# leejet/stable-diffusion.cpp

Hardware: AMD Instinct MI355X
Metric: denoise it/s (image-iterations/s: cond+uncond UNet forwards per image per step) (higher is better)
Workload: dtype f16; 1 GPU; sd15 UNet 512x512, cfg 7 (cond+uncond), f16 weights, batch 8/GPU, Euler-A step; global_batch=8, flash_attn=True, hip_graph=1, cfg_pair_in_one_graph=True, device_resident_sampler=True

## Files before the change

### include/ggml-mi355x.h

```cpp
#ifndef GGML_MI355X_H
#define GGML_MI355X_H

#include "ggml-abi.h"

#ifdef __cplusplus
extern "C" {
#endif

#define GGML_MI355X_API __attribute__((visibility("default")))

GGML_MI355X_API ggml_backend_reg_t ggml_backend_init(void);
GGML_MI355X_API int ggml_backend_score(void);
GGML_MI355X_API ggml_backend_reg_t ggml_backend_mi355x_reg(void);
GGML_MI355X_API int ggml_backend_mi355x_get_device_count(void);

struct ggml_backend_mi355x_stats {
    int64_t graphs_computed;
    int64_t plans_built;
    int64_t nodes_seen;
    int64_t kernels_planned;
    int64_t kernels_launched;
    int64_t fused_conv;
    int64_t fused_conv_bounced;
    int64_t fused_linear;
    int64_t fused_norm;
    int64_t fused_geglu;
    int64_t fused_attention;
    int64_t generic_matmul;
    int64_t swizzled_weight_bytes;
    int64_t graph_replays;
    int64_t fused_linear_geglu;
    int64_t split_k_gemms;
    int64_t head_major_gemms;
    int64_t fused_modulate;
    int64_t fused_gate;
    int64_t fused_gelu;
    int64_t fused_rope;
    int64_t fused_concat_heads;
    int64_t qgemv_linears;
    int64_t fused_chan_add;
    int64_t fused_proj_tokens;
    int64_t gemm_attention;
    int64_t fused_q16;
    int64_t split_k_inlaunch;
    int64_t qgemm16_linears;
    int64_t fgemv_linears;
    int64_t fused_presilu;
    int64_t fused_sibling_linears;
    int64_t hoisted_kv_linears;
    int64_t window_convs;
    int64_t hoisted_emb_linears;
    int64_t fused_rows16;
    int64_t fused_joint_qkv;
    int64_t jit_images;
    int64_t fused_cat_rows16;
    int64_t fused_gn_stats;
    int64_t fused_ln_reduce;
    int64_t redirect_fallbacks;
    int64_t fused_concat_gn;
    int64_t fused_conv_scale;
    int64_t view_graphs;
    int64_t plans_evicted;
    int64_t hoisted_mod_linears;
    int64_t view_external_nodes;
    int64_t qinloop_linears;
    int64_t flash_out_alias;
    int64_t flash_slice_images;
    int64_t flash_short_launches;
    int64_t flash_qb2_launches;
    int64_t flash_mslot_launches;
    int64_t flash_generic_launches;
    int64_t fused_gn_epilogue;
    int64_t fused_tile_merge;
};
GGML_MI355X_API void ggml_backend_mi355x_get_stats(struct ggml_backend_mi355x_stats* out);
GGML_MI355X_API int ggml_backend_mi355x_resolve_enums(const char* (*op_name)(int), const char* (*unary_op_name)(int), const char* (*type_name)(int));
GGML_MI355X_API const char* ggml_backend_mi355x_enum_status(void);
GGML_MI355X_API void ggml_backend_mi355x_get_enum_maps(uint8_t* ops256, uint8_t* unary256);
struct ggml_backend_mi355x_kernel_timing {
    char kernel[96];
    int64_t launches;
    double total_ms;
    double total_flops;
    double total_bytes;
    int32_t bound;
    int32_t family;
};
GGML_MI355X_API void ggml_backend_mi355x_kernel_timing_enable(int enable);
GGML_MI355X_API void ggml_backend_mi355x_kernel_timing_enable_mask(uint32_t family_mask);
GGML_MI355X_API void ggml_backend_mi355x_get_kernel_timing(struct ggml_backend_mi355x_kernel_timing* out);
GGML_MI355X_API int ggml_backend_mi355x_get_kernel_timings(struct ggml_backend_mi355x_kernel_timing* out, int capacity);
GGML_MI355X_API void ggml_backend_mi355x_set_option(const char* key, int value);
struct ggml_backend_mi355x_calibration {
    float mfma_f16_tflops;
    float mfma_clock_mhz;
    float copy_tbs;
    float read_tbs;
    int compute_units;
};
GGML_MI355X_API int ggml_backend_mi355x_calibrate(struct ggml_backend_mi355x_calibration* out);
GGML_MI355X_API void* ggml_backend_mi355x_get_stream(ggml_backend_t backend);
GGML_MI355X_API bool ggml_backend_mi355x_step_cache_probe(ggml_backend_t backend, const float* x, float c_in, const float* prev_in, int64_t n, float* stats);
GGML_MI355X_API bool ggml_backend_mi355x_step_cache_record(ggml_backend_t backend, const float* in, const float* out, float* prev_in, float* prev_out, float* diff, int64_t per,
                                                           int k, int64_t nb, bool has_prev_out, float* stats);
GGML_MI355X_API bool ggml_backend_mi355x_step_cache_probe_rel(ggml_backend_t backend, const float* x, float c_in, const float* prev_in, int64_t n, float* stats);
GGML_MI355X_API bool ggml_backend_mi355x_spectrum_predict(ggml_backend_t backend, const float* ring, int64_t slot_stride, const int* order, int k, const float* weights, float w,
                                                          int64_t n, float* out);
GGML_MI355X_API bool ggml_backend_mi355x_spectrum_push(ggml_backend_t backend, const float* src, float* dst, int64_t n);
GGML_MI355X_API const char* ggml_backend_mi355x_hip_library(void);
GGML_MI355X_API int ggml_backend_mi355x_set_device(int hip_device);
GGML_MI355X_API int ggml_backend_mi355x_get_device(void);

#ifdef __cplusplus
}
#endif
#endif
```

### include/sd-mi355x.h

```cpp
#ifndef SD_MI355X_H
#define SD_MI355X_H

#include <stdbool.h>
#include <stddef.h>
#include <stdint.h>

#ifdef __cplusplus
extern "C" {
#endif

#define SD_API __attribute__((visibility("default")))

enum sd_model_family_t {
    SD_MODEL_SD15       = 0,
    SD_MODEL_SDXL       = 1,
    SD_MODEL_SD15_TINY  = 2,
    SD_MODEL_SDXL_TINY  = 3,
    SD_MODEL_SD35_LARGE = 4,
    SD_MODEL_SD35_TINY  = 5,
    SD_MODEL_FLUX_DEV   = 6,
    SD_MODEL_FLUX_TINY  = 7,
    SD_MODEL_SD35_WIDE2 = 8,
    SD_MODEL_FLUX_WIDE1 = 9,
    SD_MODEL_SD3M_TINY  = 10,
// ... 139 lines not shown
    SDM_CACHE_CACHE_DIT  = 5,
    SDM_CACHE_SPECTRUM   = 6
};
typedef struct {
    enum sdm_cache_mode_t mode;
    float reuse_threshold;
    float start_percent;
    float end_percent;
    float error_decay_rate;
    bool use_relative_threshold;
    bool reset_error_on_compute;
} sdm_cache_params_t;
SD_API void sdm_cache_params_init(sdm_cache_params_t* p);
SD_API bool sd_set_step_cache(sdm_ctx_t* ctx, const sdm_cache_params_t* params);
typedef struct {
    int Fn_compute_blocks;
    int Bn_compute_blocks;
    float residual_diff_threshold;
} sdm_cache_dit_params_t;
typedef struct {
    float w;
    int m;
    float lam;
    int window_size;
    float flex_window;
    int warmup_steps;
    float stop_percent;
} sdm_spectrum_params_t;
SD_API void sdm_cache_dit_params_init(sdm_cache_dit_params_t* p);
SD_API void sdm_spectrum_params_init(sdm_spectrum_params_t* p);
SD_API bool sd_set_step_cache_ex(sdm_ctx_t* ctx, const sdm_cache_params_t* params, const sdm_cache_dit_params_t* cache_dit, const sdm_spectrum_params_t* spectrum);
typedef struct {
    int step;
    float sigma;
    bool active;
    bool skipped;
    float input_change;
    float output_change;
    float output_norm;
    float rate;
    float accumulated;
    float threshold;
} sdm_cache_step_t;
SD_API int sd_step_cache_trace(sdm_ctx_t* ctx, sdm_cache_step_t* out, int capacity);
SD_API const char* sd_step_cache_status(sdm_ctx_t* ctx);
SD_API bool sd_step_cache_device_passes(sdm_ctx_t* ctx);
SD_API float sd_t_to_sigma(sdm_ctx_t* ctx, float t);
SD_API bool sd_step_cache_kernels(sdm_ctx_t* ctx, const float* in, const float* out, const float* prev_in, const float* prev_out, int64_t n, int k, int nb, float c_in,
                                  float* stats, float* diff_out, float* prev_in_out, float* prev_out_out);
SD_API bool sd_step_cache_kernels_rel(sdm_ctx_t* ctx, const float* in, const float* prev_in, int64_t n, float c_in, float* sums);
SD_API bool sd_spectrum_schedule(const sdm_spectrum_params_t* params, int n_calls, uint8_t* predicted);
SD_API bool sd_spectrum_weights(const sdm_spectrum_params_t* params, const float* taus, int k, float tau_at, float* weights);
SD_API bool sd_spectrum_kernels(sdm_ctx_t* ctx, const float* hist, int k, int64_t n, const float* weights, float w, float* out);

SD_API void sd_philox_randn(uint64_t seed, uint32_t offset, uint32_t n, float* out);
SD_API void sd_philox_uint32(uint64_t seed, uint32_t offset, uint32_t n, uint32_t* out );
SD_API int sd_get_sigmas(int steps, float* out );
typedef bool (*sd_pair_exchange_fn)(void* device_eps, int64_t count, void* stream, void* user);
SD_API void sd_set_pair_exchange(sdm_ctx_t* ctx, sd_pair_exchange_fn fn, void* user, int branch);
SD_API bool sd_rccl_get_unique_id(void* id128);
SD_API void* sd_rccl_comm_create(int device, int nranks, int rank, const void* id128);
SD_API void sd_rccl_comm_destroy(void* comm);
SD_API bool sd_set_pair_exchange_rccl(sdm_ctx_t* ctx, void* comm, int branch);
SD_API const char* sd_rccl_last_error(void);
SD_API void sd_set_guidance(sdm_ctx_t* ctx, float guidance);
SD_API void sd_cfg_combine(const float* cond, const float* uncond, int64_t n, float scale, float* out);
SD_API void sd_planar_rgb_to_u8(const float* chw, int width, int height, uint8_t* out);
SD_API int sd_sample_synthetic(int family, int steps, int image_seq_len, int64_t n, uint64_t seed, int method, float eta, float* out, float* aux);
SD_API int sd_sample_synthetic2(int family, int steps, int image_seq_len, int64_t n, uint64_t seed, int method, int scheduler, float eta, float* out, float* aux, int aux_calls);
SD_API int sd_get_sigmas_sched(int family, int scheduler, int steps, int image_seq_len, float shift, float* out);
SD_API void sd_apg_sequence(const float* cond, const float* uncond, int64_t n, int steps, float scale, float eta, float momentum, float norm_threshold,
                            float norm_threshold_smoothing, float* out);
SD_API bool sd_set_vae_conv2d_scale(sdm_ctx_t* ctx, float scale);
SD_API int sd_get_flux_sigmas(int steps, int image_seq_len, float* out );
SD_API int sd_gen_flux_pe(int h, int w, int patch_size, int context_len, const int* axes_dim, int n_axes, float theta, float* out);
SD_API int sd_get_flow_sigmas(int steps, float shift, float* out );
SD_API float sd_sigma_to_t(float sigma);

struct ggml_tensor;
struct ggml_cgraph;
struct ggml_backend;
typedef bool (*sdm_graph_eval_callback_t)(struct ggml_tensor* t, bool ask, void* user_data);
SD_API void sdm_set_backend_eval_callback(sdm_graph_eval_callback_t cb, void* user_data);
SD_API int sdm_backend_graph_compute_with_eval_callback(struct ggml_backend* backend, struct ggml_cgraph* gf, sdm_graph_eval_callback_t cb, void* user_data);

SD_API size_t sdm_graph_describe(struct ggml_cgraph* gf, char* buf, size_t cap);
SD_API void sdm_set_graph_capture(int on);
SD_API size_t sdm_last_graph_description(char* buf, size_t cap);

typedef struct {
    double last_sample_ms;
    double last_decode_ms;
    int64_t unet_calls;
    int64_t graph_nodes;
    size_t compute_buffer_bytes;
    size_t weight_bytes;
    double host_build_ms, host_alloc_ms, host_submit_ms;
    int64_t graph_cache_hits;
    int64_t steps_skipped;
} sd_stats_t;
SD_API void sd_get_stats(sdm_ctx_t* ctx, sd_stats_t* out);
typedef struct {
    const int32_t* ids;
    const float* weights;
    int n;
} sd_token_list_t;
SD_API bool sd_text_encoders_init(sdm_ctx_t* ctx);
SD_API int64_t sd_clip_forward(sdm_ctx_t* ctx, int which, const int32_t* ids, int n_tokens, int max_token_idx, bool return_pooled, int clip_skip, float* out,
                               int64_t out_capacity);
SD_API int64_t sd_t5_forward(sdm_ctx_t* ctx, const int32_t* ids, int n_tokens, float* out, int64_t out_capacity);
SD_API int sd_t5_relative_position_buckets(int q_len, int k_len, int32_t* out );
SD_API bool sd_get_learned_condition(sdm_ctx_t* ctx, const sd_token_list_t* clip_l, const sd_token_list_t* clip_g, const sd_token_list_t* t5, int clip_skip,
                                     int width, int height, bool zero_out_masked, float* crossattn_out, int64_t crossattn_capacity, int64_t* crossattn_ne,
                                     float* vector_out, int64_t vector_capacity, int64_t* vector_n);


#ifdef __cplusplus
}
#endif
#endif
```

### stable-diffusion.cpp_amd/__init__.py

```python
from __future__ import annotations

import ctypes as C
import os
from pathlib import Path

import numpy as np

PKG_DIR = Path(__file__).resolve().parent
ROOT = PKG_DIR.parent
LIB_DIR = PKG_DIR / "lib"
HOST_LIB = Path(os.environ.get("SDCPP_HOST_LIB", str(LIB_DIR / "libsdcpp-host.so")))
BACKEND_LIB = Path(os.environ.get("SDCPP_BACKEND_LIB", str(LIB_DIR / "libggml-mi355x.so")))

F32, F16, Q4_0, Q8_0, I32, BF16 = 0, 1, 2, 8, 26, 30
TYPE_SIZE = {F32: 4, F16: 2, BF16: 2, I32: 4}

SD15, SDXL, SD15_TINY, SDXL_TINY, SD35_LARGE, SD35_TINY, FLUX_DEV, FLUX_TINY, SD35_WIDE2, FLUX_WIDE1, SD3M_TINY, SD35_WIDE8, FLUX_WIDE8 = 0, 1, 2, 3, 4, 5, 6, 7, 8, 9, 10, 11, 12
PAIR_EXCHANGE_FN = C.CFUNCTYPE(C.c_bool, C.c_void_p, C.c_int64, C.c_void_p, C.c_void_p)
EVAL_CALLBACK_FN = C.CFUNCTYPE(C.c_bool, C.c_void_p, C.c_bool, C.c_void_p)
EULER, EULER_A, HEUN, DPM2, DPMPP2S_A, DPMPP2M, DPMPP2Mv2, IPNDM, IPNDM_V, LCM, DDIM_TRAILING = range(11)
TCD, RES_MULTISTEP, RES_2S, ER_SDE, EULER_CFG_PP, EULER_A_CFG_PP, EULER_GE, DPMPP2M_SDE, DPMPP2M_SDE_BT, LMS = range(11, 21)
SAMPLE_METHOD_DEFAULT = 21
SCHED_DISCRETE, SCHED_KARRAS, SCHED_EXPONENTIAL, SCHED_AYS, SCHED_GITS, SCHED_SGM_UNIFORM, SCHED_SIMPLE, SCHED_SMOOTHSTEP, SCHED_KL_OPTIMAL, SCHED_LCM = range(10)
SCHED_BONG_TANGENT, SCHED_FLUX, SCHED_BETA, SCHEDULER_DEFAULT = 10, 14, 15, 16
# ... 28 lines not shown
    _fields_ = [("mem_size", C.c_size_t), ("mem_buffer", C.c_void_p), ("no_alloc", C.c_bool)]


class SdCtxParams(C.Structure):
    _fields_ = [
        ("backend", C.c_char_p),
        ("model", C.c_int),
        ("wtype", C.c_int),
        ("diffusion_flash_attn", C.c_bool),
        ("diffusion_conv_direct", C.c_bool),
        ("vae_decode_only", C.c_bool),
        ("weight_seed", C.c_uint64),
        ("n_threads", C.c_int),
    ]


class SdSampleParams(C.Structure):
    _fields_ = [("txt_cfg", C.c_float), ("scheduler", C.c_int), ("sample_method", C.c_int),
                ("sample_steps", C.c_int), ("eta", C.c_float), ("custom_sigmas", C.c_void_p), ("custom_sigmas_count", C.c_int),
                ("slg_layers", C.c_void_p), ("slg_layer_count", C.c_int), ("slg_layer_start", C.c_float), ("slg_layer_end", C.c_float), ("slg_scale", C.c_float),
                ("apg_eta", C.c_float), ("apg_momentum", C.c_float), ("apg_norm_threshold", C.c_float), ("apg_norm_threshold_smoothing", C.c_float),
                ("shifted_timestep", C.c_int), ("flow_shift", C.c_float)]


class SdCondition(C.Structure):
    _fields_ = [("c_crossattn", C.POINTER(C.c_float)), ("ctx_dim", C.c_int64), ("n_tokens", C.c_int64),
                ("c_vector", C.POINTER(C.c_float)), ("vector_dim", C.c_int64)]


class SdImgGenParams(C.Structure):
    _fields_ = [("cond", SdCondition), ("uncond", SdCondition), ("width", C.c_int), ("height", C.c_int),
                ("sample_params", SdSampleParams), ("seed", C.c_int64), ("batch_count", C.c_int),
                ("device_batch", C.c_int), ("decode", C.c_bool), ("fuse_cfg_pair", C.c_bool), ("device_sampler", C.c_bool),
                ("init_latent", C.c_void_p), ("denoise_mask", C.c_void_p), ("strength", C.c_float)]


class SdTokenList(C.Structure):
    _fields_ = [("ids", C.POINTER(C.c_int32)), ("weights", C.POINTER(C.c_float)), ("n", C.c_int)]


class SdImage(C.Structure):
    _fields_ = [("width", C.c_uint32), ("height", C.c_uint32), ("channel", C.c_uint32), ("data", C.POINTER(C.c_uint8))]


class SdTilingParams(C.Structure):
    _fields_ = [("enabled", C.c_bool), ("tile_size_x", C.c_int), ("tile_size_y", C.c_int), ("target_overlap", C.c_float),
                ("rel_size_x", C.c_float), ("rel_size_y", C.c_float), ("tile_batch", C.c_int)]


class SdStats(C.Structure):
    _fields_ = [("last_sample_ms", C.c_double), ("last_decode_ms", C.c_double), ("unet_calls", C.c_int64),
                ("graph_nodes", C.c_int64), ("compute_buffer_bytes", C.c_size_t), ("weight_bytes", C.c_size_t),
                ("host_build_ms", C.c_double), ("host_alloc_ms", C.c_double), ("host_submit_ms", C.c_double),
                ("graph_cache_hits", C.c_int64), ("steps_skipped", C.c_int64)]


class SdCacheParams(C.Structure):
    _fields_ = [("mode", C.c_int), ("reuse_threshold", C.c_float), ("start_percent", C.c_float), ("end_percent", C.c_float), ("error_decay_rate", C.c_float),
                ("use_relative_threshold", C.c_bool), ("reset_error_on_compute", C.c_bool)]


class SdCacheDitParams(C.Structure):
    _fields_ = [("Fn_compute_blocks", C.c_int), ("Bn_compute_blocks", C.c_int), ("residual_diff_threshold", C.c_float)]


class SdSpectrumParams(C.Structure):
    _fields_ = [("w", C.c_float), ("m", C.c_int), ("lam", C.c_float), ("window_size", C.c_int), ("flex_window", C.c_float), ("warmup_steps", C.c_int),
                ("stop_percent", C.c_float)]


def cache_dit_params(**over) -> SdCacheDitParams:
    p = SdCacheDitParams()
    lib().sdm_cache_dit_params_init(C.byref(p))
    for k, v in over.items():
        setattr(p, {"Fn": "Fn_compute_blocks", "Bn": "Bn_compute_blocks", "threshold": "residual_diff_threshold"}.get(k, k), v)
    return p


def spectrum_params(**over) -> SdSpectrumParams:
    p = SdSpectrumParams()
    lib().sdm_spectrum_params_init(C.byref(p))
    for k, v in over.items():
        if k not in dict(SdSpectrumParams._fields_):
            raise TypeError("sdm_spectrum_params_t has no field " + k)
        setattr(p, k, v)
    return p


def spectrum_schedule(n_calls: int, **over) -> str:
    p = spectrum_params(**over)
    buf = (C.c_uint8 * max(n_calls, 1))()
    L = lib()
    L.sd_spectrum_schedule.argtypes = [C.POINTER(SdSpectrumParams), C.c_int, C.c_void_p]
    L.sd_spectrum_schedule.restype = C.c_bool
    if not L.sd_spectrum_schedule(C.byref(p), n_calls, buf):
        raise EngineError("sd_spectrum_schedule failed: " + L.sd_last_error().decode())
    return "".join("P" if buf[i] else "C" for i in range(n_calls))


def spectrum_weights(taus, tau_at: float, **over) -> np.ndarray:
    p = spectrum_params(**over)
    t = np.ascontiguousarray(taus, dtype=np.float32)
    out = np.empty(t.size, dtype=np.float32)
    L = lib()
    L.sd_spectrum_weights.argtypes = [C.POINTER(SdSpectrumParams), C.c_void_p, C.c_int, C.c_float, C.c_void_p]
    L.sd_spectrum_weights.restype = C.c_bool
    if not L.sd_spectrum_weights(C.byref(p), _fptr(t), int(t.size), float(tau_at), _fptr(out)):
# ... 164 lines not shown
    L.sd_set_pair_exchange_rccl.argtypes = [C.c_void_p, C.c_void_p, C.c_int]
    L.sd_set_pair_exchange_rccl.restype = C.c_bool
    L.sd_rccl_last_error.restype = C.c_char_p
    L.sd_gen_flux_pe.argtypes = [C.c_int, C.c_int, C.c_int, C.c_int, C.POINTER(C.c_int), C.c_int, C.c_float, C.c_void_p]
    L.sd_sigma_to_t.argtypes = [C.c_float]
    L.sd_sigma_to_t.restype = C.c_float
    L.sd_get_stats.argtypes = [C.c_void_p, C.POINTER(SdStats)]
    L.sd_load_weights_prefixed.argtypes = [C.c_void_p, C.c_char_p, C.c_char_p, C.POINTER(C.c_int64), C.POINTER(C.c_int64)]
    L.sd_load_weights_prefixed.restype = C.c_int64
    L.sd_convert_tensor_name.argtypes = [C.c_void_p, C.c_char_p, C.c_char_p, C.c_size_t]
    L.sd_convert_tensor_name.restype = C.c_bool
    L.sd_text_encoders_init.argtypes = [C.c_void_p]
    L.sd_text_encoders_init.restype = C.c_bool
    L.sd_clip_forward.argtypes = [C.c_void_p, C.c_int, C.c_void_p, C.c_int, C.c_int, C.c_bool, C.c_int, C.c_void_p, C.c_int64]
    L.sd_clip_forward.restype = C.c_int64
    L.sd_t5_forward.argtypes = [C.c_void_p, C.c_void_p, C.c_int, C.c_void_p, C.c_int64]
    L.sd_t5_forward.restype = C.c_int64
    L.sd_t5_relative_position_buckets.argtypes = [C.c_int, C.c_int, C.c_void_p]
    L.sd_get_learned_condition.argtypes = [C.c_void_p, C.POINTER(SdTokenList), C.POINTER(SdTokenList), C.POINTER(SdTokenList), C.c_int, C.c_int, C.c_int,
                                           C.c_bool, C.c_void_p, C.c_int64, C.POINTER(C.c_int64), C.c_void_p, C.c_int64, C.POINTER(C.c_int64)]
    L.sd_get_learned_condition.restype = C.c_bool
    L.sdm_set_backend_eval_callback.argtypes = [EVAL_CALLBACK_FN, C.c_void_p]
    L.sdm_set_backend_eval_callback.restype = None
    L.sdm_backend_graph_compute_with_eval_callback.argtypes = [C.c_void_p, C.c_void_p, EVAL_CALLBACK_FN, C.c_void_p]
    L.sdm_backend_graph_compute_with_eval_callback.restype = C.c_int
    _lib = L
    return L


_loaded_plugins: set[str] = set()


def load_backend(path: os.PathLike | str) -> None:
    p = str(Path(path).resolve())
    if p in _loaded_plugins:
        return
    if not lib().sd_load_backend(p.encode()):
        raise EngineError(f"failed to load backend plug-in {p}")
    _loaded_plugins.add(p)


def load_mi355x_backend() -> None:
    if not BACKEND_LIB.exists():
        raise EngineError(f"{BACKEND_LIB} missing — the HIP backend was not built")
    load_backend(BACKEND_LIB)
    names = devices()
    if not any(n.upper().startswith("MI355X") for n in names):
        raise EngineError(f"libggml-mi355x.so loaded but exposes no MI355X device (devices: {names}); is a gfx950 GPU visible?")


_BACKEND_STAT_FIELDS = ("graphs_computed plans_built nodes_seen kernels_planned kernels_launched fused_conv fused_conv_bounced fused_linear "
                        "fused_norm fused_geglu fused_attention generic_matmul swizzled_weight_bytes graph_replays fused_linear_geglu "
                        "split_k_gemms head_major_gemms fused_modulate fused_gate fused_gelu fused_rope fused_concat_heads qgemv_linears fused_chan_add fused_proj_tokens gemm_attention fused_q16 split_k_inlaunch qgemm16_linears fgemv_linears fused_presilu fused_sibling_linears hoisted_kv_linears window_convs hoisted_emb_linears fused_rows16 fused_joint_qkv jit_images fused_cat_rows16 fused_gn_stats fused_ln_reduce redirect_fallbacks fused_concat_gn fused_conv_scale view_graphs plans_evicted hoisted_mod_linears view_external_nodes qinloop_linears flash_out_alias flash_slice_images "
                        "flash_short_launches flash_qb2_launches flash_mslot_launches flash_generic_launches fused_gn_epilogue fused_tile_merge").split()


class BackendStats(C.Structure):
    _fields_ = [(n, C.c_int64) for n in _BACKEND_STAT_FIELDS]


_backend_cdll = None


def _backend() -> C.CDLL:
    global _backend_cdll
    if _backend_cdll is None:
        load_mi355x_backend()
        _backend_cdll = C.CDLL(str(BACKEND_LIB))
        _backend_cdll.ggml_backend_mi355x_get_stats.argtypes = [C.POINTER(BackendStats)]
        _backend_cdll.ggml_backend_mi355x_set_option.argtypes = [C.c_char_p, C.c_int]
    return _backend_cdll


def backend_stats() -> dict:
    st = BackendStats()
    _backend().ggml_backend_mi355x_get_stats(C.byref(st))
    return {n: int(getattr(st, n)) for n in _BACKEND_STAT_FIELDS}


class KernelTiming(C.Structure):
    _fields_ = [("kernel", C.c_char * 96), ("launches", C.c_int64), ("total_ms", C.c_double), ("total_flops", C.c_double),
                ("total_bytes", C.c_double), ("bound", C.c_int32), ("family", C.c_int32)]


KF_ALL = 0x3FFFF


def kernel_timing_enable(on) -> None:
    b = _backend()
    b.ggml_backend_mi355x_kernel_timing_enable_mask.argtypes = [C.c_uint32]
    mask = 1 if on is True else int(on or 0)
    b.ggml_backend_mi355x_kernel_timing_enable_mask(mask)


def _timing_dict(kt) -> dict:
    return {"kernel": kt.kernel.decode(), "family": int(kt.family), "bound": "hbm" if kt.bound else "mfma", "launches": int(kt.launches),
            "total_ms": float(kt.total_ms), "total_flops": float(kt.total_flops), "total_bytes": float(kt.total_bytes)}


def kernel_timings() -> list:
    arr = (KernelTiming * 32)()
    b = _backend()
    b.ggml_backend_mi355x_get_kernel_timings.argtypes = [C.POINTER(KernelTiming), C.c_int]
    b.ggml_backend_mi355x_get_kernel_timings.restype = C.c_int
    n = b.ggml_backend_mi355x_get_kernel_timings(arr, 32)
    return [_timing_dict(arr[i]) for i in range(n)]

# ... 271 lines not shown
            ok = L.sd_set_step_cache(self._ctx, None if p is None else C.byref(p))
        else:
            d = None if cache_dit is None else C.byref(cache_dit_params(**cache_dit))
            sp = None if spectrum is None else C.byref(spectrum_params(**spectrum))
            ok = L.sd_set_step_cache_ex(self._ctx, None if p is None else C.byref(p), d, sp)
        if not ok:
            raise EngineError("sd_set_step_cache failed: " + L.sd_last_error().decode())

    def step_cache_trace(self) -> list:
        L = lib()
        L.sd_step_cache_trace.argtypes = [C.c_void_p, C.POINTER(SdCacheStep), C.c_int]
        L.sd_step_cache_trace.restype = C.c_int
        n = L.sd_step_cache_trace(self._ctx, None, 0)
        buf = (SdCacheStep * max(n, 1))()
        n = min(n, L.sd_step_cache_trace(self._ctx, buf, n))
        return [{f[0]: getattr(buf[i], f[0]) for f in SdCacheStep._fields_} for i in range(n)]

    def step_cache_status(self) -> str:
        L = lib()
        L.sd_step_cache_status.argtypes = [C.c_void_p]
        L.sd_step_cache_status.restype = C.c_char_p
        return L.sd_step_cache_status(self._ctx).decode()

    def step_cache_device_passes(self) -> bool:
        L = lib()
        L.sd_step_cache_device_passes.argtypes = [C.c_void_p]
        L.sd_step_cache_device_passes.restype = C.c_bool
        return bool(L.sd_step_cache_device_passes(self._ctx))

    def step_cache_kernels_rel(self, inp: np.ndarray, prev_in: np.ndarray, c_in: float = 1.0) -> np.ndarray:
        a = np.ascontiguousarray(inp, dtype=np.float32).ravel()
        pi = np.ascontiguousarray(prev_in, dtype=np.float32).ravel()
        assert a.size == pi.size
        sums = np.zeros(2, dtype=np.float32)
        L = lib()
        L.sd_step_cache_kernels_rel.argtypes = [C.c_void_p, C.c_void_p, C.c_void_p, C.c_int64, C.c_float, C.c_void_p]
        L.sd_step_cache_kernels_rel.restype = C.c_bool
        if not L.sd_step_cache_kernels_rel(self._ctx, _fptr(a), _fptr(pi), a.size, float(c_in), _fptr(sums)):
            raise EngineError("sd_step_cache_kernels_rel failed: " + L.sd_last_error().decode())
        return sums

    def spectrum_kernels(self, hist: np.ndarray, weights: np.ndarray, w: float) -> np.ndarray:
        h = np.ascontiguousarray(hist, dtype=np.float32)
        wt = np.ascontiguousarray(weights, dtype=np.float32)
        k, n = h.shape
        assert wt.size == k
        out = np.empty(n, dtype=np.float32)
        L = lib()
        L.sd_spectrum_kernels.argtypes = [C.c_void_p, C.c_void_p, C.c_int, C.c_int64, C.c_void_p, C.c_float, C.c_void_p]
        L.sd_spectrum_kernels.restype = C.c_bool
        if not L.sd_spectrum_kernels(self._ctx, _fptr(h), k, n, _fptr(wt), float(w), _fptr(out)):
            raise EngineError("sd_spectrum_kernels failed: " + L.sd_last_error().decode())
        return out

    def t_to_sigma(self, t: float) -> float:
        L = lib()
        L.sd_t_to_sigma.argtypes = [C.c_void_p, C.c_float]
        L.sd_t_to_sigma.restype = C.c_float
        return float(L.sd_t_to_sigma(self._ctx, float(t)))

    def step_cache_kernels(self, inp: np.ndarray, out: np.ndarray, prev_in: np.ndarray, prev_out: np.ndarray | None, c_in: float = 1.0):
        a, o, pi = _f32(inp), _f32(out), _f32(prev_in)
        po = None if prev_out is None else _f32(prev_out)
        nb, n = a.shape
        k = o.shape[1]
        assert o.shape == (nb, k, n) and pi.shape == a.shape and (po is None or po.shape == a.shape)
        stats = np.zeros(3, dtype=np.float32)
        diff, pin2, pout2 = np.empty_like(o), np.empty_like(a), np.empty_like(a)
        L = lib()
        L.sd_step_cache_kernels.argtypes = [C.c_void_p, C.c_void_p, C.c_void_p, C.c_void_p, C.c_void_p, C.c_int64, C.c_int, C.c_int, C.c_float, C.c_void_p, C.c_void_p,
                                            C.c_void_p, C.c_void_p]
        L.sd_step_cache_kernels.restype = C.c_bool
        if not L.sd_step_cache_kernels(self._ctx, _fptr(a), _fptr(o), _fptr(pi), _fptr(po), n, k, nb, float(c_in), _fptr(stats), _fptr(diff), _fptr(pin2), _fptr(pout2)):
            raise EngineError("sd_step_cache_kernels failed: " + L.sd_last_error().decode())
        return stats, diff, pin2, pout2

    def vae_encode(self, rgb: np.ndarray, seed: int = 42, return_moments: bool = False):
        x = _f32(rgb)
        n, c, h, w = x.shape
        assert c == 3
        zc = 16 if self.model in (SD35_LARGE, SD35_TINY, FLUX_DEV, FLUX_TINY, SD35_WIDE2, FLUX_WIDE1, SD3M_TINY, SD35_WIDE8, FLUX_WIDE8) else 4
        out = np.empty((n, zc, h // 8, w // 8), dtype=np.float32)
        mom = np.empty((n, 2 * zc, h // 8, w // 8), dtype=np.float32)
        L = lib()
        L.sd_vae_encode.argtypes = [C.c_void_p, C.c_void_p, C.c_int, C.c_int, C.c_int, C.c_uint64, C.c_void_p, C.c_void_p]
        L.sd_vae_encode.restype = C.c_bool
        if not L.sd_vae_encode(self._ctx, _fptr(x), w, h, n, seed, _fptr(out), _fptr(mom)):
            raise EngineError("sd_vae_encode failed: " + L.sd_last_error().decode())
        return (out, mom) if return_moments else out

    def tae_decode(self, latents: np.ndarray) -> np.ndarray:
        z = _f32(latents)
        n, c, h, w = z.shape
        out = np.empty((n, 3, h * 8, w * 8), dtype=np.float32)
        L = lib()
        L.sd_tae_decode.argtypes = [C.c_void_p, C.c_void_p, C.c_int, C.c_int, C.c_int, C.c_int, C.c_void_p]
        L.sd_tae_decode.restype = C.c_bool
        if not L.sd_tae_decode(self._ctx, _fptr(z), w, h, c, n, _fptr(out)):
            raise EngineError("sd_tae_decode failed: " + L.sd_last_error().decode())
        return out

    def set_prediction(self, prediction: int):
        L = lib()
        L.sd_set_prediction.argtypes = [C.c_void_p, C.c_int]
        L.sd_set_prediction.restype = C.c_bool
        if not L.sd_set_prediction(self._ctx, int(prediction)):
# ... 325 lines not shown
```

### stable-diffusion.cpp_amd/csrc/backend/backend.cpp

```cpp
#include <hip/hip_runtime.h>

#include <atomic>
#include <cstdio>
#include <cstdlib>
#include <cstring>
#include <mutex>
#include <string>
#include <vector>

#include "ggml-abi.h"
#include "ggml-abi-check.h"
#include <dlfcn.h>
#include <link.h>

#include "ggml-mi355x.h"
#include "ktime.h"
#include "planner.h"
#include "kernels.h"

namespace mi355x {

#define HIP_OK(expr)                                                                                          \
    do {                                                                                                      \
        hipError_t _e = (expr);                                                                               \
// ... 187 lines not shown
    p->name        = dev_get_name(d);
    p->description = dev_get_desc(d);
    dev_get_memory(d, &p->memory_free, &p->memory_total);
    p->type                      = GGML_BACKEND_DEVICE_TYPE_GPU;
    p->caps.async                = true;
    p->caps.host_buffer          = false;
    p->caps.buffer_from_host_ptr = false;
    p->caps.events               = false;
}
static ggml_backend_t dev_init_backend(ggml_backend_dev_t d, const char*) {
    DeviceCtx* dc = (DeviceCtx*)d->context;
    if (hipSetDevice(dc->id) != hipSuccess) return nullptr;
    BackendCtx* c = new BackendCtx();
    c->dev        = dc;
    if (hipStreamCreate(&c->stream) != hipSuccess) {
        delete c;
        return nullptr;
    }
    c->planner       = planner_create(dc->id);
    ggml_backend* b  = new ggml_backend();
    memset(b, 0, sizeof(*b));
    b->guid                   = &g_guid;
    b->iface.get_name         = be_get_name;
    b->iface.free             = be_free;
    b->iface.set_tensor_async = be_set_async;
    b->iface.get_tensor_async = be_get_async;
    b->iface.synchronize      = be_synchronize;
    b->iface.graph_compute    = be_graph_compute;
    b->device                 = d;
    b->context                = c;
    return b;
}
static ggml_backend_buffer_type_t dev_get_buft(ggml_backend_dev_t d) { return &((DeviceCtx*)d->context)->buft; }
static bool dev_supports_op(ggml_backend_dev_t, const ggml_tensor* op) { return planner_supports_op(op); }
static bool dev_supports_buft(ggml_backend_dev_t d, ggml_backend_buffer_type_t t) { return t == &((DeviceCtx*)d->context)->buft; }
static bool dev_offload_op(ggml_backend_dev_t, const ggml_tensor*) { return false; }

static const char* reg_get_name(ggml_backend_reg_t) { return "MI355X"; }
static size_t reg_dev_count(ggml_backend_reg_t) { return g_devices.size(); }
static ggml_backend_dev_t reg_get_dev(ggml_backend_reg_t, size_t i) { return i < g_devices.size() ? &g_devices[i]->dev : nullptr; }
static void* reg_get_proc(ggml_backend_reg_t, const char* name) {
    if (strcmp(name, "ggml_backend_mi355x_get_stats") == 0) return (void*)ggml_backend_mi355x_get_stats;
    if (strcmp(name, "ggml_backend_mi355x_set_option") == 0) return (void*)ggml_backend_mi355x_set_option;
    if (strcmp(name, "ggml_backend_mi355x_kernel_timing_enable") == 0) return (void*)ggml_backend_mi355x_kernel_timing_enable;
    if (strcmp(name, "ggml_backend_mi355x_get_kernel_timing") == 0) return (void*)ggml_backend_mi355x_get_kernel_timing;
    if (strcmp(name, "ggml_backend_mi355x_get_kernel_timings") == 0) return (void*)ggml_backend_mi355x_get_kernel_timings;
    if (strcmp(name, "ggml_backend_mi355x_kernel_timing_enable_mask") == 0) return (void*)ggml_backend_mi355x_kernel_timing_enable_mask;
    if (strcmp(name, "ggml_backend_mi355x_get_stream") == 0) return (void*)ggml_backend_mi355x_get_stream;
    if (strcmp(name, "ggml_backend_mi355x_step_cache_probe") == 0) return (void*)ggml_backend_mi355x_step_cache_probe;
    if (strcmp(name, "ggml_backend_mi355x_step_cache_record") == 0) return (void*)ggml_backend_mi355x_step_cache_record;
    if (strcmp(name, "ggml_backend_mi355x_step_cache_probe_rel") == 0) return (void*)ggml_backend_mi355x_step_cache_probe_rel;
    if (strcmp(name, "ggml_backend_mi355x_spectrum_predict") == 0) return (void*)ggml_backend_mi355x_spectrum_predict;
    if (strcmp(name, "ggml_backend_mi355x_spectrum_push") == 0) return (void*)ggml_backend_mi355x_spectrum_push;
    if (strcmp(name, "ggml_backend_mi355x_hip_library") == 0) return (void*)ggml_backend_mi355x_hip_library;
    if (strcmp(name, "ggml_backend_mi355x_set_device") == 0) return (void*)ggml_backend_mi355x_set_device;
    if (strcmp(name, "ggml_backend_mi355x_get_device") == 0) return (void*)ggml_backend_mi355x_get_device;
    return nullptr;
}

typedef const char* (*name_of_fn)(int);
static std::string g_enum_status = "not resolved (ggml_backend_init not called)";
static bool g_enum_ok            = true;
static std::mutex g_enum_mu;
static bool g_enum_explicit = false;

static void* find_host_symbol(const char* sym) {
    if (void* p = dlsym(RTLD_DEFAULT, sym)) return p;
    struct Ctx {
        const char* sym;
        void* found;
    } ctx{sym, nullptr};
    dl_iterate_phdr(
        [](struct dl_phdr_info* info, size_t, void* data) -> int {
            Ctx* c = (Ctx*)data;
            if (!info->dlpi_name || !info->dlpi_name[0]) return 0;
            if (void* h = dlopen(info->dlpi_name, RTLD_NOLOAD | RTLD_LAZY)) {
                void* p = dlsym(h, c->sym);
                dlclose(h);
                if (p) {
                    c->found = p;
                    return 1;
                }
            }
            return 0;
        },
        &ctx);
    return ctx.found;
}

static bool resolve_host_enums(name_of_fn opn, name_of_fn unn, name_of_fn tyn, const char* how) {
    char err[256] = {0};
    if (!opn && !unn && !tyn) {
        g_enum_status = "host exports no ggml_op_name / ggml_unary_op_name / ggml_type_name: enum numbering of include/ggml-abi.h assumed";
        g_enum_ok     = true;
        return true;
    }
    g_enum_ok = planner_build_op_maps(opn, unn, tyn, err, sizeof(err));
    if (g_enum_ok)
        g_enum_status = std::string("op / unary-op numbers translated by name, type numbers verified (") + how + ")";
    else
        g_enum_status = std::string("ENUM MISMATCH (") + how + "): " + err;
    return g_enum_ok;
}

static void init_once() {
    static std::once_flag once;
// ... 115 lines not shown
    o->total_ms    = t.total_ms;
    o->total_flops = t.total_flops;
    o->total_bytes = t.total_bytes;
    o->bound       = t.bound;
    o->family      = family;
}
GGML_MI355X_API void ggml_backend_mi355x_kernel_timing_enable(int enable) { mi355x::ktime_enable(enable ? 1u : 0u); }
GGML_MI355X_API void ggml_backend_mi355x_kernel_timing_enable_mask(uint32_t family_mask) { mi355x::ktime_enable(family_mask); }
GGML_MI355X_API void* ggml_backend_mi355x_get_stream(ggml_backend_t backend) {
    return backend ? (void*)((mi355x::BackendCtx*)backend->context)->stream : nullptr;
}
static float* step_cache_scratch(mi355x::BackendCtx* c) {
    if (!c->step_cache_partial && hipMalloc((void**)&c->step_cache_partial, mi355x::step_cache_partial_bytes()) != hipSuccess) {
        (void)hipGetLastError();
        c->step_cache_partial = nullptr;
    }
    return c->step_cache_partial;
}
GGML_MI355X_API bool ggml_backend_mi355x_step_cache_probe(ggml_backend_t backend, const float* x, float c_in, const float* prev_in, int64_t n, float* stats) {
    if (!backend || !x || !prev_in || !stats) return false;
    mi355x::BackendCtx* c = (mi355x::BackendCtx*)backend->context;
    if (hipSetDevice(c->dev->id) != hipSuccess) return false;
    float* partial = step_cache_scratch(c);
    return partial && mi355x::launch_step_cache_probe(c->stream, x, c_in, prev_in, n, partial, stats);
}
GGML_MI355X_API bool ggml_backend_mi355x_step_cache_record(ggml_backend_t backend, const float* in, const float* out, float* prev_in, float* prev_out, float* diff, int64_t per,
                                                           int k, int64_t nb, bool has_prev_out, float* stats) {
    if (!backend || !in || !out || !prev_in || !prev_out || !diff || !stats) return false;
    mi355x::BackendCtx* c = (mi355x::BackendCtx*)backend->context;
    if (hipSetDevice(c->dev->id) != hipSuccess) return false;
    float* partial = step_cache_scratch(c);
    return partial && mi355x::launch_step_cache_record(c->stream, in, out, prev_in, prev_out, diff, per, k, nb, has_prev_out, partial, stats + 1);
}
GGML_MI355X_API bool ggml_backend_mi355x_step_cache_probe_rel(ggml_backend_t backend, const float* x, float c_in, const float* prev_in, int64_t n, float* stats) {
    if (!backend || !x || !prev_in || !stats) return false;
    mi355x::BackendCtx* c = (mi355x::BackendCtx*)backend->context;
    if (hipSetDevice(c->dev->id) != hipSuccess) return false;
    float* partial = step_cache_scratch(c);
    return partial && mi355x::launch_step_cache_probe_rel(c->stream, x, c_in, prev_in, n, partial, stats);
}
GGML_MI355X_API bool ggml_backend_mi355x_spectrum_predict(ggml_backend_t backend, const float* ring, int64_t slot_stride, const int* order, int k, const float* weights, float w,
                                                          int64_t n, float* out) {
    if (!backend || !ring || !order || !weights || !out) return false;
    mi355x::BackendCtx* c = (mi355x::BackendCtx*)backend->context;
    if (hipSetDevice(c->dev->id) != hipSuccess) return false;
    return mi355x::launch_spectrum_predict(c->stream, ring, slot_stride, order, k, weights, w, n, out);
}
GGML_MI355X_API bool ggml_backend_mi355x_spectrum_push(ggml_backend_t backend, const float* src, float* dst, int64_t n) {
    if (!backend || !src || !dst || n < 1) return false;
    mi355x::BackendCtx* c = (mi355x::BackendCtx*)backend->context;
    if (hipSetDevice(c->dev->id) != hipSuccess) return false;
    return hipMemcpyAsync(dst, src, (size_t)n * sizeof(float), hipMemcpyDeviceToDevice, c->stream) == hipSuccess;
}
GGML_MI355X_API const char* ggml_backend_mi355x_hip_library(void) {
    static std::string path;
    if (path.empty()) {
        Dl_info info;
        if (dladdr((void*)&hipGetDeviceCount, &info) && info.dli_fname) path = info.dli_fname;
    }
    return path.c_str();
}
GGML_MI355X_API int ggml_backend_mi355x_set_device(int hip_device) { return hipSetDevice(hip_device) == hipSuccess ? 0 : -1; }
GGML_MI355X_API int ggml_backend_mi355x_get_device(void) {
    int d = -1;
    return hipGetDevice(&d) == hipSuccess ? d : -1;
}
GGML_MI355X_API int ggml_backend_mi355x_get_kernel_timings(struct ggml_backend_mi355x_kernel_timing* out, int capacity) {
    mi355x::KFamTiming t[mi355x::KF_COUNT];
    int fam[mi355x::KF_COUNT];
    const int n = mi355x::ktime_read(t, mi355x::KF_COUNT, fam);
    int m       = 0;
    for (int i = 0; i < n && m < capacity; ++i) fill_timing(&out[m++], t[i], fam[i]);
    return m;
}
GGML_MI355X_API void ggml_backend_mi355x_get_kernel_timing(struct ggml_backend_mi355x_kernel_timing* out) {
    struct ggml_backend_mi355x_kernel_timing all[mi355x::KF_COUNT];
    const int n = ggml_backend_mi355x_get_kernel_timings(all, mi355x::KF_COUNT);
    if (n > 0) {
        *out = all[0];
    } else {
        memset(out, 0, sizeof(*out));
        snprintf(out->kernel, sizeof(out->kernel), "(no timed launches)");
    }
}
}
```

### stable-diffusion.cpp_amd/csrc/backend/planner.cpp

```cpp
#include "planner.h"

#include <atomic>
#include <cstddef>
#include <cstdio>
#include <cstdlib>
#include <cstring>
#include <functional>
#include <memory>
#include <mutex>
#include <string>
#include <algorithm>
#include <map>
#include <unordered_map>
#include <unordered_set>
#include <vector>

#include "kernels.h"
#include "ktime.h"

namespace mi355x {

static uint8_t g_opmap[256];
static uint8_t g_unmap[256];
static bool g_opmap_init = [] {
// ... 1266 lines not shown
            for (int c : cj) {
                gi.done[c] = 1;
                members.push_back(c);
            }
        }
    }
    B.hm_grouping = false;
    const Builder::HmLaunch& h0 = B.hm_group[0];
    bool fuse = B.hm_group.size() >= 2;
    for (const auto& h : B.hm_group) {
        fuse = fuse && h.a_off == h0.a_off && h.lda == h0.lda && h.tokens == h0.tokens && h.K == h0.K && h.M == h0.M && h.hd == h0.hd && h.hH == h0.hH && h.hL == h0.hL &&
               h.ep.scale == h0.ep.scale;
        emit_pos = std::max(emit_pos, h.out_node);
    }
    for (const auto& h : B.hm_group) fuse = fuse && read_only_after(gi, h.out_node, emit_pos, members);
    if (!fuse) {
        for (const auto& h : B.hm_group) {
            if (h.node == i)
                B.emit(hm_single_step(P, h));
            else
                B.deferred[h.node].push_back(hm_single_step(P, h));
        }
        B.hm_group.clear();
        return;
    }
    const std::vector<Builder::HmLaunch> grp = B.hm_group;
    B.hm_group.clear();
    STAT(fused_sibling_linears) += (int64_t)grp.size() - 1;
    B.emit_at(emit_pos, i, [=](hipStream_t st) {
        float* dst[16]        = {};
        void* dst16[16]       = {};
        const void* wswz[16]  = {};
        const float* bias[16] = {};
        const int nn = (int)grp.size();
        for (int k = 0; k < nn; ++k) {
            dst[k]   = grp[k].dst;
            dst16[k] = grp[k].dst16_arena ? (void*)(P->arena + grp[k].dst16_off) : grp[k].dst16;
            wswz[k]  = grp[k].swz;
            bias[k]  = grp[k].ep.bias;
        }
        launch_gemm16_linear_multi(st, nn, dst, dst16, P->arena + grp[0].a_off, grp[0].lda, wswz, grp[0].tokens, grp[0].K, grp[0].M, bias, grp[0].ep.scale, grp[0].hd, grp[0].hH,
                                   grp[0].hL);
    });
}

void plan_hoisted_kv(Builder& B, hipStream_t s) {
    if (!g_opt.hoist_kv || !g_opt.fusion || !g_opt.fuse_siblings) return;
    GInfo& gi  = B.gi;
    Planner* P = B.P;
    struct Key {
        const ggml_tensor* x;
        int wtype;
        int64_t K, M, d, H, L;
        bool operator<(const Key& o) const { return std::tie(x, wtype, K, M, d, H, L) < std::tie(o.x, o.wtype, o.K, o.M, o.d, o.H, o.L); }
    };
    std::map<Key, std::vector<int>> groups;
    for (int j = 0; j < gi.g->n_nodes; ++j) {
        const ggml_tensor* n = gi.node(j);
        if (xop(n) != GGML_OP_MUL_MAT || !linear_fast_ok(n)) continue;
        const ggml_tensor* x  = n->src[1];
        const ggml_tensor* xr = strip_reshape(x);
        if (!(gi.idx(xr) < 0 || xop(xr) == GGML_OP_REPEAT)) continue;
        const int j1 = gi.sole(j);
        const int j2 = (j1 >= 0 && xop(gi.node(j1)) == GGML_OP_RESHAPE) ? gi.sole(j1) : -1;
        const int j3 = (j2 >= 0 && xop(gi.node(j2)) == GGML_OP_PERMUTE) ? gi.sole(j2) : -1;
        const int j4 = (j3 >= 0 && xop(gi.node(j3)) == GGML_OP_CONT) ? gi.sole(j3) : -1;
        const int j5 = (j4 >= 0 && xop(gi.node(j4)) == GGML_OP_RESHAPE) ? gi.sole(j4) : -1;
        if (j5 < 0 || xop(gi.node(j5)) != GGML_OP_CPY || gi.node(j5)->type != GGML_TYPE_F16) continue;
        int jf = -1, nread = 0;
        for (int c : gi.consumers[j5])
            if (c != j5) {
                jf = c;
                ++nread;
            }
        if (nread != 1 || (gi.node(j5)->flags & GGML_TENSOR_FLAG_OUTPUT) || xop(gi.node(jf)) != GGML_OP_FLASH_ATTN_EXT || !planner_supports_op(gi.node(jf))) continue;
        const ggml_tensor* f = gi.node(jf);
        if (!((f->src[1] == gi.node(j5)) != (f->src[2] == gi.node(j5))) || f->src[0] == gi.node(j5)) continue;
        const ggml_tensor* r4 = gi.node(j1);
        const ggml_tensor* w  = n->src[0];
        groups[Key{x, (int)w->type, w->ne[0], w->ne[1], r4->ne[0], r4->ne[1], r4->ne[2]}].push_back(j);
    }
    for (auto& kv : groups) {
        std::vector<int>& mem = kv.second;
        if (mem.size() < 3) continue;
        const int j0 = mem[0];
        for (size_t c0 = 0; c0 < mem.size(); c0 += 16) {
            const size_t c1 = std::min(mem.size(), c0 + 16);
            if (c1 - c0 < 2) break;
            B.hm_group.clear();
            B.hm_grouping = true;
            B.hm_hoisting = true;
            for (size_t m = c0; m < c1; ++m) {
                const int j = mem[m];
                std::vector<int> cj;
                B.emit_redirect = j;
                if (m == c0) B.emit_redirect = j0;
                const size_t before = B.hm_group.size();
                plan_linear(B, j, s, cj);
                B.emit_redirect = -1;
                if (B.hm_group.size() != before + 1) {
                    fprintf(stderr, "[ggml-mi355x] plan_hoisted_kv: projection at node %d was not captured\n", j);
                    abort();
                }
                for (int c : cj) gi.done[c] = 1;
            }
            B.hm_grouping = false;
            B.hm_hoisting = false;
            std::vector<Builder::HmLaunch> grp = B.hm_group;
            B.hm_group.clear();
            bool ok = grp.size() >= 2;
            for (const auto& h : grp)
                ok = ok && h.dst16 && !h.dst && !h.dst16_arena && h.a_off == grp[0].a_off && h.lda == grp[0].lda && h.tokens == grp[0].tokens && h.K == grp[0].K && h.M == grp[0].M &&
                     h.hd == grp[0].hd && h.hH == grp[0].hH && h.hL == grp[0].hL && h.ep.scale == grp[0].ep.scale;
            if (!ok) {
                for (const auto& h : grp) B.deferred[h.node].push_back(hm_single_step(P, h));
                continue;
            }
            for (auto& h : grp) {
                h.dst16_off   = B.alloc((size_t)h.tokens * h.M * 2);
                h.dst16_arena = true;
                h.dst16       = nullptr;
                B.moved[gi.node(h.out_node)] = h.dst16_off;
            }
            STAT(hoisted_kv_linears) += (int64_t)grp.size();
            STAT(fused_sibling_linears) += (int64_t)grp.size() - 1;
            B.deferred[j0].push_back([=](hipStream_t st) {
                float* dst[16]        = {};
                void* dst16[16]       = {};
                const void* wswz[16]  = {};
                const float* bias[16] = {};
                const int nn = (int)grp.size();
                for (int k = 0; k < nn; ++k) {
                    dst16[k] = P->arena + grp[k].dst16_off;
                    wswz[k]  = grp[k].swz;
                    bias[k]  = grp[k].ep.bias;
                }
                launch_gemm16_linear_multi(st, nn, dst, dst16, P->arena + grp[0].a_off, grp[0].lda, wswz, grp[0].tokens, grp[0].K, grp[0].M, bias, grp[0].ep.scale, grp[0].hd,
                                           grp[0].hH, grp[0].hL);
            });
        }
    }
}

struct EmbMember {
    int silu, mm, add;
    int64_t M;
};
void plan_hoisted_emb(Builder& B, hipStream_t s) {
    if (!g_opt.hoist_emb || !g_opt.fusion || !g_opt.fuse_chan_add) return;
    GInfo& gi  = B.gi;
    Planner* P = B.P;
    struct Key {
        const ggml_tensor* e;
        int wtype;
        int64_t K, rows;
        bool operator<(const Key& o) const { return std::tie(e, wtype, K, rows) < std::tie(o.e, o.wtype, o.K, o.rows); }
    };
    std::map<Key, std::vector<EmbMember>> groups;
    for (int j = 0; j < gi.g->n_nodes; ++j) {
        const ggml_tensor* n = gi.node(j);
        if (xop(n) != GGML_OP_MUL_MAT || !linear_fast_ok(n)) continue;
        const ggml_tensor* w = n->src[0];
        const ggml_tensor* x = n->src[1];
        const int is = gi.idx(x);
        if (is < 0 || xop(x) != GGML_OP_UNARY || xunary(x) != GGML_UNARY_OP_SILU || gi.sole(is) != j || !contig(x) || !is_f32(x)) continue;
        const ggml_tensor* e = x->src[0];
        if (!e || !is_f32(e) || !contig(e) || e->ne[2] != 1 || e->ne[3] != 1 || !aligned16(e->data) || (x->flags & GGML_TENSOR_FLAG_OUTPUT)) continue;
        const int64_t K = w->ne[0], M = w->ne[1], rows = x->ne[1];
        if (x->ne[2] != 1 || x->ne[3] != 1 || !aligned16(w->data) || w->nb[1] != ggml_abi_row_size(w->type, K)) continue;
        const bool fg = g_opt.fgemv && fgemv_supported((int)w->type, rows, K);
        const bool qg = g_opt.qgemv && qgemv_supported((int)w->type, rows, K);
        if (!fg && !qg) continue;
        const int ja = gi.sole(j);
        if (ja < 0 || xop(gi.node(ja)) != GGML_OP_ADD || gi.node(ja)->src[0] != n || !bias_like_row(gi.node(ja)->src[1], M) || gi.node(ja)->data != n->data ||
            !is_static_weight(gi.node(ja)->src[1]) || (gi.node(ja)->flags & GGML_TENSOR_FLAG_OUTPUT))
            continue;
        int jr = gi.sole(ja);
        if (jr < 0 || xop(gi.node(jr)) != GGML_OP_RESHAPE) continue;
        const ggml_tensor* r = gi.node(jr);
        if (!(r->ne[0] == 1 && r->ne[1] == 1 && r->ne[2] == M && r->ne[3] == rows)) continue;
        const int jc = gi.sole(jr);
        if (jc < 0 || xop(gi.node(jc)) != GGML_OP_ADD || gi.node(jc)->src[1] != r) continue;
        if (gi.idx(e) > j) continue;
        groups[Key{e, (int)w->type, K, rows}].push_back(EmbMember{is, j, ja, M});
    }
    for (auto& kv : groups) {
// ... 2285 lines not shown
        case GGML_OP_NORM:
        case GGML_OP_RMS_NORM:
            return f32c(n) && f32c(n->src[0]) && n->src[0]->nb[0] == 4;
        case GGML_OP_GROUP_NORM:
            return f32c(n) && f32c(n->src[0]) && ggml_abi_is_contiguous(n->src[0]) && ggml_abi_is_contiguous(n);
        case GGML_OP_SOFT_MAX:
            return f32c(n) && f32c(n->src[0]) && ggml_abi_is_contiguous(n->src[0]) && ggml_abi_op_param_f32(n, 1) == 0.0f &&
                   (!n->src[1] || ((n->src[1]->type == GGML_TYPE_F16 || n->src[1]->type == GGML_TYPE_F32) && n->src[1]->ne[2] == 1 && n->src[1]->ne[3] == 1));
        case GGML_OP_MUL_MAT: {
            const ggml_tensor *a = n->src[0], *b = n->src[1];
            if (!a || !b || n->type != GGML_TYPE_F32) return false;
            const bool at = a->type == GGML_TYPE_F32 || a->type == GGML_TYPE_F16 || a->type == GGML_TYPE_BF16 || a->type == GGML_TYPE_Q8_0 || a->type == GGML_TYPE_Q4_0;
            const bool bt = b->type == GGML_TYPE_F32 || b->type == GGML_TYPE_F16;
            return at && bt && a->nb[0] == ggml_abi_type_size(a->type) && b->nb[0] == ggml_abi_type_size(b->type);
        }
        case GGML_OP_IM2COL:
            return f32c(n->src[1]) && (n->type == GGML_TYPE_F16 || n->type == GGML_TYPE_F32);
        case GGML_OP_CONV_2D: {
            const ggml_tensor *k = n->src[0], *x = n->src[1];
            if (!k || !x || k->type != GGML_TYPE_F16 || !f32c(x) || !ggml_abi_is_contiguous(x) || !ggml_abi_is_contiguous(k)) return false;
            const int32_t* p = n->op_params;
            const int ks     = (int)k->ne[0];
            if (k->ne[1] != ks || p[0] != p[1] || p[2] != p[3] || p[4] != 1 || p[5] != 1) return false;
            return (ks == 3 && p[2] == 1 && (p[0] == 1 || p[0] == 2)) || (ks == 1 && p[2] == 0 && p[0] == 1);
        }
        case GGML_OP_CONCAT:
        case GGML_OP_REPEAT:
        case GGML_OP_UPSCALE:
        case GGML_OP_PAD:
            if (xop(n) == GGML_OP_UPSCALE && n->op_params[0] != GGML_SCALE_MODE_NEAREST) return false;
            return f32c(n) && f32c(n->src[0]);
        case GGML_OP_GET_ROWS: {
            const ggml_tensor *a = n->src[0], *b = n->src[1];
            if (!a || !b || !f32c(n) || b->type != GGML_TYPE_I32 || n->nb[0] != 4) return false;
            const bool at = a->type == GGML_TYPE_F32 || a->type == GGML_TYPE_F16 || a->type == GGML_TYPE_BF16 || a->type == GGML_TYPE_Q8_0 || a->type == GGML_TYPE_Q4_0;
            return at && a->nb[0] == ggml_abi_type_size(a->type);
        }
        case GGML_OP_TIMESTEP_EMBEDDING:
            return f32c(n) && f32c(n->src[0]);
        case GGML_OP_FLASH_ATTN_EXT: {
            const ggml_tensor *q = n->src[0], *k = n->src[1], *v = n->src[2];
            if (!q || !k || !v || n->src[3] != nullptr) return false;
            if (!f32c(q) || !(k->type == GGML_TYPE_F16 || k->type == GGML_TYPE_F32) || v->type != k->type) return false;
            if (ggml_abi_op_param_f32(n, 1) != 0.0f || ggml_abi_op_param_f32(n, 2) != 0.0f) return false;
            if (q->nb[0] != 4 || k->nb[0] != ggml_abi_type_size(k->type) || v->nb[0] != ggml_abi_type_size(v->type)) return false;
            if (q->ne[3] != 1 || k->ne[2] != q->ne[2]) return false;
            return flash_attn_supported(q->ne[0], v->ne[0]);
        }
        default:
            return false;
    }
}

void planner_get_stats(ggml_backend_mi355x_stats* o) {
    int64_t* out = reinterpret_cast<int64_t*>(o);
    for (size_t i = 0; i < N_STATS; ++i) out[i] = g_stat_counters[i].load();
    o->flash_short_launches   = flash_attn_variant_launches(FLASH_VAR_SHORT);
    o->flash_qb2_launches     = flash_attn_variant_launches(FLASH_VAR_QB2);
    o->flash_mslot_launches   = flash_attn_variant_launches(FLASH_VAR_MSLOT);
    o->flash_generic_launches = flash_attn_variant_launches(FLASH_VAR_GENERIC);
}

namespace {
struct OptionRow {
    const char* key;
    std::atomic<int> Options::*member;
    void (*setter)(int);
};
#define OPT(name) {#name, &Options::name, nullptr}
const OptionRow g_option_table[] = {
    OPT(fusion),
    OPT(mfma_gemm),
    OPT(hip_graph),
    OPT(flash_pattern),
    {"gemm16_t320", nullptr, gemm16_set_t320},
    {"t256p_pad", nullptr, gemm16_set_t256p_pad},
    {"tail_split", nullptr, gemm16_set_tail_split},
    {"conv_wmajor", nullptr, gemm16_set_conv_wmajor},
    {"ln16_rows", nullptr, gemm16_set_ln16_rows},
    {"t320_linear_max_split", nullptr, gemm16_set_t320_linear_max_split},
    OPT(qgemv),
    OPT(fuse_q16),
    {"streamk", nullptr, gemm16_set_streamk},
    {"geglu16", nullptr, gemm16_set_geglu16},
    {"bn64_max_tiles", nullptr, gemm16_set_bn64_max},
    {"conv3w_prio", nullptr, conv3w_set_prio},
    {"t256p_min_nt_sk", nullptr, gemm16_set_t256p_min_nt_sk},
    {"t256p_min_tiles_sk", nullptr, gemm16_set_t256p_min_tiles_sk},
    {"conv3w", nullptr, conv3w_set},
    OPT(hoist_emb),
    OPT(fuse_rows16),
    OPT(fuse_cat_rows16),
    OPT(fuse_gn_stats),
    OPT(fuse_gn_epilogue),
    OPT(fuse_tile_merge),
    OPT(fuse_joint_qkv),
    OPT(fuse_ln_reduce),
    OPT(jit_qimages),
    {"qinloop_min_rows", nullptr, gemm16_set_qinloop_min_rows},
    OPT(fuse_flash_slices),
    {"gemm16_t192p", nullptr, gemm16_set_t192p},
    {"conv3w_min_blocks", nullptr, conv3w_set_min_blocks},
    {"conv3w_min_blocks_deep", nullptr, conv3w_set_min_blocks_deep},
    {"gemm16_bn64", nullptr, gemm16_set_bn64},
    OPT(qgemm16),
    {"qgemv_max_rows", nullptr, qgemv_set_max_rows},
// ... 60 lines not shown
```

### stable-diffusion.cpp_amd/csrc/backend/planner.h

```cpp
#pragma once
#include <hip/hip_runtime.h>

#include "ggml-abi.h"
#include "ggml-mi355x.h"

namespace mi355x {

struct Planner;
Planner* planner_create(int device);
void planner_destroy(Planner* p);
enum ggml_status planner_compute(Planner* p, ggml_cgraph* g, hipStream_t stream);
bool planner_supports_op(const ggml_tensor* op);
void planner_forget_range(const void* ptr, size_t size);
void planner_get_stats(ggml_backend_mi355x_stats* out);
void planner_set_option(const char* key, int value);
bool planner_build_op_maps(const char* (*op_name)(int), const char* (*unary_name)(int), const char* (*type_name)(int), char* err, size_t err_len);
void planner_get_op_maps(uint8_t* ops256, uint8_t* unary256);

}
```

### stable-diffusion.cpp_amd/csrc/host/engine.cpp

```cpp
#include <dlfcn.h>

#include <atomic>
#include <chrono>
#include <cmath>
#include <cstdio>
#include <cstdlib>
#include <cstring>
#include <future>
#include <memory>
#include <mutex>
#include <string>
#include <thread>
#include <unordered_map>
#include <vector>

#include "ggml.h"
#include "models.hpp"
#include "conditioner.hpp"
#include "sampler.hpp"
#include "step_cache.hpp"
#include "model_io.hpp"
#include "torch_ckpt_io.hpp"
#include "name_conversion.hpp"
#include "sd-mi355x.h"
// ... 256 lines not shown
                    ggml_fp32_to_bf16_row(src + i0, (ggml_bf16_t*)dst + i0, (int64_t)(i1 - i0));
            }, 1 << 20);
        } else if (n < (1 << 20)) {
            ggml_quantize_chunk(ty, src, dst, 0, rows, per_row, nullptr);
        } else {
            parallel_chunks((size_t)rows, [&](size_t r0, size_t r1) { ggml_quantize_chunk(ty, src, dst, (int64_t)r0 * per_row, (int64_t)(r1 - r0), per_row, nullptr); }, 2);
        }
        ggml_backend_tensor_set(t, scratch.data(), 0, scratch.size());
    }

    std::string cache_sig;
    ggml_context* cache_ctx = nullptr;
    ggml_cgraph* cache_gf   = nullptr;
    ggml_tensor* cache_res  = nullptr;
    std::vector<HostInput> cache_inputs, cache_builtin;
    int64_t cache_hits = 0;
    void drop_cache() {
        if (cache_ctx) ggml_free(cache_ctx);
        cache_ctx = nullptr;
        cache_gf  = nullptr;
        cache_res = nullptr;
        cache_inputs.clear();
        cache_builtin.clear();
        cache_sig.clear();
    }

    template <typename BuildFn>
    bool compute(BuildFn&& build, float* out, size_t out_bytes, const std::string& sig = std::string(), const std::vector<const void*>& ptrs = {}) {
        ggml_context* cctx = nullptr;
        ggml_cgraph* gf    = nullptr;
        ggml_tensor* res   = nullptr;
        std::vector<HostInput> local_inputs, local_builtin;
        std::vector<HostInput>* inputs = &local_inputs;
        const bool cacheable = !sig.empty();
        double t_s = now_ms();
        if (cacheable && cache_ctx && cache_sig == sig && cache_inputs.size() == ptrs.size()) {
            cctx = cache_ctx;
            gf   = cache_gf;
            res  = cache_res;
            for (size_t i = 0; i < ptrs.size(); ++i) cache_inputs[i].data = ptrs[i];
            inputs = &cache_inputs;
            ++cache_hits;
        } else {
            drop_cache();
            ggml_init_params ip{0, nullptr, true};
            cctx = ggml_init(ip);
            gf   = ggml_new_graph_custom(cctx, graph_size, false);
            GraphCtx g;
            g.ctx            = cctx;
            g.backend        = backend;
            const double t_b = now_ms();
            res              = build(g, local_inputs);
            ggml_set_name(res, "ggml_runner_final_result_tensor");
            ggml_build_forward_expand(gf, res);
            {
                ggml_tensor* one = ggml_new_tensor_1d(cctx, GGML_TYPE_F32, 1);
                ggml_set_name(one, "ggml_runner_build_in_tensor:one");
                ggml_set_input(one);
                ggml_tensor* zero_int = ggml_new_tensor_1d(cctx, GGML_TYPE_I32, 1);
                ggml_set_name(zero_int, "ggml_runner_build_in_tensor:zero_int");
                ggml_set_input(zero_int);
                ggml_build_forward_expand(gf, one);
                ggml_build_forward_expand(gf, zero_int);
                static const float one_v    = 1.f;
                static const int32_t zero_v = 0;
                local_builtin.push_back(HostInput{one, &one_v, sizeof(one_v)});
                local_builtin.push_back(HostInput{zero_int, &zero_v, sizeof(zero_v)});
            }
            const double t_a = now_ms();
            build_ms += t_a - t_b;
            if (!galloc) galloc = ggml_gallocr_new(ggml_backend_get_default_buffer_type(backend));
            const bool ok = ggml_gallocr_alloc_graph(galloc, gf);
            t_s           = now_ms();
            alloc_ms += t_s - t_a;
            if (!ok) {
                set_error("compute buffer allocation failed");
                ggml_free(cctx);
                return false;
            }
            if (cacheable) {
                bool same = ptrs.size() == local_inputs.size();
                for (size_t i = 0; same && i < ptrs.size(); ++i) same = ptrs[i] == local_inputs[i].data;
                if (same) {
                    cache_sig    = sig;
                    cache_ctx    = cctx;
                    cache_gf     = gf;
                    cache_res    = res;
                    cache_inputs = local_inputs;
                    inputs       = &cache_inputs;
                    cache_builtin = local_builtin;
                }
            }
        }
        const bool keep  = cctx == cache_ctx;
        const bool async = out == nullptr;
        if (g_graph_capture) g_last_graph = describe_graph(gf);
        if (g_graph_capture == 2) {
            set_error("graph captured, compute skipped (sdm_set_graph_capture(2))");
            if (keep)
                drop_cache();
            else
                ggml_free(cctx);
            return false;
        }
        for (const std::vector<HostInput>* list : {(const std::vector<HostInput>*)inputs, (const std::vector<HostInput>*)(keep ? &cache_builtin : &local_builtin)})
            for (auto& in : *list) {
// ... 36 lines not shown
struct sdm_ctx_t {
    sdm_ctx_params_t params;
    ggml_backend_t backend = nullptr;
    Runner unet_runner, vae_runner;
    UNetModel unet;
    MMDiTModel mmdit;
    FluxModel flux;
    bool is_dit = false, is_flux = false;
    float guidance = 3.5f;
    float vae_conv2d_scale = 1.f;
    FluxFlowDenoiser flux_denoiser;
    VaeDecoder vae;
    CompVisDenoiser denoiser;
    DiscreteFlowDenoiser flow_denoiser;
    int in_channels() const { return is_flux ? 16 : (is_dit ? (int)mmdit.cfg.in_channels : unet.cfg.in_channels); }
    int out_channels() const { return is_flux ? 16 : (is_dit ? (int)mmdit.cfg.out_channels : unet.cfg.out_channels); }
    std::vector<float> get_sigmas(uint32_t n, int image_seq_len, int sched = SCHED_COUNT) const {
        if (sched == SCHED_COUNT) sched = is_flux ? SCHED_FLUX : SCHED_DISCRETE;
        if (sched == SCHED_FLUX) return flux_denoiser.get_sigmas(n, image_seq_len);
        if (is_flux) return scheduler_sigmas(sched, n, flux_denoiser.sigma_min(), flux_denoiser.sigma_max(), [&](float t) { return flux_denoiser.t_to_sigma(t); }, -1);
        if (is_dit) return scheduler_sigmas(sched, n, flow_denoiser.sigma_min(), flow_denoiser.sigma_max(), [&](float t) { return flow_denoiser.t_to_sigma(t); }, -1);
        const int ays = (params.model == SD_MODEL_SD15 || params.model == SD_MODEL_SD15_TINY) ? 0 : 1;
        return scheduler_sigmas(sched, n, denoiser.sigma_min(), denoiser.sigma_max(), [&](float t) { return denoiser.t_to_sigma(t); }, ays);
    }
    void scalings(float sigma, float& c_skip, float& c_out, float& c_in) const {
        if (is_flux)
            flux_denoiser.scalings(sigma, c_skip, c_out, c_in);
        else if (is_dit)
            flow_denoiser.scalings(sigma, c_skip, c_out, c_in);
        else if (prediction == SDM_V_PRED) {
            const float sigma_data = 1.0f;
            c_skip = sigma_data * sigma_data / (sigma * sigma + sigma_data * sigma_data);
            c_out  = -sigma * sigma_data / std::sqrt(sigma * sigma + sigma_data * sigma_data);
            c_in   = 1.0f / std::sqrt(sigma * sigma + sigma_data * sigma_data);
        } else
            denoiser.scalings(sigma, c_skip, c_out, c_in);
    }
    int prediction = SDM_EPS_PRED;
    float sigma_to_t(float sigma) const { return is_flux ? sigma : (is_dit ? flow_denoiser.sigma_to_t(sigma) : denoiser.sigma_to_t(sigma)); }
    sd_stats_t stats{};
    std::vector<std::pair<std::string, ggml_tensor*>> all_tensors;
    struct TextEncoders {
        Runner l_runner, g_runner, t5_runner;
        ClipTextModel clip_l, clip_g;
        T5Model t5;
        ConditionerSpec spec;
        Runner* runner(int which) { return which == 0 ? &l_runner : (which == 1 ? &g_runner : &t5_runner); }
    };
    std::unique_ptr<TextEncoders> te;
    struct SamplerState {
        ggml_context* sctx        = nullptr;
        ggml_backend_buffer_t buf = nullptr;
        ggml_tensor *x = nullptr, *noise = nullptr, *eps = nullptr;
        int64_t W = 0, H = 0, C = 0, N = 0;
        struct Cache {
            ggml_context* cctx        = nullptr;
            ggml_backend_buffer_t buf = nullptr;
            ggml_tensor *in = nullptr, *out = nullptr, *prev_in = nullptr, *prev_out = nullptr, *diff = nullptr, *stats = nullptr;
            int k = 0;
            uint64_t serial = 0;
            ~Cache() {
                if (buf) ggml_backend_buffer_free(buf);
                if (cctx) ggml_free(cctx);
            }
        };
        std::unique_ptr<Cache> cache;
        struct Spectrum {
            ggml_context* cctx        = nullptr;
            ggml_backend_buffer_t buf = nullptr;
            ggml_tensor *ring = nullptr, *denoised = nullptr;
            int K = 0;
            int64_t stride = 0;
            uint64_t serial = 0;
            ~Spectrum() {
                if (buf) ggml_backend_buffer_free(buf);
                if (cctx) ggml_free(cctx);
            }
        };
        std::unique_ptr<Spectrum> spectrum;
        ~SamplerState() {
            cache.reset();
            spectrum.reset();
            if (buf) ggml_backend_buffer_free(buf);
            if (sctx) ggml_free(sctx);
        }
    };
    std::unique_ptr<SamplerState> sstate;
    sd_pair_exchange_fn pair_fn = nullptr;
    void* pair_user             = nullptr;
    int pair_branch             = 0;
    Runner pair_runner;
    sdm_cache_params_t cache_params{SDM_CACHE_DISABLED, INFINITY, 0.15f, 0.95f, 1.0f, true, true};
    sdm_cache_dit_params_t cache_dit_params{8, 0, 0.08f};
    sdm_spectrum_params_t spectrum_params{0.40f, 3, 1.0f, 2, 0.50f, 4, 0.9f};
    StepCacheRuntime step_cache;
    Runner skip_runner;
    float t_to_sigma(float t) const { return is_flux ? flux_denoiser.t_to_sigma(t) : (is_dit ? flow_denoiser.t_to_sigma(t) : denoiser.t_to_sigma(t)); }
    bool step_cache_would_arm(int method) const {
        if (!StepCacheRuntime::has_valid_cache_percent_range(cache_params)) return false;
        if (cache_params.mode == SDM_CACHE_SPECTRUM) return !sample_method_needs_uncond(method);
        if (StepCacheRuntime::is_cachedit_mode(cache_params.mode)) return is_dit;
        return (cache_params.mode == SDM_CACHE_EASYCACHE && is_dit) || (cache_params.mode == SDM_CACHE_UCACHE && !is_dit);
    }
    void step_cache_begin_trajectory(const std::vector<float>& sigmas, int method) {
        step_cache.init(&cache_params, is_dit, !is_dit, [this](float t) { return t_to_sigma(t); }, sigmas, &cache_dit_params, &spectrum_params,
                        sample_method_needs_uncond(method));
    }
    std::vector<float> pe_cache;
    int pe_h = 0, pe_w = 0;
    int64_t pe_tokens = 0;
    Runner vae_enc_runner;
    VaeEncoder vae_enc;
    bool vae_enc_ready = false;
    Runner tae_runner;
    TaeDecoder tae;
    bool tae_ready = false, tae_for_images = false;
    sdm_tiling_params_t tiling{false, 0, 0, 0.5f, 0.f, 0.f, 0};
    struct TileState {
        ggml_context* sctx        = nullptr;
        ggml_backend_buffer_t buf = nullptr;
        ggml_gallocr_t merge_galloc = nullptr;
        ggml_tensor* canvas = nullptr;
        ggml_tensor* store[2] = {nullptr, nullptr};
        ggml_tensor *wx = nullptr, *wy = nullptr;
        std::string key;
        uint64_t serial = 0;
        ~TileState() {
            if (merge_galloc) ggml_gallocr_free(merge_galloc);
            if (buf) ggml_backend_buffer_free(buf);
            if (sctx) ggml_free(sctx);
        }
    };
    std::unique_ptr<TileState> tstate[3];
    std::vector<Runner*> runners() {
        std::vector<Runner*> v{&unet_runner, &vae_runner};
        if (tae_ready) v.push_back(&tae_runner);
        if (vae_enc_ready) v.push_back(&vae_enc_runner);
        if (te) {
            if (te->spec.has_l) v.push_back(&te->l_runner);
            if (te->spec.has_g) v.push_back(&te->g_runner);
            if (te->spec.has_t5) v.push_back(&te->t5_runner);
        }
        return v;
    }
    ~sdm_ctx_t() {
    }
};

extern "C" {
// ... 59 lines not shown
    ggml_backend_dev_t dev = ggml_backend_dev_by_name(dev_name);
    if (!dev && !params->backend) {
        const std::string path = self_dir() + "/libggml-mi355x.so";
        if (!ggml_backend_load(path.c_str())) {
            set_error("MI355X backend plug-in missing or failed to load: " + path);
            return nullptr;
        }
        dev = ggml_backend_dev_by_name(dev_name);
    }
    if (!dev) {
        set_error(std::string("no ggml device named '") + dev_name + "' (is a gfx950 GPU visible?)");
        return nullptr;
    }
    ggml_backend_t backend = ggml_backend_dev_init(dev, nullptr);
    if (!backend) {
        set_error("ggml_backend_dev_init failed");
        return nullptr;
    }
    sdm_ctx_t* ctx = new sdm_ctx_t();
    ctx->params   = *params;
    ctx->backend  = backend;

    const bool xl   = params->model == SD_MODEL_SDXL || params->model == SD_MODEL_SDXL_TINY;
    const bool tiny = params->model == SD_MODEL_SD15_TINY || params->model == SD_MODEL_SDXL_TINY;
    const bool flux     = params->model == SD_MODEL_FLUX_DEV || params->model == SD_MODEL_FLUX_TINY || params->model == SD_MODEL_FLUX_WIDE1 || params->model == SD_MODEL_FLUX_WIDE8;
    const bool dit      = params->model == SD_MODEL_SD35_LARGE || params->model == SD_MODEL_SD35_TINY || params->model == SD_MODEL_SD35_WIDE2 || params->model == SD_MODEL_SD35_WIDE8 || params->model == SD_MODEL_SD3M_TINY || flux;
    const bool dit_tiny = params->model == SD_MODEL_SD35_TINY || params->model == SD_MODEL_FLUX_TINY || params->model == SD_MODEL_SD3M_TINY;
    UNetConfig ucfg = tiny ? UNetConfig::tiny(xl) : (xl ? UNetConfig::sdxl_base() : UNetConfig::sd15());
    VaeConfig vcfg  = (tiny || dit_tiny) ? VaeConfig::tiny() : (xl ? VaeConfig::sdxl() : VaeConfig::sd15());
    if (tiny && xl) vcfg.scale_factor = 0.13025f;
    if (dit) {
        vcfg.z_channels   = 16;
        vcfg.use_quant    = false;
        vcfg.scale_factor = flux ? 0.3611f : 1.5305f;
        vcfg.shift_factor = flux ? 0.1159f : 0.0609f;
    }

    ctx->unet_runner.backend        = backend;
    ctx->unet_runner.ps.linear_type = (ggml_type)params->wtype;
    ctx->is_dit                     = dit;
    ctx->is_flux                    = flux;
    if (flux) {
        ctx->unet_runner.graph_size = 32768 * 4;
        ctx->flux.init(ctx->unet_runner.ps, "model.diffusion_model.", dit_tiny ? FluxConfig::tiny() : (params->model == SD_MODEL_FLUX_WIDE1 ? FluxConfig::flux_wide1() : (params->model == SD_MODEL_FLUX_WIDE8 ? FluxConfig::flux_wide8() : FluxConfig::flux_dev())));
    } else if (dit) {
        ctx->unet_runner.graph_size = 10240 * 8;
        ctx->mmdit.init(ctx->unet_runner.ps, "model.diffusion_model.", dit_tiny ? (params->model == SD_MODEL_SD3M_TINY ? MMDiTConfig::tiny_medium() : MMDiTConfig::tiny()) : (params->model == SD_MODEL_SD35_WIDE2 ? MMDiTConfig::sd35_wide2() : (params->model == SD_MODEL_SD35_WIDE8 ? MMDiTConfig::sd35_wide8() : MMDiTConfig::sd35_large())));
    } else
        ctx->unet.init(ctx->unet_runner.ps, "model.diffusion_model.", ucfg);
    ctx->pair_runner.backend       = backend;
    ctx->pair_runner.graph_size    = 256;
    ctx->skip_runner.backend       = backend;
    ctx->skip_runner.graph_size    = 256;
    ctx->vae_runner.backend        = backend;
    ctx->vae_runner.ps.linear_type = GGML_TYPE_F16;
    ctx->vae_runner.graph_size     = 20480;
    ctx->vae.init(ctx->vae_runner.ps, "first_stage_model.", vcfg);
    if (xl) {
        ctx->vae_conv2d_scale = 1.f / 32.f;
        ctx->vae.set_conv2d_scale(ctx->vae_conv2d_scale);
    }

    if (!ctx->unet_runner.alloc_weights(params->weight_seed) || !ctx->vae_runner.alloc_weights(params->weight_seed)) {
        set_error("weight buffer allocation failed");
        sdm_free_ctx(ctx);
        return nullptr;
    }
    for (auto* r : {&ctx->unet_runner, &ctx->vae_runner})
        for (auto& sp : r->ps.specs) ctx->all_tensors.push_back({sp.name, sp.tensor});
    ctx->stats.weight_bytes = ggml_backend_buffer_get_size(ctx->unet_runner.weights) + ggml_backend_buffer_get_size(ctx->vae_runner.weights);
    return ctx;
}

void sdm_free_ctx(sdm_ctx_t* ctx) {
    if (!ctx) return;
    ggml_backend_t b = ctx->backend;
    delete ctx;
    ggml_backend_free(b);
}

int64_t sd_tensor_count(sdm_ctx_t* ctx) { return (int64_t)ctx->all_tensors.size(); }
const char* sd_tensor_name(sdm_ctx_t* ctx, int64_t i) { return ctx->all_tensors[i].first.c_str(); }
static ggml_tensor* find_tensor(sdm_ctx_t* ctx, const char* name) {
    for (Runner* r : ctx->runners()) {
        auto it = r->ps.by_name.find(name);
        if (it != r->ps.by_name.end()) return it->second;
    }
    return nullptr;
}
bool sd_tensor_info(sdm_ctx_t* ctx, const char* name, int64_t* ne, int* type, size_t* nbytes) {
    ggml_tensor* t = find_tensor(ctx, name);
    if (!t) return false;
    for (int i = 0; i < 4; ++i) ne[i] = t->ne[i];
    *type   = (int)t->type;
    *nbytes = ggml_nbytes(t);
    return true;
}
bool sd_get_tensor(sdm_ctx_t* ctx, const char* name, void* dst, size_t nbytes) {
    ggml_tensor* t = find_tensor(ctx, name);
    if (!t || nbytes != ggml_nbytes(t)) return false;
    ggml_backend_tensor_get(t, dst, 0, nbytes);
    return true;
}
bool sd_get_tensor_f32(sdm_ctx_t* ctx, const char* name, float* dst, int64_t nelem) {
    ggml_tensor* t = find_tensor(ctx, name);
    if (!t || nelem != ggml_nelements(t)) return false;
// ... 1249 lines not shown
        ggml_backend_tensor_get(prev_in, b.data(), 0, (size_t)n * sizeof(float));
        float sum = 0.0f, mag = 0.0f;
        for (int64_t i = 0; i < n; ++i) {
            const float m = a[(size_t)i] * c_in;
            sum += std::fabs(b[(size_t)i] - m);
            mag += std::fabs(b[(size_t)i]);
        }
        ggml_backend_tensor_set(stats, &sum, 0, sizeof(float));
        ggml_backend_tensor_set(stats, &mag, 3 * sizeof(float), sizeof(float));
        return true;
    }
    bool spectrum_predict(ggml_tensor* ring, int64_t stride, int K, const int* order, int k, const float* weights, float w, int64_t n, ggml_tensor* out) {
        if (predict_k) return predict_k(backend, (const float*)ring->data, stride, order, k, weights, w, n, (float*)out->data);
        a.resize((size_t)(stride * K)), b.resize((size_t)n);
        ggml_backend_tensor_get(ring, a.data(), 0, a.size() * sizeof(float));
        spectrum_predict_host(a.data(), (size_t)stride, order, k, weights, w, (size_t)n, b.data());
        ggml_backend_tensor_set(out, b.data(), 0, (size_t)n * sizeof(float));
        return true;
    }
    bool spectrum_push(ggml_tensor* src, ggml_tensor* ring, int64_t stride, int slot, int64_t n) {
        if (push_k) return push_k(backend, (const float*)src->data, (float*)ring->data + (int64_t)slot * stride, n);
        a.resize((size_t)n);
        ggml_backend_tensor_get(src, a.data(), 0, (size_t)n * sizeof(float));
        ggml_backend_tensor_set(ring, a.data(), (size_t)slot * (size_t)stride * sizeof(float), (size_t)n * sizeof(float));
        return true;
    }
    bool record(ggml_tensor* in, ggml_tensor* out, ggml_tensor* prev_in, ggml_tensor* prev_out, ggml_tensor* diff, int64_t per, int k, int64_t nb, bool has_prev_out,
                ggml_tensor* stats) {
        if (record_k)
            return record_k(backend, (const float*)in->data, (const float*)out->data, (float*)prev_in->data, (float*)prev_out->data, (float*)diff->data, per, k, nb, has_prev_out,
                            (float*)stats->data);
        const size_t n = (size_t)(per * nb);
        a.resize(n), b.resize(n * k), c.resize(n), d.resize(n * k);
        ggml_backend_tensor_get(in, a.data(), 0, n * sizeof(float));
        ggml_backend_tensor_get(out, b.data(), 0, n * k * sizeof(float));
        if (has_prev_out) ggml_backend_tensor_get(prev_out, c.data(), 0, n * sizeof(float));
        float sums[2] = {0.0f, 0.0f};
        for (int64_t im = 0; im < nb; ++im)
            for (int64_t i = 0; i < per; ++i) {
                const size_t e = (size_t)(im * per + i), o = (size_t)(im * k * per + i);
                for (int j = 0; j < k; ++j) d[o + (size_t)j * per] = b[o + (size_t)j * per] - a[e];
                if (has_prev_out) sums[0] += std::fabs(b[o] - c[e]);
                sums[1] += std::fabs(b[o]);
                c[e] = b[o];
            }
        ggml_backend_tensor_set(diff, d.data(), 0, n * k * sizeof(float));
        ggml_backend_tensor_set(prev_in, a.data(), 0, n * sizeof(float));
        ggml_backend_tensor_set(prev_out, c.data(), 0, n * sizeof(float));
        ggml_backend_tensor_set(stats, sums, sizeof(float), sizeof(sums));
        return true;
    }
};

static bool sample_group_device(sdm_ctx_t* ctx, const sdm_img_gen_params_t* p, int b0, int nb, float* out, bool* handled) {
    *handled = false;
    const int W = p->width / 8, H = p->height / 8, C = ctx->in_channels();
    const sdm_sample_params_t& sp = p->sample_params;
    const bool use_cfg = sp.txt_cfg != 1.0f && p->uncond.c_crossattn != nullptr;
    const bool has_y   = p->cond.c_vector != nullptr;
    if (use_cfg && (p->cond.ctx_dim != p->uncond.ctx_dim || p->cond.n_tokens != p->uncond.n_tokens || has_y != (p->uncond.c_vector != nullptr))) return true;
    if (ctx->out_channels() != C) return true;
    int method, scheduler;
    float eta;
    if (!resolve_sampling(ctx, sp, method, scheduler, eta)) {
        *handled = true;
        return false;
    }
    if (method != SDM_EULER_SAMPLE_METHOD && method != SDM_EULER_A_SAMPLE_METHOD) return true;
    if (p->denoise_mask && p->init_latent) return true;
    if (ApgParams{sp.apg_eta, sp.apg_momentum, sp.apg_norm_threshold, sp.apg_norm_threshold_smoothing}.enabled()) return true;
    if (sp.slg_scale != 0.0f && sp.slg_layers && sp.slg_layer_count > 0 && ctx->is_dit && !ctx->is_flux) return true;
    *handled = true;
    const size_t per = (size_t)W * H * C;
    const std::vector<float> sigmas = call_sigmas(ctx, p, W * H, scheduler);
    const int steps                 = (int)sigmas.size() - 1;
    if (steps < 1) {
        set_error("the scheduler returned no sigma ladder for " + std::to_string(sp.sample_steps) + " steps");
        return false;
    }
    const bool euler_a              = method == SDM_EULER_A_SAMPLE_METHOD;
    const bool flow                 = ctx->is_dit;

    if (!ctx->sstate || ctx->sstate->W != W || ctx->sstate->H != H || ctx->sstate->C != C || ctx->sstate->N != nb) {
        ctx->sstate.reset(new sdm_ctx_t::SamplerState());
        auto& st = *ctx->sstate;
        ggml_init_params ip{0, nullptr, true};
        st.sctx  = ggml_init(ip);
        st.x     = ggml_new_tensor_4d(st.sctx, GGML_TYPE_F32, W, H, C, nb);
        st.noise = ggml_new_tensor_4d(st.sctx, GGML_TYPE_F32, W, H, C, nb);
        st.eps   = ggml_new_tensor_4d(st.sctx, GGML_TYPE_F32, W, H, C, nb);
        ggml_set_name(st.eps, "sampler.eps");
        ggml_set_name(st.x, "sampler.x");
        ggml_set_name(st.noise, "sampler.noise");
        st.buf = ggml_backend_alloc_ctx_tensors(st.sctx, ctx->backend);
        if (!st.buf) {
            ctx->sstate.reset();
            set_error("sampler state allocation failed");
            return false;
        }
        st.W = W, st.H = H, st.C = C, st.N = nb;
    }
    auto& st = *ctx->sstate;

    std::vector<PhiloxRNG> rngs;
    std::vector<float> x(per * nb), noise(per * nb, 0.f);
    for (int b = 0; b < nb; ++b) rngs.emplace_back((uint64_t)(p->seed + b0 + b));
    parallel_chunks((size_t)nb, [&](size_t i0, size_t i1) {
        for (size_t b = i0; b < i1; ++b) {
            std::vector<float> nz = rngs[b].randn((uint32_t)per);
            noise_scaling(&x[b * per], nz.data(), p->init_latent, per, sigmas[0], ctx->is_dit);
        }
    }, 2);
    ggml_backend_tensor_set_async(ctx->backend, st.x, x.data(), 0, x.size() * sizeof(float));
    ggml_backend_tensor_set_async(ctx->backend, st.noise, noise.data(), 0, noise.size() * sizeof(float));

    const bool pair = ctx->pair_fn != nullptr && use_cfg;
    const bool both   = use_cfg && !pair;
    const int n_model = both ? 2 * nb : nb;
    const int ctx_n   = both ? 2 : 1;
    const size_t cn   = (size_t)p->cond.ctx_dim * p->cond.n_tokens;
    const sd_condition_t& first = (pair && ctx->pair_branch == 1) ? p->uncond : p->cond;
    std::vector<float> c2(cn * ctx_n), y2;
    memcpy(&c2[0], first.c_crossattn, cn * sizeof(float));
    if (both) memcpy(&c2[cn], p->uncond.c_crossattn, cn * sizeof(float));
    if (has_y) {
        y2.resize((size_t)p->cond.vector_dim * ctx_n);
        memcpy(&y2[0], first.c_vector, p->cond.vector_dim * sizeof(float));
        if (both) memcpy(&y2[p->cond.vector_dim], p->uncond.c_vector, p->cond.vector_dim * sizeof(float));
    }
    void* pair_stream = nullptr;
    if (pair) {
        typedef void* (*get_stream_fn)(ggml_backend_t);
        ggml_backend_dev_t dev = ggml_backend_get_device(ctx->backend);
        ggml_backend_reg_t reg = dev ? ggml_backend_dev_backend_reg(dev) : nullptr;
        get_stream_fn gs       = reg ? (get_stream_fn)ggml_backend_reg_get_proc_address(reg, "ggml_backend_mi355x_get_stream") : nullptr;
        pair_stream            = gs ? gs(ctx->backend) : nullptr;
    }
    ctx->step_cache_begin_trajectory(sigmas, method);
    StepCacheRuntime& rt = ctx->step_cache;
    const int ck = both ? 2 : 1;
    StepCacheDevice cache_dev(ctx->backend);
    if ((rt.is_cachedit() || rt.spectrum_enabled) && cache_dev.mode_exports_missing) {
        set_error("step cache: the MI355X backend does not export the passes of this mode (ggml_backend_mi355x_step_cache_probe_rel / _spectrum_predict / _spectrum_push)");
        return false;
    }
    if (rt.spectrum_enabled) {
// ... 27 lines not shown
        }
        if (!st.cache || st.cache->k != ck) {
            st.cache.reset(new sdm_ctx_t::SamplerState::Cache());
            auto& cc = *st.cache;
            ggml_init_params ip{0, nullptr, true};
            cc.cctx     = ggml_init(ip);
            cc.in       = ggml_new_tensor_4d(cc.cctx, GGML_TYPE_F32, W, H, C, nb);
            cc.prev_in  = ggml_new_tensor_4d(cc.cctx, GGML_TYPE_F32, W, H, C, nb);
            cc.prev_out = ggml_new_tensor_4d(cc.cctx, GGML_TYPE_F32, W, H, C, nb);
            cc.out   = both ? ggml_new_tensor_3d(cc.cctx, GGML_TYPE_F32, (int64_t)((size_t)W * H * C), 2, nb) : ggml_new_tensor_4d(cc.cctx, GGML_TYPE_F32, W, H, C, nb);
            cc.diff  = both ? ggml_new_tensor_3d(cc.cctx, GGML_TYPE_F32, (int64_t)((size_t)W * H * C), 2, nb) : ggml_new_tensor_4d(cc.cctx, GGML_TYPE_F32, W, H, C, nb);
            cc.stats = ggml_new_tensor_1d(cc.cctx, GGML_TYPE_F32, 4);
            ggml_set_name(cc.in, "cache.in");
            ggml_set_name(cc.out, "cache.out");
            ggml_set_name(cc.prev_in, "cache.prev_in");
            ggml_set_name(cc.prev_out, "cache.prev_out");
            ggml_set_name(cc.diff, "cache.diff");
            ggml_set_name(cc.stats, "cache.stats");
            cc.buf = ggml_backend_alloc_ctx_tensors(cc.cctx, ctx->backend);
            if (!cc.buf) {
                st.cache.reset();
                set_error("step cache state allocation failed");
                return false;
            }
            cc.k = ck;
            static std::atomic<uint64_t> g_cache_serial{0};
            cc.serial = ++g_cache_serial;
        }
    }
    sdm_ctx_t::SamplerState::Cache* cc = rt.armed() ? st.cache.get() : nullptr;
    int pending = -1;
    auto book_pending = [&](const float* stats) {
        sdm_cache_step_t* rec = &rt.trace[(size_t)pending];
        const float ne        = static_cast<float>(per * (size_t)nb);
        rt.after_condition(0, stats[1] / ne, stats[2] / ne, rec);
        if (ck == 2) rt.after_condition(1, 0.0f, 0.0f, rec);
        pending = -1;
    };
    ModelSideInputs si;
    if (!prepare_side_inputs(ctx, W, H, n_model, p->cond.n_tokens, has_y, si)) return false;
    std::vector<float> ts(n_model);
    Runner& r = ctx->unet_runner;
    char step_sig[200];
    snprintf(step_sig, sizeof(step_sig), "step %d %d %d %d cfg%d ea%d %lld %lld y%lld %p pair%d", W, H, C, nb, (int)use_cfg, (int)euler_a + 2 * (int)flow, (long long)p->cond.ctx_dim,
             (long long)p->cond.n_tokens, (long long)(has_y ? p->cond.vector_dim : -1), (void*)st.x, (int)pair);
    const std::string update_sig = std::string("update ") + step_sig;
    const std::string cache_tag  = cc ? " cache" + std::to_string(cc->serial) : std::string();
    const std::string record_sig = std::string("record ") + step_sig + cache_tag;
    const std::string skip_sig   = std::string("skip ") + step_sig + cache_tag;
    const std::string spectrum_tag        = ss ? " spectrum" + std::to_string(ss->serial) : std::string();
    const std::string spectrum_record_sig = std::string("spectrum-record ") + step_sig + spectrum_tag;
    const std::string spectrum_step_sig   = std::string("spectrum-step ") + step_sig + spectrum_tag;
    const bool rel = rt.is_cachedit();

    for (int i = 0; i < steps; ++i) {
        const float sigma = sigmas[i], sigma_to = sigmas[i + 1];
        float c_skip, c_out, c_in, t_model;
        step_scalings(ctx, sp, sigma, c_skip, c_out, c_in, t_model);
        std::fill(ts.begin(), ts.end(), t_model);
        float sc[8] = {c_in, pair ? (ctx->pair_branch == 0 ? sp.txt_cfg : 1.0f - sp.txt_cfg) : sp.txt_cfg, c_out, c_skip, 0.f, 0.f, 0.f, 1.f};
        bool fresh_noise = false;
        if (euler_a) {
            if (sigma_to == 0.f) {
                sc[4] = 0.f, sc[5] = 1.f;
            } else if (eta == 0.f) {
                const float ratio = sigma_to / sigma;
                sc[4] = ratio, sc[5] = (float)(1.0 - ratio);
            } else {
                float sigma_down, sigma_up, alpha_scale = 1.f;
                if (flow)
                    ancestral_step_flow(sigma, sigma_to, eta, sigma_down, sigma_up, alpha_scale);
                else
                    ancestral_step(sigma, sigma_to, eta, sigma_down, sigma_up);
                const float ratio = sigma_down / sigma;
                sc[4] = ratio, sc[5] = 1.0f - ratio;
                if (sigma_up > 0.f) {
                    sc[6]       = sigma_up;
                    sc[7]       = alpha_scale;
                    fresh_noise = true;
                }
            }
        } else {
            sc[4] = sigma, sc[5] = sigma_to - sigma;
        }
        if (fresh_noise) {
            parallel_chunks((size_t)nb, [&](size_t i0, size_t i1) {
                for (size_t b = i0; b < i1; ++b) {
                    std::vector<float> nz = rngs[b].randn((uint32_t)per);
                    memcpy(&noise[b * per], nz.data(), per * sizeof(float));
                }
            }, 2);
            ggml_backend_tensor_set_async(ctx->backend, st.noise, noise.data(), 0, noise.size() * sizeof(float));
        }
        bool skip_step = false, record_step = false;
        if (cc) {
            const bool active  = rt.in_window(sigma);
            const bool measure = active && (pending >= 0 || rt.core().has_prev_input);
            float stats[4]     = {0.f, 0.f, 0.f, 0.f};
            if (measure && !(rel ? cache_dev.probe_rel(st.x, c_in, cc->prev_in, (int64_t)(per * (size_t)nb), cc->stats)
                                 : cache_dev.probe(st.x, c_in, cc->prev_in, (int64_t)(per * (size_t)nb), cc->stats))) {
                set_error("step cache: the probe pass could not be enqueued");
                return false;
            }
            if (measure || (pending >= 0 && !rel)) ggml_backend_tensor_get(cc->stats, stats, 0, sizeof(stats));
            if (pending >= 0) book_pending(stats);
            rt.begin_call(i + 1, sigma);
// ... 15 lines not shown
            in.push_back({tsc, sc, sizeof(sc)});
            auto S = [&](int k) { return ggml_view_1d(c, tsc, 1, (size_t)k * sizeof(float)); };
            ggml_tensor* xs     = st.x;
            ggml_tensor* noised = variant == 4 ? nullptr : ggml_mul(c, xs, S(0));
            if (variant == 1) noised = ggml_cpy(c, noised, cc->in);
            ggml_tensor *eps = nullptr, *e3 = nullptr;
            if (variant == 4) {
            } else if (variant == 2) {
                if (both) {
                    ggml_tensor* flat = ggml_reshape_3d(c, noised, (int64_t)per, 1, nb);
                    ggml_tensor* rep  = ggml_repeat(c, flat, ggml_new_tensor_3d(c, GGML_TYPE_F32, (int64_t)per, 2, nb));
                    e3                = ggml_add(c, rep, cc->diff);
                } else {
                    eps = ggml_add(c, noised, cc->diff);
                }
            } else {
                ggml_tensor* xin = noised;
                if (both) {
                    ggml_tensor* flat = ggml_reshape_3d(c, noised, (int64_t)per, 1, nb);
                    ggml_tensor* rep  = ggml_repeat(c, flat, ggml_new_tensor_3d(c, GGML_TYPE_F32, (int64_t)per, 2, nb));
                    xin               = ggml_reshape_4d(c, rep, W, H, C, 2 * nb);
                }
                eps = build_model_call(ctx, g, in, xin, n_model, ts.data(), c2.data(), p->cond.ctx_dim, p->cond.n_tokens, ctx_n,
                                       has_y ? y2.data() : nullptr, p->cond.vector_dim, ctx_n, si);
                if (pair) return ggml_cpy(c, ggml_mul(c, eps, S(1)), st.eps);
                if (both) {
                    e3 = ggml_reshape_3d(c, ggml_cont(c, eps), (int64_t)per, 2, nb);
                    if (variant == 1) e3 = ggml_cpy(c, e3, cc->out);
                } else if (variant == 1) {
                    eps = ggml_cpy(c, eps, cc->out);
                }
            }
            ggml_tensor* guided = eps;
            if (both && variant != 4) {
                ggml_tensor* ec = ggml_view_3d(c, e3, (int64_t)per, 1, nb, e3->nb[1], e3->nb[2], 0);
                ggml_tensor* eu = ggml_view_3d(c, e3, (int64_t)per, 1, nb, e3->nb[1], e3->nb[2], e3->nb[1]);
                ggml_tensor* d  = ggml_mul(c, ggml_sub(c, ec, eu), S(1));
                guided          = ggml_reshape_4d(c, ggml_add(c, eu, d), W, H, C, nb);
            }
            ggml_tensor* den = variant == 4 ? ss->denoised : ggml_add(c, ggml_mul(c, guided, S(2)), ggml_mul(c, xs, S(3)));
            if (variant == 3) den = ggml_cpy(c, den, ss->denoised);
            ggml_tensor* xn;
            if (euler_a) {
                xn = ggml_add(c, ggml_mul(c, xs, S(4)), ggml_mul(c, den, S(5)));
                if (flow) xn = ggml_mul(c, xn, S(7));
                xn = ggml_add(c, xn, ggml_mul(c, st.noise, S(6)));
            } else {
                ggml_tensor* d = ggml_div(c, ggml_sub(c, xs, den), S(4));
                xn             = ggml_add(c, xs, ggml_mul(c, d, S(5)));
            }
            return ggml_cpy(c, xn, xs);
          };
        };
        std::vector<const void*> ptrs{sc, ts.data(), c2.data()};
        if (has_y) ptrs.push_back(y2.data());
        if (ctx->is_flux) {
            ptrs.push_back(si.guidance.data());
            ptrs.push_back(si.pe().data());
        }
        if (skip_step) {
            if (!ctx->skip_runner.compute(build_variant(2), nullptr, 0, skip_sig, {sc})) return false;
            continue;
        }
        if (predict_step) {
            float weights[SpectrumState::MAX_K];
            int order[SpectrumState::MAX_K];
            const int k = rt.spectrum.predict(weights, order);
            if (!cache_dev.spectrum_predict(ss->ring, ss->stride, ss->K, order, k, weights, rt.spectrum.config.w, (int64_t)(per * (size_t)nb), ss->denoised)) {
                set_error("step cache: the spectrum forecast pass could not be enqueued");
                return false;
            }
            if (!ctx->skip_runner.compute(build_variant(4), nullptr, 0, spectrum_step_sig, {sc})) return false;
            continue;
        }
        if (!r.compute(build_variant(record_step ? 1 : (spectrum_record ? 3 : 0)), nullptr, 0,
                       record_step ? record_sig : (spectrum_record ? spectrum_record_sig : std::string(step_sig)), ptrs))
            return false;
        if (ss) {
            const int slot = rt.spectrum.update();
            if (spectrum_record && !cache_dev.spectrum_push(ss->denoised, ss->ring, ss->stride, slot, (int64_t)(per * (size_t)nb))) {
                set_error("step cache: the spectrum ring copy could not be enqueued");
                return false;
            }
        }
        if (record_step) {
            if (!cache_dev.record(cc->in, cc->out, cc->prev_in, cc->prev_out, cc->diff, (int64_t)per, ck, nb, rt.core().has_prev_output, cc->stats)) {
                set_error("step cache: the record pass could not be enqueued");
                return false;
            }
            pending = (int)rt.trace.size() - 1;
        }
        if (pair) {
            if (!ctx->pair_fn(st.eps->data, (int64_t)(per * nb), pair_stream, ctx->pair_user)) {
                set_error("CFG-pair exchange failed");
                return false;
            }
            auto update = [&](GraphCtx& g, std::vector<HostInput>& in) {
                ggml_context* c  = g.ctx;
                ggml_tensor* tsc = ggml_new_tensor_1d(c, GGML_TYPE_F32, 8);
                ggml_set_input(tsc);
                in.push_back({tsc, sc, sizeof(sc)});
                auto S = [&](int k) { return ggml_view_1d(c, tsc, 1, (size_t)k * sizeof(float)); };
                ggml_tensor* xs  = st.x;
                ggml_tensor* den = ggml_add(c, ggml_mul(c, st.eps, S(2)), ggml_mul(c, xs, S(3)));
                ggml_tensor* xn;
                if (euler_a) {
// ... 8 lines not shown
            };
            if (!ctx->pair_runner.compute(update, nullptr, 0, update_sig, {sc})) return false;
        }
    }
    ggml_backend_tensor_get(st.x, out, 0, per * nb * sizeof(float));
    if (pending >= 0) {
        float stats[4];
        ggml_backend_tensor_get(cc->stats, stats, 0, sizeof(stats));
        book_pending(stats);
    }
    ctx->stats.unet_calls  = r.calls;
    ctx->stats.graph_nodes = r.last_nodes;
    if (r.galloc) ctx->stats.compute_buffer_bytes = ggml_gallocr_get_buffer_size(r.galloc, 0);
    return true;
}

void sdm_cache_params_init(sdm_cache_params_t* p) { *p = sdm_cache_params_t{SDM_CACHE_DISABLED, INFINITY, 0.15f, 0.95f, 1.0f, true, true}; }
bool sd_set_step_cache(sdm_ctx_t* ctx, const sdm_cache_params_t* params) {
    if (params && params->mode != SDM_CACHE_DISABLED &&
        (std::isnan(params->reuse_threshold) || std::isnan(params->start_percent) || std::isnan(params->end_percent) || std::isnan(params->error_decay_rate))) {
        set_error("sd_set_step_cache: NaN parameter");
        return false;
    }
    if (params)
        ctx->cache_params = *params;
    else
        sdm_cache_params_init(&ctx->cache_params);
    if (ctx->cache_params.mode == SDM_CACHE_DISABLED && ctx->sstate) ctx->sstate->cache.reset();
    if (ctx->cache_params.mode != SDM_CACHE_SPECTRUM && ctx->sstate) ctx->sstate->spectrum.reset();
    sdm_cache_dit_params_init(&ctx->cache_dit_params);
    sdm_spectrum_params_init(&ctx->spectrum_params);
    return true;
}
void sdm_cache_dit_params_init(sdm_cache_dit_params_t* p) { *p = sdm_cache_dit_params_t{8, 0, 0.08f}; }
void sdm_spectrum_params_init(sdm_spectrum_params_t* p) { *p = sdm_spectrum_params_t{0.40f, 3, 1.0f, 2, 0.50f, 4, 0.9f}; }
bool sd_set_step_cache_ex(sdm_ctx_t* ctx, const sdm_cache_params_t* params, const sdm_cache_dit_params_t* cache_dit, const sdm_spectrum_params_t* spectrum) {
    if (cache_dit && std::isnan(cache_dit->residual_diff_threshold)) {
        set_error("sd_set_step_cache_ex: NaN parameter");
        return false;
    }
    if (spectrum && (std::isnan(spectrum->w) || std::isnan(spectrum->lam) || std::isnan(spectrum->flex_window) || std::isnan(spectrum->stop_percent))) {
        set_error("sd_set_step_cache_ex: NaN parameter");
        return false;
    }
    if (spectrum && (spectrum->m < 0 || spectrum->m > SpectrumState::MAX_K - 1)) {
        set_error("sd_set_step_cache_ex: spectrum m must be 0 .. 15 (the history holds max(m + 1, 6) <= 16 tensors)");
        return false;
    }
    if (!sd_set_step_cache(ctx, params)) return false;
    if (cache_dit) ctx->cache_dit_params = *cache_dit;
    if (spectrum) ctx->spectrum_params = *spectrum;
    return true;
}
bool sd_spectrum_schedule(const sdm_spectrum_params_t* params, int n_calls, uint8_t* predicted) {
    if (!params || n_calls < 0 || (n_calls > 0 && !predicted) || params->m < 0 || params->m > SpectrumState::MAX_K - 1) {
        set_error("sd_spectrum_schedule: bad arguments");
        return false;
    }
    SpectrumState s;
    s.init(SpectrumConfig{params->w, params->m, params->lam, params->window_size, params->flex_window, params->warmup_steps, params->stop_percent}, (size_t)n_calls);
    float weights[SpectrumState::MAX_K];
    int order[SpectrumState::MAX_K];
    for (int i = 0; i < n_calls; ++i) {
        predicted[i] = s.should_predict() ? 1 : 0;
        if (predicted[i])
            s.predict(weights, order);
        else
            s.update();
    }
    return true;
}
bool sd_spectrum_weights(const sdm_spectrum_params_t* params, const float* taus, int k, float tau_at, float* weights) {
    if (!params || !taus || !weights || k < 1 || k > SpectrumState::MAX_K || params->m < 0 || params->m > SpectrumState::MAX_K - 1) {
        set_error("sd_spectrum_weights: bad arguments");
        return false;
    }
    SpectrumState::weights(SpectrumConfig{params->w, params->m, params->lam, params->window_size, params->flex_window, params->warmup_steps, params->stop_percent}, taus, k, tau_at,
                           weights);
    return true;
}
bool sd_spectrum_kernels(sdm_ctx_t* ctx, const float* hist, int k, int64_t n, const float* weights, float w, float* out) {
    if (!hist || !weights || !out || k < 2 || k > SpectrumState::MAX_K || n < 1) {
        set_error("sd_spectrum_kernels: bad arguments");
        return false;
    }
    ggml_init_params ip{0, nullptr, true};
    ggml_context* c       = ggml_init(ip);
    const int64_t stride  = (n + 3) / 4 * 4;
    ggml_tensor* t_ring   = ggml_new_tensor_2d(c, GGML_TYPE_F32, stride, k);
    ggml_tensor* t_src    = ggml_new_tensor_1d(c, GGML_TYPE_F32, n);
    ggml_tensor* t_out    = ggml_new_tensor_1d(c, GGML_TYPE_F32, n);
    ggml_backend_buffer_t buf = ggml_backend_alloc_ctx_tensors(c, ctx->backend);
    if (!buf) {
        ggml_free(c);
        set_error("sd_spectrum_kernels: allocation failed");
        return false;
    }
    StepCacheDevice dev(ctx->backend);
    bool ok = !dev.mode_exports_missing;
    int order[SpectrumState::MAX_K];
    for (int j = 0; ok && j < k; ++j) {
        order[j] = (j + 1) % k;
        ggml_backend_tensor_set(t_src, hist + (size_t)j * (size_t)n, 0, (size_t)n * sizeof(float));
        ok = dev.spectrum_push(t_src, t_ring, stride, order[j], n);
        ggml_backend_synchronize(ctx->backend);
    }
// ... 50 lines not shown
float sd_t_to_sigma(sdm_ctx_t* ctx, float t) { return ctx->t_to_sigma(t); }
bool sd_step_cache_device_passes(sdm_ctx_t* ctx) { return StepCacheDevice(ctx->backend).on_device(); }
bool sd_step_cache_kernels(sdm_ctx_t* ctx, const float* in, const float* out, const float* prev_in, const float* prev_out, int64_t n, int k, int nb, float c_in, float* stats,
                           float* diff_out, float* prev_in_out, float* prev_out_out) {
    if (!in || !out || !prev_in || !stats || n < 1 || nb < 1 || k < 1 || k > 2) {
        set_error("sd_step_cache_kernels: bad arguments");
        return false;
    }
    ggml_init_params ip{0, nullptr, true};
    ggml_context* c = ggml_init(ip);
    ggml_tensor* t_in   = ggml_new_tensor_2d(c, GGML_TYPE_F32, n, nb);
    ggml_tensor* t_pin  = ggml_new_tensor_2d(c, GGML_TYPE_F32, n, nb);
    ggml_tensor* t_pout = ggml_new_tensor_2d(c, GGML_TYPE_F32, n, nb);
    ggml_tensor* t_out  = ggml_new_tensor_3d(c, GGML_TYPE_F32, n, k, nb);
    ggml_tensor* t_diff = ggml_new_tensor_3d(c, GGML_TYPE_F32, n, k, nb);
    ggml_tensor* t_st   = ggml_new_tensor_1d(c, GGML_TYPE_F32, 4);
    ggml_backend_buffer_t buf = ggml_backend_alloc_ctx_tensors(c, ctx->backend);
    if (!buf) {
        ggml_free(c);
        set_error("sd_step_cache_kernels: allocation failed");
        return false;
    }
    const size_t bytes = (size_t)n * nb * sizeof(float);
    const float zero[4] = {0.f, 0.f, 0.f, 0.f};
    ggml_backend_tensor_set(t_in, in, 0, bytes);
    ggml_backend_tensor_set(t_out, out, 0, bytes * k);
    ggml_backend_tensor_set(t_pin, prev_in, 0, bytes);
    if (prev_out) ggml_backend_tensor_set(t_pout, prev_out, 0, bytes);
    ggml_backend_tensor_set(t_st, zero, 0, sizeof(zero));
    StepCacheDevice dev(ctx->backend);
    const bool ok = !dev.exports_missing && dev.probe(t_in, c_in, t_pin, n * nb, t_st) && dev.record(t_in, t_out, t_pin, t_pout, t_diff, n, k, nb, prev_out != nullptr, t_st);
    if (ok) {
        float st4[4];
        ggml_backend_tensor_get(t_st, st4, 0, sizeof(st4));
        memcpy(stats, st4, 3 * sizeof(float));
        if (diff_out) ggml_backend_tensor_get(t_diff, diff_out, 0, bytes * k);
        if (prev_in_out) ggml_backend_tensor_get(t_pin, prev_in_out, 0, bytes);
        if (prev_out_out) ggml_backend_tensor_get(t_pout, prev_out_out, 0, bytes);
    } else {
        ggml_backend_synchronize(ctx->backend);
        set_error("sd_step_cache_kernels: the passes could not be run (size beyond the summation-depth bound?)");
    }
    ggml_backend_buffer_free(buf);
    ggml_free(c);
    return ok;
}

bool sd_sample_latents(sdm_ctx_t* ctx, const sdm_img_gen_params_t* p, float* out_latents) {
    const int W = p->width / 8, H = p->height / 8, C = ctx->in_channels();
    const size_t per = (size_t)W * H * C;
    const int group  = p->device_batch > 0 ? p->device_batch : p->batch_count;
    const double t0  = now_ms();
    ctx->stats.steps_skipped = 0;
    if (ctx->step_cache_would_arm(resolve_sample_method(ctx, p->sample_params.sample_method))) {
        const sdm_sample_params_t& sp = p->sample_params;
        if (ctx->is_dit && !ctx->is_flux && sp.slg_scale != 0.0f && sp.slg_layers && sp.slg_layer_count > 0) {
            set_error("step cache: not available together with skip-layer guidance");
            return false;
        }
        if (ctx->pair_fn != nullptr && p->device_sampler) {
            set_error("step cache: not available with a CFG-pair exchange (the anchor condition lives on one rank only)");
            return false;
        }
    }
    for (int b0 = 0; b0 < p->batch_count; b0 += group) {
        const int nb = std::min(group, p->batch_count - b0);
        if (p->device_sampler) {
            bool handled = false;
            if (!sample_group_device(ctx, p, b0, nb, out_latents + b0 * per, &handled)) return false;
            if (handled) {
                ctx->stats.steps_skipped += ctx->step_cache.total_steps_skipped();
                continue;
            }
        }
        if (!sample_group(ctx, p, b0, nb, out_latents + b0 * per)) return false;
        ctx->stats.steps_skipped += ctx->step_cache.total_steps_skipped();
    }
    ctx->stats.last_sample_ms = now_ms() - t0;
    return true;
}

static inline uint8_t float_to_u8(float v) {
    if (v <= 0.0f) return 0;
    if (v >= 1.0f) return 255;
    return (uint8_t)(v * 255.0f + 0.5f);
}

static void planar_rgb_to_u8(const float* f, size_t pix, uint8_t* d) {
    parallel_chunks(pix, [&](size_t i0, size_t i1) {
        for (size_t i = i0; i < i1; ++i) {
            d[i * 3 + 0] = float_to_u8(f[i]);
            d[i * 3 + 1] = float_to_u8(f[pix + i]);
            d[i * 3 + 2] = float_to_u8(f[2 * pix + i]);
        }
    });
}
void sd_planar_rgb_to_u8(const float* chw, int width, int height, uint8_t* out) { planar_rgb_to_u8(chw, (size_t)width * height, out); }

bool sdm_generate_image(sdm_ctx_t* ctx, const sdm_img_gen_params_t* p, sdm_image_t** images_out, int* num_images_out) {
    const int W = p->width / 8, H = p->height / 8, C = ctx->in_channels();
    const size_t per = (size_t)W * H * C;
    std::vector<float> latents(per * p->batch_count);
    if (!sd_sample_latents(ctx, p, latents.data())) return false;
    const int PW = W * 8, PH = H * 8;
    const size_t pix = (size_t)PW * PH;
    sdm_image_t* imgs = (sdm_image_t*)calloc(p->batch_count, sizeof(sdm_image_t));
// ... 232 lines not shown
```

### stable-diffusion.cpp_amd/csrc/host/models.hpp

```cpp
#pragma once
#include <algorithm>

#include "nn.hpp"

namespace sdmi {

struct UNetConfig {
    bool sdxl                              = false;
    int in_channels                        = 4;
    int out_channels                       = 4;
    int num_res_blocks                     = 2;
    std::vector<int> attention_resolutions = {4, 2, 1};
    std::vector<int> channel_mult          = {1, 2, 4, 4};
    std::vector<int> transformer_depth     = {1, 1, 1, 1};
    int time_embed_dim                     = 1280;
    int num_heads                          = 8;
    int num_head_channels                  = -1;
    int context_dim                        = 768;
    bool use_linear_projection             = false;
    int model_channels                     = 320;
    int adm_in_channels                    = 2816;

    static UNetConfig sd15() { return UNetConfig(); }
    static UNetConfig sdxl_base() {
// ... 83 lines not shown
            if (i != L - 1) {
                ++idx;
                Level lv;
                lv.down = std::make_unique<Conv2d>();
                lv.down->init(ps, prefix + "input_blocks." + std::to_string(idx) + ".0.op.", ch, ch, 3, 2, 1);
                input_blocks.push_back(std::move(lv));
                chans.push_back(ch);
                ds *= 2;
            }
        }
        {
            int nh, dh;
            heads(ch, nh, dh);
            mid0.res = std::make_unique<ResBlock>();
            mid0.res->init(ps, prefix + "middle_block.0.", ch, ted, ch);
            mid1.attn = std::make_unique<SpatialTransformer>();
            mid1.attn->init(ps, prefix + "middle_block.1.", ch, nh, dh, cfg.transformer_depth.back(), cfg.context_dim, cfg.use_linear_projection);
            mid2.res = std::make_unique<ResBlock>();
            mid2.res->init(ps, prefix + "middle_block.2.", ch, ted, ch);
        }
        int oidx = 0;
        for (int i = L - 1; i >= 0; --i) {
            const int mult = cfg.channel_mult[i];
            for (int j = 0; j < cfg.num_res_blocks + 1; ++j) {
                const int ich = chans.back();
                chans.pop_back();
                Level lv;
                lv.res = std::make_unique<ResBlock>();
                lv.res->init(ps, prefix + "output_blocks." + std::to_string(oidx) + ".0.", ch + ich, ted, mult * mc);
                ch         = mult * mc;
                int up_idx = 1;
                if (has_attn(ds)) {
                    int nh, dh;
                    heads(ch, nh, dh);
                    lv.attn = std::make_unique<SpatialTransformer>();
                    lv.attn->init(ps, prefix + "output_blocks." + std::to_string(oidx) + ".1.", ch, nh, dh, cfg.transformer_depth[i], cfg.context_dim, cfg.use_linear_projection);
                    ++up_idx;
                }
                if (i > 0 && j == cfg.num_res_blocks) {
                    lv.up = std::make_unique<Conv2d>();
                    lv.up->init(ps, prefix + "output_blocks." + std::to_string(oidx) + "." + std::to_string(up_idx) + ".conv.", ch, ch, 3, 1, 1);
                    ds /= 2;
                }
                output_blocks.push_back(std::move(lv));
                ++oidx;
            }
        }
        out_norm.init(ps, prefix + "out.0.", ch);
        out_conv.init(ps, prefix + "out.2.", mc, cfg.out_channels, 3, 1, 1);
    }

    ggml_tensor* forward(GraphCtx& g, ggml_tensor* x, ggml_tensor* timesteps, ggml_tensor* context, ggml_tensor* y) const {
        ggml_context* c = g.ctx;
        if (context != nullptr && context->ne[2] != x->ne[3]) {
            context = ggml_repeat(c, context, ggml_new_tensor_3d(c, GGML_TYPE_F32, context->ne[0], context->ne[1], x->ne[3]));
        }
        if (y != nullptr && y->ne[1] != x->ne[3]) {
            y = ggml_repeat(c, y, ggml_new_tensor_2d(c, GGML_TYPE_F32, y->ne[0], x->ne[3]));
        }
        ggml_tensor* t_emb = ggml_timestep_embedding(c, ext_scale(c, timesteps, 1.0f), cfg.model_channels, 10000);
        ggml_tensor* emb   = time_embed_0.forward(g, t_emb);
        emb                = ggml_silu_inplace(c, emb);
        emb                = time_embed_2.forward(g, emb);
        if (y != nullptr) {
            ggml_tensor* le = label_emb_0.forward(g, y);
            le              = ggml_silu_inplace(c, le);
            le              = label_emb_2.forward(g, le);
            emb             = ggml_add(c, emb, le);
        }
        std::vector<ggml_tensor*> hs;
        ggml_tensor* h = input_conv.forward(g, x);
        ggml_set_name(h, "bench-start");
        hs.push_back(h);
        for (auto& lv : input_blocks) {
            if (lv.down) {
                h = lv.down->forward(g, h);
            } else {
                h = lv.res->forward(g, h, emb);
                if (lv.attn) h = lv.attn->forward(g, h, context);
            }
            hs.push_back(h);
        }
        h = mid0.res->forward(g, h, emb);
        h = mid1.attn->forward(g, h, context);
        h = mid2.res->forward(g, h, emb);
        for (auto& lv : output_blocks) {
            ggml_tensor* skip = hs.back();
            hs.pop_back();
            h = ggml_concat(c, h, skip, 2);
            h = lv.res->forward(g, h, emb);
            if (lv.attn) h = lv.attn->forward(g, h, context);
            if (lv.up) {
                h = ggml_upscale(c, h, 2, GGML_SCALE_MODE_NEAREST);
                h = lv.up->forward(g, h);
            }
        }
        h = out_norm.forward(g, h);
        h = ggml_silu_inplace(c, h);
        h = out_conv.forward(g, h);
        ggml_set_name(h, "bench-end");
        return h;
    }
};

struct VaeResnetBlock {
    int64_t in_ch = 0, out_ch = 0;
    GroupNorm32 norm1, norm2;
    Conv2d conv1, conv2, nin;
    void init(ParamStore& ps, const std::string& prefix, int64_t ic, int64_t oc) {
        in_ch  = ic;
        out_ch = oc;
        norm1.init(ps, prefix + "norm1.", ic);
        conv1.init(ps, prefix + "conv1.", ic, oc, 3, 1, 1);
        norm2.init(ps, prefix + "norm2.", oc);
        conv2.init(ps, prefix + "conv2.", oc, oc, 3, 1, 1);
        if (ic != oc) nin.init(ps, prefix + "nin_shortcut.", ic, oc, 1, 1, 0);
    }
    ggml_tensor* forward(GraphCtx& g, ggml_tensor* x) const {
        ggml_context* c = g.ctx;
        ggml_tensor* h  = norm1.forward(g, x);
        h               = ggml_silu_inplace(c, h);
        h               = conv1.forward(g, h);
        h               = norm2.forward(g, h);
        h               = ggml_silu_inplace(c, h);
        h               = conv2.forward(g, h);
        if (in_ch != out_ch) x = nin.forward(g, x);
        return ggml_add(c, h, x);
    }
};

struct VaeAttnBlock {
    GroupNorm32 norm;
    Conv2d q, k, v, proj_out;
    void init(ParamStore& ps, const std::string& prefix, int64_t ch) {
        norm.init(ps, prefix + "norm.", ch);
        q.init(ps, prefix + "q.", ch, ch, 1);
        k.init(ps, prefix + "k.", ch, ch, 1);
        v.init(ps, prefix + "v.", ch, ch, 1);
        proj_out.init(ps, prefix + "proj_out.", ch, ch, 1);
    }
    ggml_tensor* forward(GraphCtx& g, ggml_tensor* x) const {
        ggml_context* cx = g.ctx;
        ggml_tensor* h_  = norm.forward(g, x);
        const int64_t n = h_->ne[3], c = h_->ne[2], h = h_->ne[1], w = h_->ne[0];
        auto tok = [&](const Conv2d& proj) {
            ggml_tensor* t = proj.forward(g, h_);
            t              = ggml_cont(cx, ggml_permute(cx, t, 1, 2, 0, 3));
            return ggml_reshape_3d(cx, t, c, h * w, n);
        };
        ggml_tensor* qq = tok(q);
        ggml_tensor* kk = tok(k);
        ggml_tensor* vv = tok(v);
        h_              = ext_attention(g, qq, kk, vv, 1);
        h_              = ggml_cont(cx, ggml_permute(cx, h_, 1, 0, 2, 3));
// ... 756 lines not shown
```

### stable-diffusion.cpp_amd/csrc/host/nn.hpp

```cpp
#pragma once
#include <cmath>
#include <cstring>
#include <functional>
#include <map>
#include <memory>
#include <string>
#include <vector>

#include "ggml.h"

namespace sdmi {

enum class InitKind { WEIGHT, BIAS, NORM_SCALE, ZERO };

struct ParamSpec {
    std::string name;
    ggml_tensor* tensor;
    InitKind kind;
    int64_t fan_in;
};

struct ParamStore {
    ggml_context* ctx = nullptr;
    std::vector<ParamSpec> specs;
    std::map<std::string, ggml_tensor*> by_name;
    ggml_type linear_type = GGML_TYPE_F16;

    ParamStore() {
        ggml_init_params p{0, nullptr, true};
        ctx = ggml_init(p);
    }
    ~ParamStore() { ggml_free(ctx); }
    ParamStore(const ParamStore&) = delete;

    ggml_tensor* add(const std::string& name, ggml_type type, std::vector<int64_t> ne, InitKind kind, int64_t fan_in) {
        ggml_tensor* t = ggml_new_tensor(ctx, type, (int)ne.size(), ne.data());
        ggml_set_name(t, name.c_str());
        specs.push_back({name, t, kind, fan_in});
        by_name[name] = t;
        return t;
    }
};

struct GraphCtx {
    ggml_context* ctx      = nullptr;
    ggml_backend_t backend = nullptr;
    bool flash_attn        = false;
    bool conv_direct       = false;
    const std::vector<int>* skip_layers = nullptr;
};

inline bool is_padded_1d(const ggml_tensor* x) {
    return x->nb[0] == ggml_type_size(x->type) && x->nb[2] == x->nb[1] * x->ne[1] && x->nb[3] == x->nb[2] * x->ne[2];
}
inline ggml_tensor* ext_scale(ggml_context* c, ggml_tensor* x, float f, bool inplace = false) {
    if (!is_padded_1d(x)) x = ggml_cont(c, x);
    return inplace ? ggml_scale_inplace(c, x, f) : ggml_scale(c, x, f);
}
inline ggml_tensor* ext_cont(ggml_context* c, ggml_tensor* x) { return ggml_is_contiguous(x) ? x : ggml_cont(c, x); }
inline ggml_tensor* ext_gelu(ggml_context* c, ggml_tensor* x, bool inplace) {
    if (!ggml_is_contiguous(x)) x = ggml_cont(c, x);
    return inplace ? ggml_gelu_inplace(c, x) : ggml_gelu(c, x);
}
inline std::vector<ggml_tensor*> ext_chunk(ggml_context* c, ggml_tensor* x, int num, int64_t dim, bool cont) {
    std::vector<ggml_tensor*> out;
    const int64_t chunk = x->ne[dim] / num;
    const size_t stride = chunk * x->nb[dim];
    int64_t ne[4]       = {x->ne[0], x->ne[1], x->ne[2], x->ne[3]};
    ne[dim]             = chunk;
    for (int i = 0; i < num; ++i) {
        ggml_tensor* v = ggml_view_4d(c, x, ne[0], ne[1], ne[2], ne[3], x->nb[1], x->nb[2], x->nb[3], stride * i);
        out.push_back(cont ? ggml_cont(c, v) : v);
    }
    return out;
}

inline ggml_tensor* ext_linear(ggml_context* c, ggml_tensor* x, ggml_tensor* w, ggml_tensor* b, bool force_prec_f32 = false, float scale = 1.f) {
    if (scale != 1.f) x = ext_scale(c, x, scale);
    if (x->ne[2] * x->ne[3] > 1024) {
        const int64_t ne2 = x->ne[2], ne3 = x->ne[3];
        x = ggml_reshape_2d(c, x, x->ne[0], x->ne[1] * x->ne[2] * x->ne[3]);
        x = ggml_mul_mat(c, w, x);
        if (force_prec_f32) ggml_mul_mat_set_prec(x, GGML_PREC_F32);
        x = ggml_reshape_4d(c, x, x->ne[0], x->ne[1] / ne2 / ne3, ne2, ne3);
    } else {
        x = ggml_mul_mat(c, w, x);
        if (force_prec_f32) ggml_mul_mat_set_prec(x, GGML_PREC_F32);
    }
    if (scale != 1.f) x = ext_scale(c, x, 1.f / scale);
    if (b != nullptr) x = ggml_add_inplace(c, x, b);
    return x;
}

inline ggml_tensor* ext_conv_2d(ggml_context* c, ggml_tensor* x, ggml_tensor* w, ggml_tensor* b, int s0, int s1, int p0, int p1, int d0, int d1, bool direct, float scale = 1.f) {
    if (scale != 1.f) x = ext_scale(c, x, scale);
    if (w->ne[2] != x->ne[2] && ggml_n_dims(w) == 2) w = ggml_reshape_4d(c, w, 1, 1, w->ne[0], w->ne[1]);
    x = direct ? ggml_conv_2d_direct(c, w, x, s0, s1, p0, p1, d0, d1) : ggml_conv_2d(c, w, x, s0, s1, p0, p1, d0, d1);
    if (scale != 1.f) x = ext_scale(c, x, 1.f / scale);
    if (b != nullptr) {
        b = ggml_reshape_4d(c, b, 1, 1, b->ne[0], 1);
        x = ggml_add_inplace(c, x, b);
    }
// ... 26 lines not shown
    ggml_context* c = g.ctx;
    int64_t L_q = q->ne[1], L_k = k->ne[1], C = q->ne[0], N = q->ne[2];
    int64_t d_head = C / n_head, n_kv_head = k->ne[0] / d_head;
    if (!skip_reshape) {
        q = ggml_reshape_4d(c, q, d_head, n_head, L_q, N);
        q = ext_cont(c, ggml_permute(c, q, 0, 2, 1, 3));
        q = ggml_reshape_3d(c, q, d_head, L_q, n_head * N);
        k = ggml_reshape_4d(c, k, d_head, n_kv_head, L_k, N);
        k = ext_cont(c, ggml_permute(c, k, 0, 2, 1, 3));
        k = ggml_reshape_3d(c, k, d_head, L_k, n_kv_head * N);
        v = ggml_reshape_4d(c, v, d_head, n_kv_head, L_k, N);
    } else {
        d_head    = v->ne[0];
        N         = v->ne[3];
        n_kv_head = k->ne[2] / N;
        C         = d_head * n_head;
    }

    const float scale = 1.0f / sqrtf((float)d_head);
    ggml_tensor* kqv  = nullptr;
    if (g.flash_attn && (mask == nullptr || mask->ne[3] == 1)) {
        ggml_tensor* k_in = ggml_cast(c, k, GGML_TYPE_F16);
        ggml_tensor* v_in = ext_cont(c, ggml_permute(c, v, 0, 2, 1, 3));
        v_in              = ggml_reshape_3d(c, v_in, d_head, L_k, n_kv_head * N);
        v_in              = ggml_cast(c, v_in, GGML_TYPE_F16);
        ggml_tensor* m_in = mask;
        if (m_in != nullptr) {
            if (m_in->ne[1] != L_q) m_in = ggml_repeat(c, m_in, ggml_new_tensor_4d(c, m_in->type, m_in->ne[0], L_q, m_in->ne[2], m_in->ne[3]));
            m_in = ggml_cast(c, m_in, GGML_TYPE_F16);
        }
        ggml_tensor* out  = ggml_flash_attn_ext(c, q, k_in, v_in, m_in, scale, 0, 0);
        if (g.backend == nullptr || ggml_backend_supports_op(g.backend, out)) {
            ggml_flash_attn_ext_set_prec(out, GGML_PREC_F32);
            kqv = ggml_view_4d(c, out, d_head, n_head, L_q, N, out->nb[1], out->nb[2], out->nb[1] * n_head, 0);
        }
    }
    if (kqv == nullptr) {
        v               = ext_cont(c, ggml_permute(c, v, 1, 2, 0, 3));
        v               = ggml_reshape_3d(c, v, L_k, d_head, n_kv_head * N);
        ggml_tensor* kq = ggml_mul_mat(c, k, q);
        ggml_mul_mat_set_prec(kq, GGML_PREC_F32);
        kq  = ggml_scale_inplace(c, kq, scale);
        if (mask) kq = ggml_add_inplace(c, kq, mask);
        kq  = ggml_soft_max_inplace(c, kq);
        kqv = ggml_mul_mat(c, v, kq);
        kqv = ggml_reshape_4d(c, kqv, d_head, L_q, n_head, N);
        kqv = ggml_permute(c, kqv, 0, 2, 1, 3);
    }
    kqv = ext_cont(c, kqv);
    kqv = ggml_reshape_3d(c, kqv, d_head * n_head, L_q, N);
    return kqv;
}

struct Linear {
    ggml_tensor *w = nullptr, *b = nullptr;
    bool force_prec_f32 = false;
    float scale         = 1.f;
    void init(ParamStore& ps, const std::string& prefix, int64_t in, int64_t out, bool bias = true, bool never_quant = false, bool force_f32 = false) {
        ggml_type t = ps.linear_type;
        if (never_quant && ggml_is_quantized(t)) t = GGML_TYPE_F16;
        if (in % ggml_blck_size(t) != 0 || force_f32) t = GGML_TYPE_F32;
        w = ps.add(prefix + "weight", t, {in, out}, InitKind::WEIGHT, in);
        if (bias) b = ps.add(prefix + "bias", GGML_TYPE_F32, {out}, InitKind::BIAS, in);
    }
    ggml_tensor* forward(GraphCtx& g, ggml_tensor* x) const { return ext_linear(g.ctx, x, w, b, force_prec_f32, scale); }
};

struct Conv2d {
    ggml_tensor *w = nullptr, *b = nullptr;
    int s = 1, p = 0;
    float scale = 1.f;
    void init(ParamStore& ps, const std::string& prefix, int64_t in, int64_t out, int k, int stride = 1, int pad = 0, bool bias = true) {
        s = stride;
        p = pad;
        w = ps.add(prefix + "weight", GGML_TYPE_F16, {k, k, in, out}, InitKind::WEIGHT, in * k * k);
        if (bias) b = ps.add(prefix + "bias", GGML_TYPE_F32, {out}, InitKind::BIAS, in * k * k);
    }
    ggml_tensor* forward(GraphCtx& g, ggml_tensor* x) const { return ext_conv_2d(g.ctx, x, w, b, s, s, p, p, 1, 1, g.conv_direct, scale); }
};

struct GroupNorm32 {
    ggml_tensor *w = nullptr, *b = nullptr;
    void init(ParamStore& ps, const std::string& prefix, int64_t ch) {
        w = ps.add(prefix + "weight", GGML_TYPE_F32, {ch}, InitKind::NORM_SCALE, ch);
        b = ps.add(prefix + "bias", GGML_TYPE_F32, {ch}, InitKind::BIAS, ch);
    }
    ggml_tensor* forward(GraphCtx& g, ggml_tensor* x) const { return ext_group_norm(g.ctx, x, w, b, 32); }
};

struct LayerNorm {
    ggml_tensor *w = nullptr, *b = nullptr;
    float eps = 1e-5f;
    void init(ParamStore& ps, const std::string& prefix, int64_t dim, float eps_ = 1e-5f) {
        eps = eps_;
        w   = ps.add(prefix + "weight", GGML_TYPE_F32, {dim}, InitKind::NORM_SCALE, dim);
        b   = ps.add(prefix + "bias", GGML_TYPE_F32, {dim}, InitKind::BIAS, dim);
    }
    ggml_tensor* forward(GraphCtx& g, ggml_tensor* x) const { return ext_layer_norm(g.ctx, x, w, b, eps); }
};

struct ResBlock {
    int64_t channels = 0, out_channels = 0;
    GroupNorm32 in_norm, out_norm;
    Conv2d in_conv, out_conv, skip;
    Linear emb;
    void init(ParamStore& ps, const std::string& prefix, int64_t ch, int64_t emb_ch, int64_t out_ch) {
// ... 9 lines not shown
    ggml_tensor* forward(GraphCtx& g, ggml_tensor* x, ggml_tensor* emb_in) const {
        ggml_context* c = g.ctx;
        ggml_tensor* h  = in_norm.forward(g, x);
        h               = ggml_silu_inplace(c, h);
        h               = in_conv.forward(g, h);
        ggml_tensor* e  = ggml_silu(c, emb_in);
        e               = emb.forward(g, e);
        e               = ggml_reshape_4d(c, e, 1, 1, e->ne[0], e->ne[1]);
        h               = ggml_add(c, h, e);
        h               = out_norm.forward(g, h);
        h               = ggml_silu_inplace(c, h);
        h               = out_conv.forward(g, h);
        if (out_channels != channels) x = skip.forward(g, x);
        return ggml_add(c, h, x);
    }
};

struct FeedForward {
    Linear proj, out;
    void init(ParamStore& ps, const std::string& prefix, int64_t dim, int64_t dim_out, int64_t mult = 4) {
        const int64_t inner = dim * mult;
        proj.init(ps, prefix + "net.0.proj.", dim, inner * 2);
        out.init(ps, prefix + "net.2.", inner, dim_out);
    }
    ggml_tensor* forward(GraphCtx& g, ggml_tensor* x) const {
        ggml_context* c   = g.ctx;
        x                 = proj.forward(g, x);
        auto parts        = ext_chunk(c, x, 2, 0, false);
        ggml_tensor* gate = ggml_cont(c, parts[1]);
        gate              = ext_gelu(c, gate, true);
        x                 = ggml_mul(c, parts[0], gate);
        return out.forward(g, x);
    }
};

struct CrossAttention {
    int64_t n_head = 0;
    Linear to_q, to_k, to_v, to_out;
    void init(ParamStore& ps, const std::string& prefix, int64_t query_dim, int64_t context_dim, int64_t heads, int64_t d_head) {
        n_head              = heads;
        const int64_t inner = heads * d_head;
        to_q.init(ps, prefix + "to_q.", query_dim, inner, false);
        to_k.init(ps, prefix + "to_k.", context_dim, inner, false);
        to_v.init(ps, prefix + "to_v.", context_dim, inner, false);
        to_out.init(ps, prefix + "to_out.0.", inner, query_dim);
    }
    ggml_tensor* forward(GraphCtx& g, ggml_tensor* x, ggml_tensor* context) const {
        ggml_tensor* q = to_q.forward(g, x);
        ggml_tensor* k = to_k.forward(g, context);
        ggml_tensor* v = to_v.forward(g, context);
        x              = ext_attention(g, q, k, v, n_head);
        return to_out.forward(g, x);
    }
};

struct BasicTransformerBlock {
    CrossAttention attn1, attn2;
    FeedForward ff;
    LayerNorm norm1, norm2, norm3;
    void init(ParamStore& ps, const std::string& prefix, int64_t dim, int64_t heads, int64_t d_head, int64_t context_dim) {
        attn1.init(ps, prefix + "attn1.", dim, dim, heads, d_head);
        attn2.init(ps, prefix + "attn2.", dim, context_dim, heads, d_head);
        ff.init(ps, prefix + "ff.", dim, dim);
        norm1.init(ps, prefix + "norm1.", dim);
        norm2.init(ps, prefix + "norm2.", dim);
        norm3.init(ps, prefix + "norm3.", dim);
    }
    ggml_tensor* forward(GraphCtx& g, ggml_tensor* x, ggml_tensor* context) const {
        ggml_context* c = g.ctx;
        ggml_tensor* r  = x;
        x               = norm1.forward(g, x);
        x               = attn1.forward(g, x, x);
        x               = ggml_add(c, x, r);
        r               = x;
        x               = norm2.forward(g, x);
        x               = attn2.forward(g, x, context);
        x               = ggml_add(c, x, r);
        r               = x;
        x               = norm3.forward(g, x);
        x               = ff.forward(g, x);
        return ggml_add(c, x, r);
    }
};

struct SpatialTransformer {
    int64_t in_channels = 0, n_head = 0, d_head = 0;
    bool use_linear = false;
    GroupNorm32 norm;
    Conv2d proj_in_c, proj_out_c;
    Linear proj_in_l, proj_out_l;
    std::vector<BasicTransformerBlock> blocks;
    void init(ParamStore& ps, const std::string& prefix, int64_t ch, int64_t heads, int64_t dh, int64_t depth, int64_t context_dim, bool linear) {
        in_channels         = ch;
        n_head              = heads;
        d_head              = dh;
        use_linear          = linear;
        const int64_t inner = heads * dh;
        norm.init(ps, prefix + "norm.", ch);
        if (linear) {
            proj_in_l.init(ps, prefix + "proj_in.", ch, inner);
        } else {
            proj_in_c.init(ps, prefix + "proj_in.", ch, inner, 1);
        }
        blocks.resize(depth);
        for (int64_t i = 0; i < depth; ++i) blocks[i].init(ps, prefix + "transformer_blocks." + std::to_string(i) + ".", inner, heads, dh, context_dim);
        if (linear) {
            proj_out_l.init(ps, prefix + "proj_out.", inner, ch);
        } else {
            proj_out_c.init(ps, prefix + "proj_out.", inner, ch, 1);
        }
    }
    ggml_tensor* forward(GraphCtx& g, ggml_tensor* x, ggml_tensor* context) const {
        ggml_context* c   = g.ctx;
        ggml_tensor* x_in = x;
        const int64_t n = x->ne[3], h = x->ne[1], w = x->ne[0], inner = n_head * d_head;
        x = norm.forward(g, x);
        if (use_linear) {
            x = ggml_cont(c, ggml_permute(c, x, 1, 2, 0, 3));
            x = ggml_reshape_3d(c, x, inner, w * h, n);
            x = proj_in_l.forward(g, x);
        } else {
            x = proj_in_c.forward(g, x);
            x = ggml_cont(c, ggml_permute(c, x, 1, 2, 0, 3));
            x = ggml_reshape_3d(c, x, inner, w * h, n);
        }
        for (auto& b : blocks) x = b.forward(g, x, context);
        if (use_linear) {
            x = proj_out_l.forward(g, x);
            x = ggml_cont(c, ggml_permute(c, x, 1, 0, 2, 3));
// ... 95 lines not shown
```

### stable-diffusion.cpp_amd/csrc/host/sampler.hpp

```cpp
#pragma once
#include <algorithm>
#include <cmath>
#include <cstdint>
#include <cstring>
#include <functional>
#include <limits>
#include <map>
#include <random>
#include <vector>

namespace sdmi {

constexpr int TIMESTEPS = 1000;

struct PhiloxRNG {
    uint64_t seed   = 0;
    uint32_t offset = 0;
    explicit PhiloxRNG(uint64_t s = 0) : seed(s) {}
    void manual_seed(uint64_t s) {
        seed   = s;
        offset = 0;
    }
    static inline void round(uint32_t c[4], const uint32_t k[2]) {
        const uint64_t p0 = (uint64_t)c[0] * 0xD2511F53u;
// ... 1156 lines not shown
        } else {
            const float x = prm.norm_threshold / diff_norm;
            factor        = x / std::pow(1.0f + std::pow(x, 1.0f / prm.norm_threshold_smoothing), prm.norm_threshold_smoothing);
        }
    }
    for (size_t k = 0; k < n; ++k) deltas[k] *= factor;
    if (prm.eta != 1.0f) {
        const float cond_norm_sq = sum_prod(cond, cond);
        if (cond_norm_sq != 0.0f) {
            const float projection_scale = sum_prod(cond, deltas.data()) / cond_norm_sq;
            const float em1              = prm.eta - 1.0f;
            for (size_t k = 0; k < n; ++k) {
                const float pc = projection_scale * cond[k];
                deltas[k] += em1 * pc;
            }
        }
    }
    if (scale != 1.0f) {
        const float sm1 = scale - 1.0f;
        for (size_t k = 0; k < n; ++k) out[k] = cond[k] + sm1 * deltas[k];
    } else {
        for (size_t k = 0; k < n; ++k) out[k] = cond[k];
    }
}

template <class NoiseFn>
inline void sampler_update(float* x, const float* denoised, size_t per, int nb, bool euler_a, bool flow, float sigma, float sigma_to, float eta, float sigma_down,
                           float sigma_up, float alpha_scale, NoiseFn&& noise) {
    const size_t n = per * (size_t)nb;
    if (!euler_a) {
        const float ds = sigma_to - sigma;
        for (size_t k = 0; k < n; ++k) {
            const float d = (x[k] - denoised[k]) / sigma;
            x[k] += d * ds;
        }
        return;
    }
    if (sigma_to == 0.f) {
        for (size_t k = 0; k < n; ++k) x[k] = denoised[k];
        return;
    }
    const float ratio = (eta == 0.f ? sigma_to : sigma_down) / sigma;
    const float one_m = 1.0f - ratio;
    for (size_t k = 0; k < n; ++k) x[k] = ratio * x[k] + one_m * denoised[k];
    if (eta != 0.f && sigma_up > 0.f) {
        if (flow)
            for (size_t k = 0; k < n; ++k) x[k] *= alpha_scale;
        for (int b = 0; b < nb; ++b) {
            const float* nz = noise(b);
            for (size_t k = 0; k < per; ++k) x[(size_t)b * per + k] += nz[k] * sigma_up;
        }
    }
}
```

### stable-diffusion.cpp_amd/csrc/kernels/kernels.h

```cpp
#pragma once
#include <hip/hip_runtime.h>
#include <stddef.h>
#include <stdint.h>

namespace mi355x {

struct View4 {
    const void* data;
    int64_t ne[4];
    int64_t nb[4];
    int type;
};

enum BinOp { BIN_ADD = 0, BIN_SUB = 1, BIN_MUL = 2, BIN_DIV = 3 };
enum UnOp { UN_SILU = 0, UN_GELU = 1, UN_GELU_QUICK = 2, UN_SIGMOID = 3, UN_TANH = 4, UN_RELU = 5, UN_NEG = 6, UN_EXP = 7 };

void launch_binary(hipStream_t s, BinOp op, void* dst, const int64_t dnb[4], const View4& a, const View4& b);
constexpr int TILE_MERGE_MAX = 32;
struct TileMergeTile {
    int x, y, w, h;
    int64_t src;
    int64_t wx, wy;
};
struct TileMergeArgs {
    TileMergeTile t[TILE_MERGE_MAX];
    int k;
    int bx, by, bw, bh;
    int planes, C;
    int64_t c_row, c_plane, c_img;
    int64_t s_row, s_plane, s_img;
    int store;
};
void launch_tile_merge(hipStream_t s, float* canvas, const float* tiles, const float* wx, const float* wy, const TileMergeArgs& a);
void launch_unary(hipStream_t s, UnOp op, float* dst, const float* src, int64_t n);
void launch_scale(hipStream_t s, float* dst, const float* src, int64_t n, float scale, float bias);
void launch_copy(hipStream_t s, const View4& dst, const View4& src);
void launch_concat(hipStream_t s, const View4& dst, const View4& a, const View4& b, int dim);
void launch_repeat(hipStream_t s, const View4& dst, const View4& src);
void launch_concat_heads(hipStream_t s, void* out, bool out_f16, const float* a, const float* b, int64_t d, int64_t H, int64_t La, int64_t Lb, int64_t N);
bool joint_heads_supported(int64_t d);
void launch_joint_heads(hipStream_t s, void* out, bool out_f16, const float* a, int64_t xsa, const float* wa, const float* b, int64_t xsb, const float* wb, float eps,
                        int64_t d, int64_t H, int64_t La, int64_t Lb, int64_t N, const float* pe = nullptr);
void launch_rope_pairs(hipStream_t s, float* out, const View4& x, const float* pe);
void launch_upscale_nearest(hipStream_t s, const View4& dst, const View4& src);
void launch_pad(hipStream_t s, const View4& dst, const View4& src, const int32_t pads[8]);
void launch_get_rows(hipStream_t s, float* dst, const int64_t dnb[4], const View4& table, const View4& ids);
void launch_timestep_embedding(hipStream_t s, float* dst, const float* t, int n, int dim, int max_period, int64_t dst_row_stride);
void launch_geglu(hipStream_t s, float* dst, const float* x, int64_t tokens, int64_t inner, int64_t x_stride);

size_t step_cache_partial_bytes();
bool launch_step_cache_probe(hipStream_t s, const float* x, float c_in, const float* prev_in, int64_t n, float* partial, float* stats);
bool launch_step_cache_record(hipStream_t s, const float* in, const float* out, float* prev_in, float* prev_out, float* diff, int64_t per, int k, int64_t nb, bool has_prev_out,
                              float* partial, float* stats2);
bool launch_step_cache_probe_rel(hipStream_t s, const float* x, float c_in, const float* prev_in, int64_t n, float* partial, float* stats);
bool launch_spectrum_predict(hipStream_t s, const float* ring, int64_t slot_stride, const int* order, int k, const float* weights, float w, int64_t n, float* out);

void launch_group_norm(hipStream_t s, float* dst, const float* x, int64_t hw, int64_t C, int64_t N, int groups, float eps,
                       const float* w, const float* b, bool silu);
void launch_layer_norm(hipStream_t s, float* dst, const float* x, int64_t ne0, int64_t nrows, int64_t x_stride, int64_t d_stride,
                       float eps, const float* w, const float* b, bool rms);
void launch_layer_norm_4d(hipStream_t s, float* dst, const float* x, const int64_t ne[4], const int64_t xnb[4], const int64_t dnb[4], float eps, const float* w,
                          const float* b, bool rms);
void launch_soft_max(hipStream_t s, float* dst, const float* x, int64_t ncols, int64_t nrows, float scale, const View4* mask,
                     int64_t rows_per_mat);
void launch_soft_max_rows_f16(hipStream_t s, void* dst16, const float* x, int64_t ncols, int64_t nrows);

void launch_mul_mat_generic(hipStream_t s, float* dst, const int64_t dne[4], const int64_t dnb[4], const View4& a, const View4& b);
void launch_im2col_f16(hipStream_t s, void* dst, int dst_type, const View4& x, int64_t KW, int64_t KH, int64_t OW, int64_t OH,
                       int s0, int s1, int p0, int p1, int d0, int d1);

size_t wswz_bytes(int64_t R, int64_t K);
void launch_wswz_linear(hipStream_t s, void* dst, const void* src, int src_type, int64_t K, int64_t R, int64_t src_row_bytes, int64_t geglu_inner = 0);
void launch_wswz_conv(hipStream_t s, void* dst, const void* src, int64_t KW, int64_t KH, int64_t IC, int64_t OC, int kblk = 0);

struct GnRec {
    float mean, m2;
};
constexpr int GN_REC_CHUNK = 256;

struct Epilogue {
    const float* bias     = nullptr;
    const float* residual = nullptr;
    const float* chan_add = nullptr;
    int64_t chan_ld       = 0;
    float scale           = 1.0f;
    int act               = -1;
    float* gn_scale       = nullptr;
    float* gn_shift       = nullptr;
    const float* gn_w     = nullptr;
    const float* gn_b     = nullptr;
    int gn_groups         = 0;
    float gn_eps          = 0.f;
    GnRec* gn_rec         = nullptr;
    void* ln_dst16        = nullptr;
    const float* ln_w     = nullptr;
    const float* ln_b     = nullptr;
    float ln_eps          = 0.f;
    const float* gate     = nullptr;
    int gate_L            = 0;
    int gelu              = 0;
    int64_t split_col     = 0;
    void* split_dst16     = nullptr;
    int64_t split_ldd16   = 0;
    int qtype             = 0;
    int64_t qrow_bytes    = 0;
    int64_t a_run_L       = 0;
    int64_t a_run_S       = 0;
};
// ... 116 lines not shown
```

Before: 372.9 it/s.

## Fuse sampler step on device and hoist cross-attention K/V projections out of loop

Adds a fused HIP kernel that applies CFG guidance, the Euler/Euler-A update and the next-step c_in input scaling in one pass, replacing several separate elementwise ops and copies per step. A trajectory-hoist mode computes the text-context cross-attention K/V projections once in a prologue graph and reuses them across denoise steps. The planner is extended so these K/V linears can write straight into their persistent buffers. This trades extra persistent memory and more code paths for fewer per-step launches and less redundant GEMM work.

New measurement: 376.5 it/s (median of 6 runs). No clear change (+1.0%).

```diff
diff --git a/include/ggml-mi355x.h b/include/ggml-mi355x.h
--- a/include/ggml-mi355x.h
+++ b/include/ggml-mi355x.h
@@ -72,6 +72,7 @@
     int64_t flash_generic_launches;
     int64_t fused_gn_epilogue;
     int64_t fused_tile_merge;
+    int64_t sampler_update_launches;
 };
 GGML_MI355X_API void ggml_backend_mi355x_get_stats(struct ggml_backend_mi355x_stats* out);
 GGML_MI355X_API int ggml_backend_mi355x_resolve_enums(const char* (*op_name)(int), const char* (*unary_op_name)(int), const char* (*type_name)(int));
@@ -107,6 +108,8 @@
 GGML_MI355X_API bool ggml_backend_mi355x_spectrum_predict(ggml_backend_t backend, const float* ring, int64_t slot_stride, const int* order, int k, const float* weights, float w,
                                                           int64_t n, float* out);
 GGML_MI355X_API bool ggml_backend_mi355x_spectrum_push(ggml_backend_t backend, const float* src, float* dst, int64_t n);
+GGML_MI355X_API bool ggml_backend_mi355x_sampler_update(ggml_backend_t backend, float* x, const float* eps, const float* noise, float* xin, int64_t per, int k, int64_t nb,
+                                                        bool euler_a, const float* sc, float c_in_next);
 GGML_MI355X_API const char* ggml_backend_mi355x_hip_library(void);
 GGML_MI355X_API int ggml_backend_mi355x_set_device(int hip_device);
 GGML_MI355X_API int ggml_backend_mi355x_get_device(void);
diff --git a/include/sd-mi355x.h b/include/sd-mi355x.h
--- a/include/sd-mi355x.h
+++ b/include/sd-mi355x.h
@@ -215,6 +215,10 @@
 SD_API bool sd_spectrum_schedule(const sdm_spectrum_params_t* params, int n_calls, uint8_t* predicted);
 SD_API bool sd_spectrum_weights(const sdm_spectrum_params_t* params, const float* taus, int k, float tau_at, float* weights);
 SD_API bool sd_spectrum_kernels(sdm_ctx_t* ctx, const float* hist, int k, int64_t n, const float* weights, float w, float* out);
+SD_API void sd_set_trajectory_hoist(sdm_ctx_t* ctx, bool on);
+SD_API bool sd_get_trajectory_hoist(sdm_ctx_t* ctx);
+SD_API bool sd_sampler_update_kernels(sdm_ctx_t* ctx, const float* x, const float* eps, const float* noise, int64_t per, int k, int nb, bool euler_a, const float* sc,
+                                      float c_in_next, float* x_out, float* xin_out);
 
 SD_API void sd_philox_randn(uint64_t seed, uint32_t offset, uint32_t n, float* out);
 SD_API void sd_philox_uint32(uint64_t seed, uint32_t offset, uint32_t n, uint32_t* out );
@@ -261,6 +265,8 @@
     double host_build_ms, host_alloc_ms, host_submit_ms;
     int64_t graph_cache_hits;
     int64_t steps_skipped;
+    int64_t sampler_update_launches;
+    int64_t prologue_computes;
 } sd_stats_t;
 SD_API void sd_get_stats(sdm_ctx_t* ctx, sd_stats_t* out);
 typedef struct {
diff --git a/stable-diffusion.cpp_amd/__init__.py b/stable-diffusion.cpp_amd/__init__.py
--- a/stable-diffusion.cpp_amd/__init__.py
+++ b/stable-diffusion.cpp_amd/__init__.py
@@ -104,7 +104,8 @@
     _fields_ = [("last_sample_ms", C.c_double), ("last_decode_ms", C.c_double), ("unet_calls", C.c_int64),
                 ("graph_nodes", C.c_int64), ("compute_buffer_bytes", C.c_size_t), ("weight_bytes", C.c_size_t),
                 ("host_build_ms", C.c_double), ("host_alloc_ms", C.c_double), ("host_submit_ms", C.c_double),
-                ("graph_cache_hits", C.c_int64), ("steps_skipped", C.c_int64)]
+                ("graph_cache_hits", C.c_int64), ("steps_skipped", C.c_int64), ("sampler_update_launches", C.c_int64),
+                ("prologue_computes", C.c_int64)]
 
 
 class SdCacheParams(C.Structure):
@@ -375,7 +376,7 @@
 _BACKEND_STAT_FIELDS = ("graphs_computed plans_built nodes_seen kernels_planned kernels_launched fused_conv fused_conv_bounced fused_linear "
                         "fused_norm fused_geglu fused_attention generic_matmul swizzled_weight_bytes graph_replays fused_linear_geglu "
                         "split_k_gemms head_major_gemms fused_modulate fused_gate fused_gelu fused_rope fused_concat_heads qgemv_linears fused_chan_add fused_proj_tokens gemm_attention fused_q16 split_k_inlaunch qgemm16_linears fgemv_linears fused_presilu fused_sibling_linears hoisted_kv_linears window_convs hoisted_emb_linears fused_rows16 fused_joint_qkv jit_images fused_cat_rows16 fused_gn_stats fused_ln_reduce redirect_fallbacks fused_concat_gn fused_conv_scale view_graphs plans_evicted hoisted_mod_linears view_external_nodes qinloop_linears flash_out_alias flash_slice_images "
-                        "flash_short_launches flash_qb2_launches flash_mslot_launches flash_generic_launches fused_gn_epilogue fused_tile_merge").split()
+                        "flash_short_launches flash_qb2_launches flash_mslot_launches flash_generic_launches fused_gn_epilogue fused_tile_merge sampler_update_launches").split()
 
 
 class BackendStats(C.Structure):
@@ -753,6 +754,29 @@
         if not L.sd_spectrum_kernels(self._ctx, _fptr(h), k, n, _fptr(wt), float(w), _fptr(out)):
             raise EngineError("sd_spectrum_kernels failed: " + L.sd_last_error().decode())
         return out
+
+    def set_trajectory_hoist(self, on: bool = True) -> None:
+        L = lib()
+        L.sd_set_trajectory_hoist.argtypes = [C.c_void_p, C.c_bool]
+        L.sd_set_trajectory_hoist.restype = None
+        L.sd_set_trajectory_hoist(self._ctx, bool(on))
+
+    def sampler_update_kernels(self, x: np.ndarray, eps: np.ndarray | None, noise: np.ndarray | None, k: int, euler_a: bool, sc, c_in_next: float, want_xin: bool = True):
+        xa = np.ascontiguousarray(x, dtype=np.float32)
+        nb, per = xa.shape
+        ea = None if eps is None else np.ascontiguousarray(eps, dtype=np.float32).reshape(nb, k, per)
+        na = None if noise is None else np.ascontiguousarray(noise, dtype=np.float32).reshape(nb, per)
+        sca = np.ascontiguousarray(sc, dtype=np.float32).reshape(8)
+        x_out = None if ea is None else np.empty_like(xa)
+        xin_out = np.empty((nb, k, per), dtype=np.float32) if want_xin else None
+        L = lib()
+        L.sd_sampler_update_kernels.argtypes = [C.c_void_p, C.c_void_p, C.c_void_p, C.c_void_p, C.c_int64, C.c_int, C.c_int, C.c_bool, C.c_void_p, C.c_float, C.c_void_p,
+                                                C.c_void_p]
+        L.sd_sampler_update_kernels.restype = C.c_bool
+        if not L.sd_sampler_update_kernels(self._ctx, _fptr(xa), _fptr(ea), _fptr(na), per, int(k), nb, bool(euler_a), _fptr(sca), float(c_in_next), _fptr(x_out),
+                                           _fptr(xin_out)):
+            raise EngineError("sd_sampler_update_kernels failed: " + L.sd_last_error().decode())
+        return x_out, xin_out
 
     def t_to_sigma(self, t: float) -> float:
         L = lib()
diff --git a/stable-diffusion.cpp_amd/csrc/backend/backend.cpp b/stable-diffusion.cpp_amd/csrc/backend/backend.cpp
--- a/stable-diffusion.cpp_amd/csrc/backend/backend.cpp
+++ b/stable-diffusion.cpp_amd/csrc/backend/backend.cpp
@@ -263,6 +263,7 @@
     if (strcmp(name, "ggml_backend_mi355x_step_cache_probe_rel") == 0) return (void*)ggml_backend_mi355x_step_cache_probe_rel;
     if (strcmp(name, "ggml_backend_mi355x_spectrum_predict") == 0) return (void*)ggml_backend_mi355x_spectrum_predict;
     if (strcmp(name, "ggml_backend_mi355x_spectrum_push") == 0) return (void*)ggml_backend_mi355x_spectrum_push;
+    if (strcmp(name, "ggml_backend_mi355x_sampler_update") == 0) return (void*)ggml_backend_mi355x_sampler_update;
     if (strcmp(name, "ggml_backend_mi355x_hip_library") == 0) return (void*)ggml_backend_mi355x_hip_library;
     if (strcmp(name, "ggml_backend_mi355x_set_device") == 0) return (void*)ggml_backend_mi355x_set_device;
     if (strcmp(name, "ggml_backend_mi355x_get_device") == 0) return (void*)ggml_backend_mi355x_get_device;
@@ -484,6 +485,15 @@
     if (hipSetDevice(c->dev->id) != hipSuccess) return false;
     return hipMemcpyAsync(dst, src, (size_t)n * sizeof(float), hipMemcpyDeviceToDevice, c->stream) == hipSuccess;
 }
+GGML_MI355X_API bool ggml_backend_mi355x_sampler_update(ggml_backend_t backend, float* x, const float* eps, const float* noise, float* xin, int64_t per, int k, int64_t nb,
+                                                        bool euler_a, const float* sc, float c_in_next) {
+    if (!backend || !x || !sc) return false;
+    mi355x::BackendCtx* c = (mi355x::BackendCtx*)backend->context;
+    if (hipSetDevice(c->dev->id) != hipSuccess) return false;
+    if (!mi355x::launch_sampler_update(c->stream, x, eps, noise, xin, per, k, nb, euler_a, sc, c_in_next)) return false;
+    mi355x::planner_count_sampler_update();
+    return true;
+}
 GGML_MI355X_API const char* ggml_backend_mi355x_hip_library(void) {
     static std::string path;
     if (path.empty()) {
diff --git a/stable-diffusion.cpp_amd/csrc/backend/planner.cpp b/stable-diffusion.cpp_amd/csrc/backend/planner.cpp
--- a/stable-diffusion.cpp_amd/csrc/backend/planner.cpp
+++ b/stable-diffusion.cpp_amd/csrc/backend/planner.cpp
@@ -1342,7 +1342,8 @@
         const ggml_tensor* x;
         int wtype;
         int64_t K, M, d, H, L;
-        bool operator<(const Key& o) const { return std::tie(x, wtype, K, M, d, H, L) < std::tie(o.x, o.wtype, o.K, o.M, o.d, o.H, o.L); }
+        bool sink;
+        bool operator<(const Key& o) const { return std::tie(x, wtype, K, M, d, H, L, sink) < std::tie(o.x, o.wtype, o.K, o.M, o.d, o.H, o.L, o.sink); }
     };
     std::map<Key, std::vector<int>> groups;
     for (int j = 0; j < gi.g->n_nodes; ++j) {
@@ -1363,12 +1364,17 @@
                 jf = c;
                 ++nread;
             }
-        if (nread != 1 || (gi.node(j5)->flags & GGML_TENSOR_FLAG_OUTPUT) || xop(gi.node(jf)) != GGML_OP_FLASH_ATTN_EXT || !planner_supports_op(gi.node(jf))) continue;
-        const ggml_tensor* f = gi.node(jf);
-        if (!((f->src[1] == gi.node(j5)) != (f->src[2] == gi.node(j5))) || f->src[0] == gi.node(j5)) continue;
+        const ggml_tensor* cp = gi.node(j5);
+        const bool sink = nread == 0 && cp->src[1] && cp->src[1] != cp && gi.idx(cp->src[1]) < 0 && cp->data == cp->src[1]->data && contig(cp) && aligned16(cp->data) &&
+                          !(cp->flags & GGML_TENSOR_FLAG_OUTPUT);
+        if (!sink) {
+            if (nread != 1 || (gi.node(j5)->flags & GGML_TENSOR_FLAG_OUTPUT) || xop(gi.node(jf)) != GGML_OP_FLASH_ATTN_EXT || !planner_supports_op(gi.node(jf))) continue;
+            const ggml_tensor* f = gi.node(jf);
+            if (!((f->src[1] == gi.node(j5)) != (f->src[2] == gi.node(j5))) || f->src[0] == gi.node(j5)) continue;
+        }
         const ggml_tensor* r4 = gi.node(j1);
         const ggml_tensor* w  = n->src[0];
-        groups[Key{x, (int)w->type, w->ne[0], w->ne[1], r4->ne[0], r4->ne[1], r4->ne[2]}].push_back(j);
+        groups[Key{x, (int)w->type, w->ne[0], w->ne[1], r4->ne[0], r4->ne[1], r4->ne[2], sink}].push_back(j);
     }
     for (auto& kv : groups) {
         std::vector<int>& mem = kv.second;
@@ -1406,12 +1412,13 @@
                 for (const auto& h : grp) B.deferred[h.node].push_back(hm_single_step(P, h));
                 continue;
             }
-            for (auto& h : grp) {
-                h.dst16_off   = B.alloc((size_t)h.tokens * h.M * 2);
-                h.dst16_arena = true;
-                h.dst16       = nullptr;
-                B.moved[gi.node(h.out_node)] = h.dst16_off;
-            }
+            if (!kv.first.sink)
+                for (auto& h : grp) {
+                    h.dst16_off   = B.alloc((size_t)h.tokens * h.M * 2);
+                    h.dst16_arena = true;
+                    h.dst16       = nullptr;
+                    B.moved[gi.node(h.out_node)] = h.dst16_off;
+                }
             STAT(hoisted_kv_linears) += (int64_t)grp.size();
             STAT(fused_sibling_linears) += (int64_t)grp.size() - 1;
             B.deferred[j0].push_back([=](hipStream_t st) {
@@ -1421,7 +1428,7 @@
                 const float* bias[16] = {};
                 const int nn = (int)grp.size();
                 for (int k = 0; k < nn; ++k) {
-                    dst16[k] = P->arena + grp[k].dst16_off;
+                    dst16[k] = grp[k].dst16_arena ? (void*)(P->arena + grp[k].dst16_off) : grp[k].dst16;
                     wswz[k]  = grp[k].swz;
                     bias[k]  = grp[k].ep.bias;
                 }
@@ -3813,6 +3820,11 @@
     }
 }
 
+void planner_count_sampler_update() {
+    STAT(sampler_update_launches)++;
+    STAT(kernels_launched)++;
+}
+
 void planner_get_stats(ggml_backend_mi355x_stats* o) {
     int64_t* out = reinterpret_cast<int64_t*>(o);
     for (size_t i = 0; i < N_STATS; ++i) out[i] = g_stat_counters[i].load();
diff --git a/stable-diffusion.cpp_amd/csrc/backend/planner.h b/stable-diffusion.cpp_amd/csrc/backend/planner.h
--- a/stable-diffusion.cpp_amd/csrc/backend/planner.h
+++ b/stable-diffusion.cpp_amd/csrc/backend/planner.h
@@ -13,6 +13,7 @@
 bool planner_supports_op(const ggml_tensor* op);
 void planner_forget_range(const void* ptr, size_t size);
 void planner_get_stats(ggml_backend_mi355x_stats* out);
+void planner_count_sampler_update();
 void planner_set_option(const char* key, int value);
 bool planner_build_op_maps(const char* (*op_name)(int), const char* (*unary_name)(int), const char* (*type_name)(int), char* err, size_t err_len);
 void planner_get_op_maps(uint8_t* ops256, uint8_t* unary256);
diff --git a/stable-diffusion.cpp_amd/csrc/host/engine.cpp b/stable-diffusion.cpp_amd/csrc/host/engine.cpp
--- a/stable-diffusion.cpp_amd/csrc/host/engine.cpp
+++ b/stable-diffusion.cpp_amd/csrc/host/engine.cpp
@@ -332,6 +332,8 @@
             const double t_b = now_ms();
             res              = build(g, local_inputs);
             ggml_set_name(res, "ggml_runner_final_result_tensor");
+            for (ggml_tensor* e : g.extra_outputs)
+                if (e != res) ggml_build_forward_expand(gf, e);
             ggml_build_forward_expand(gf, res);
             {
                 ggml_tensor* one = ggml_new_tensor_1d(cctx, GGML_TYPE_F32, 1);
@@ -474,6 +476,7 @@
         ggml_context* sctx        = nullptr;
         ggml_backend_buffer_t buf = nullptr;
         ggml_tensor *x = nullptr, *noise = nullptr, *eps = nullptr;
+        ggml_tensor *xin1 = nullptr, *xin2 = nullptr;
         int64_t W = 0, H = 0, C = 0, N = 0;
         struct Cache {
             ggml_context* cctx        = nullptr;
@@ -500,9 +503,22 @@
             }
         };
         std::unique_ptr<Spectrum> spectrum;
+        struct ContextKv {
+            ggml_context* cctx        = nullptr;
+            ggml_backend_buffer_t buf = nullptr;
+            std::vector<std::pair<ggml_tensor*, ggml_tensor*>> kv;
+            int64_t images = 0, tokens = 0;
+            uint64_t serial = 0;
+            ~ContextKv() {
+                if (buf) ggml_backend_buffer_free(buf);
+                if (cctx) ggml_free(cctx);
+            }
+        };
+        std::unique_ptr<ContextKv> context_kv;
         ~SamplerState() {
             cache.reset();
             spectrum.reset();
+            context_kv.reset();
             if (buf) ggml_backend_buffer_free(buf);
             if (sctx) ggml_free(sctx);
         }
@@ -517,6 +533,8 @@
     sdm_spectrum_params_t spectrum_params{0.40f, 3, 1.0f, 2, 0.50f, 4, 0.9f};
     StepCacheRuntime step_cache;
     Runner skip_runner;
+    Runner prologue_runner;
+    bool traj_hoist = true;
     float t_to_sigma(float t) const { return is_flux ? flux_denoiser.t_to_sigma(t) : (is_dit ? flow_denoiser.t_to_sigma(t) : denoiser.t_to_sigma(t)); }
     bool step_cache_would_arm(int method) const {
         if (!StepCacheRuntime::has_valid_cache_percent_range(cache_params)) return false;
@@ -682,6 +700,8 @@
     ctx->pair_runner.graph_size    = 256;
     ctx->skip_runner.backend       = backend;
     ctx->skip_runner.graph_size    = 256;
+    ctx->prologue_runner.backend    = backend;
+    ctx->prologue_runner.graph_size = 8192;
     ctx->vae_runner.backend        = backend;
     ctx->vae_runner.ps.linear_type = GGML_TYPE_F16;
     ctx->vae_runner.graph_size     = 20480;
@@ -2037,6 +2057,41 @@
     }
 };
 
+struct SamplerUpdateDevice {
+    typedef bool (*update_fn)(ggml_backend_t, float*, const float*, const float*, float*, int64_t, int, int64_t, bool, const float*, float);
+    ggml_backend_t backend = nullptr;
+    update_fn update_k     = nullptr;
+    bool export_missing    = false;
+    std::vector<float> hx, he, hn, hi;
+    explicit SamplerUpdateDevice(ggml_backend_t be) : backend(be) {
+        ggml_backend_dev_t dev = ggml_backend_get_device(be);
+        ggml_backend_reg_t reg = dev ? ggml_backend_dev_backend_reg(dev) : nullptr;
+        if (reg) update_k = (update_fn)ggml_backend_reg_get_proc_address(reg, "ggml_backend_mi355x_sampler_update");
+        export_missing = !update_k && reg && strcmp(ggml_backend_reg_name(reg), "MI355X") == 0;
+    }
+    bool run(ggml_tensor* x, ggml_tensor* eps, ggml_tensor* noise, ggml_tensor* xin, int64_t per, int k, int64_t nb, bool euler_a, const float* sc, float c_in_next) {
+        if (update_k)
+            return update_k(backend, (float*)x->data, eps ? (const float*)eps->data : nullptr, noise ? (const float*)noise->data : nullptr, xin ? (float*)xin->data : nullptr, per, k,
+                            nb, euler_a, sc, c_in_next);
+        const size_t n = (size_t)(per * nb);
+        hx.resize(n);
+        ggml_backend_tensor_get(x, hx.data(), 0, n * sizeof(float));
+        if (eps) {
+            he.resize(n * k);
+            ggml_backend_tensor_get(eps, he.data(), 0, n * k * sizeof(float));
+            if (euler_a) {
+                hn.resize(n);
+                ggml_backend_tensor_get(noise, hn.data(), 0, n * sizeof(float));
+            }
+        }
+        if (xin) hi.resize(n * k);
+        sampler_update_fused_host(hx.data(), eps ? he.data() : nullptr, hn.data(), xin ? hi.data() : nullptr, (size_t)per, k, (size_t)nb, euler_a, sc, c_in_next);
+        if (eps) ggml_backend_tensor_set(x, hx.data(), 0, n * sizeof(float));
+        if (xin) ggml_backend_tensor_set(xin, hi.data(), 0, n * k * sizeof(float));
+        return true;
+    }
+};
+
 static bool sample_group_device(sdm_ctx_t* ctx, const sdm_img_gen_params_t* p, int b0, int nb, float* out, bool* handled) {
     *handled = false;
     const int W = p->width / 8, H = p->height / 8, C = ctx->in_channels();
@@ -2077,6 +2132,10 @@
         ggml_set_name(st.eps, "sampler.eps");
         ggml_set_name(st.x, "sampler.x");
         ggml_set_name(st.noise, "sampler.noise");
+        st.xin1 = ggml_new_tensor_4d(st.sctx, GGML_TYPE_F32, W, H, C, nb);
+        st.xin2 = ggml_new_tensor_4d(st.sctx, GGML_TYPE_F32, W, H, C, 2 * (int64_t)nb);
+        ggml_set_name(st.xin1, "sampler.xin");
+        ggml_set_name(st.xin2, "sampler.xin_pair");
         st.buf = ggml_backend_alloc_ctx_tensors(st.sctx, ctx->backend);
         if (!st.buf) {
             ctx->sstate.reset();
@@ -2210,6 +2269,83 @@
     const std::string spectrum_record_sig = std::string("spectrum-record ") + step_sig + spectrum_tag;
     const std::string spectrum_step_sig   = std::string("spectrum-step ") + step_sig + spectrum_tag;
     const bool rel = rt.is_cachedit();
+    const bool hoist = ctx->traj_hoist && !ctx->is_dit && !ctx->is_flux && !pair && !cc && !ss;
+    SamplerUpdateDevice upd(ctx->backend);
+    if (hoist && upd.export_missing) {
+        set_error("the MI355X backend does not export the sampler-update launch (ggml_backend_mi355x_sampler_update)");
+        return false;
+    }
+    ggml_tensor* xin            = both ? st.xin2 : st.xin1;
+    const std::string model_sig = std::string("model ") + step_sig + " " + std::to_string((long long)(intptr_t)xin);
+    auto c_in_of = [&](float sg) {
+        float cs, co, ci, tm;
+        step_scalings(ctx, sp, sg, cs, co, ci, tm);
+        return ci;
+    };
+    if (hoist) {
+        const float none[8] = {0.f, 0.f, 0.f, 0.f, 0.f, 0.f, 0.f, 0.f};
+        if (!upd.run(st.x, nullptr, nullptr, xin, (int64_t)per, ck, nb, euler_a, none, c_in_of(sigmas[0]))) {
+            set_error("the sampler-update launch could not be enqueued");
+            return false;
+        }
+        ++ctx->stats.sampler_update_launches;
+    }
+    const std::vector<std::pair<ggml_tensor*, ggml_tensor*>>* kv = nullptr;
+    std::string kv_tag;
+    if (hoist && ctx->params.diffusion_flash_attn) {
+        bool flash_all = true;
+        size_t n_attn  = 0;
+        {
+            ggml_init_params ip{0, nullptr, true};
+            ggml_context* pc = ggml_init(ip);
+            ctx->unet.for_each_cross_attention([&](const CrossAttention& a) {
+                const int64_t inner = a.to_k.w->ne[1], d = inner / a.n_head;
+                ggml_tensor* q  = ggml_new_tensor_3d(pc, GGML_TYPE_F32, d, 64, a.n_head * n_model);
+                ggml_tensor* k  = ggml_new_tensor_3d(pc, GGML_TYPE_F16, d, p->cond.n_tokens, a.n_head * n_model);
+                ggml_tensor* v  = ggml_new_tensor_3d(pc, GGML_TYPE_F16, d, p->cond.n_tokens, a.n_head * n_model);
+                ggml_tensor* fa = ggml_flash_attn_ext(pc, q, k, v, nullptr, 1.0f / sqrtf((float)d), 0, 0);
+                flash_all       = flash_all && ggml_backend_supports_op(ctx->backend, fa);
+                ++n_attn;
+            });
+            ggml_free(pc);
+        }
+        if (flash_all && n_attn > 0) {
+            if (!st.context_kv || st.context_kv->images != n_model || st.context_kv->tokens != p->cond.n_tokens) {
+                st.context_kv.reset(new sdm_ctx_t::SamplerState::ContextKv());
+                auto& ck2 = *st.context_kv;
+                ggml_init_params ip{0, nullptr, true};
+                ck2.cctx = ggml_init(ip);
+                ctx->unet.for_each_cross_attention([&](const CrossAttention& a) {
+                    const int64_t inner = a.to_k.w->ne[1], d = inner / a.n_head;
+                    ggml_tensor* k = ggml_new_tensor_3d(ck2.cctx, GGML_TYPE_F16, d, p->cond.n_tokens, a.n_head * n_model);
+                    ggml_tensor* v = ggml_new_tensor_3d(ck2.cctx, GGML_TYPE_F16, d, p->cond.n_tokens, a.n_head * n_model);
+                    ggml_set_name(k, "context.k");
+                    ggml_set_name(v, "context.v");
+                    ck2.kv.emplace_back(k, v);
+                });
+                ck2.buf = ggml_backend_alloc_ctx_tensors(ck2.cctx, ctx->backend);
+                if (!ck2.buf) {
+                    st.context_kv.reset();
+                    set_error("sampler state allocation failed");
+                    return false;
+                }
+                ck2.images = n_model, ck2.tokens = p->cond.n_tokens;
+                static std::atomic<uint64_t> g_kv_serial{0};
+                ck2.serial = ++g_kv_serial;
+            }
+            kv     = &st.context_kv->kv;
+            kv_tag = " kv" + std::to_string(st.context_kv->serial);
+            auto prologue = [&](GraphCtx& g, std::vector<HostInput>& in) {
+                g.flash_attn    = ctx->params.diffusion_flash_attn;
+                ggml_tensor* tc = ggml_new_tensor_3d(g.ctx, GGML_TYPE_F32, p->cond.ctx_dim, p->cond.n_tokens, ctx_n);
+                ggml_set_input(tc);
+                in.push_back({tc, c2.data(), ggml_nbytes(tc)});
+                return ctx->unet.forward_context_kv(g, tc, n_model, *kv);
+            };
+            if (!ctx->prologue_runner.compute(prologue, nullptr, 0, std::string("prologue ") + step_sig + kv_tag, {c2.data()})) return false;
+            ++ctx->stats.prologue_computes;
+        }
+    }
 
     for (int i = 0; i < steps; ++i) {
         const float sigma = sigmas[i], sigma_to = sigmas[i + 1];
@@ -2331,6 +2467,28 @@
             return ggml_cpy(c, xn, xs);
           };
         };
+        if (hoist) {
+            auto model_only = [&](GraphCtx& g, std::vector<HostInput>& in) {
+                g.kv = kv;
+                return build_model_call(ctx, g, in, xin, n_model, ts.data(), c2.data(), p->cond.ctx_dim, p->cond.n_tokens, ctx_n, has_y ? y2.data() : nullptr, p->cond.vector_dim,
+                                        ctx_n, si);
+            };
+            std::vector<const void*> mptrs{ts.data(), c2.data()};
+            if (has_y) mptrs.push_back(y2.data());
+            if (!r.compute(model_only, nullptr, 0, model_sig + kv_tag, mptrs)) return false;
+            ggml_tensor* eps = r.cache_ctx ? r.cache_res : nullptr;
+            if (!eps || ggml_nelements(eps) != (int64_t)(per * (size_t)n_model)) {
+                set_error("device sampler: the model graph's output is not available to the sampler-update launch");
+                return false;
+            }
+            const bool last = i + 1 == steps;
+            if (!upd.run(st.x, eps, st.noise, last ? nullptr : xin, (int64_t)per, ck, nb, euler_a, sc, last ? 0.f : c_in_of(sigmas[i + 1]))) {
+                set_error("the sampler-update launch could not be enqueued");
+                return false;
+            }
+            ++ctx->stats.sampler_update_launches;
+            continue;
+        }
         std::vector<const void*> ptrs{sc, ts.data(), c2.data()};
         if (has_y) ptrs.push_back(y2.data());
         if (ctx->is_flux) {
@@ -2445,6 +2603,43 @@
     if (spectrum) ctx->spectrum_params = *spectrum;
     return true;
 }
+void sd_set_trajectory_hoist(sdm_ctx_t* ctx, bool on) { ctx->traj_hoist = on; }
+bool sd_get_trajectory_hoist(sdm_ctx_t* ctx) { return ctx->traj_hoist; }
+bool sd_sampler_update_kernels(sdm_ctx_t* ctx, const float* x, const float* eps, const float* noise, int64_t per, int k, int nb, bool euler_a, const float* sc, float c_in_next,
+                               float* x_out, float* xin_out) {
+    if (!x || per < 1 || nb < 1 || (k != 1 && k != 2) || !sc || (!eps && !xin_out) || (eps && !x_out) || (eps && euler_a && !noise)) {
+        set_error("sd_sampler_update_kernels: bad arguments");
+        return false;
+    }
+    ggml_init_params ip{0, nullptr, true};
+    ggml_context* c   = ggml_init(ip);
+    const int64_t n   = per * nb;
+    ggml_tensor* t_x  = ggml_new_tensor_1d(c, GGML_TYPE_F32, n);
+    ggml_tensor* t_e  = ggml_new_tensor_1d(c, GGML_TYPE_F32, n * k);
+    ggml_tensor* t_n  = ggml_new_tensor_1d(c, GGML_TYPE_F32, n);
+    ggml_tensor* t_in = ggml_new_tensor_1d(c, GGML_TYPE_F32, n * k);
+    ggml_backend_buffer_t buf = ggml_backend_alloc_ctx_tensors(c, ctx->backend);
+    if (!buf) {
+        ggml_free(c);
+        set_error("sd_sampler_update_kernels: allocation failed");
+        return false;
+    }
+    ggml_backend_tensor_set(t_x, x, 0, (size_t)n * sizeof(float));
+    if (eps) ggml_backend_tensor_set(t_e, eps, 0, (size_t)(n * k) * sizeof(float));
+    if (eps && euler_a) ggml_backend_tensor_set(t_n, noise, 0, (size_t)n * sizeof(float));
+    SamplerUpdateDevice dev(ctx->backend);
+    const bool ok = !dev.export_missing && dev.run(t_x, eps ? t_e : nullptr, t_n, xin_out ? t_in : nullptr, per, k, nb, euler_a, sc, c_in_next);
+    ggml_backend_synchronize(ctx->backend);
+    if (ok) {
+        if (x_out) ggml_backend_tensor_get(t_x, x_out, 0, (size_t)n * sizeof(float));
+        if (xin_out) ggml_backend_tensor_get(t_in, xin_out, 0, (size_t)(n * k) * sizeof(float));
+    } else {
+        set_error("sd_sampler_update_kernels: the launch could not be enqueued");
+    }
+    ggml_backend_buffer_free(buf);
+    ggml_free(c);
+    return ok;
+}
 bool sd_spectrum_schedule(const sdm_spectrum_params_t* params, int n_calls, uint8_t* predicted) {
     if (!params || n_calls < 0 || (n_calls > 0 && !predicted) || params->m < 0 || params->m > SpectrumState::MAX_K - 1) {
         set_error("sd_spectrum_schedule: bad arguments");
@@ -2601,6 +2796,8 @@
     const int group  = p->device_batch > 0 ? p->device_batch : p->batch_count;
     const double t0  = now_ms();
     ctx->stats.steps_skipped = 0;
+    ctx->stats.sampler_update_launches = 0;
+    ctx->stats.prologue_computes       = 0;
     if (ctx->step_cache_would_arm(resolve_sample_method(ctx, p->sample_params.sample_method))) {
         const sdm_sample_params_t& sp = p->sample_params;
         if (ctx->is_dit && !ctx->is_flux && sp.slg_scale != 0.0f && sp.slg_layers && sp.slg_layer_count > 0) {
diff --git a/stable-diffusion.cpp_amd/csrc/host/models.hpp b/stable-diffusion.cpp_amd/csrc/host/models.hpp
--- a/stable-diffusion.cpp_amd/csrc/host/models.hpp
+++ b/stable-diffusion.cpp_amd/csrc/host/models.hpp
@@ -159,6 +159,10 @@
 
     ggml_tensor* forward(GraphCtx& g, ggml_tensor* x, ggml_tensor* timesteps, ggml_tensor* context, ggml_tensor* y) const {
         ggml_context* c = g.ctx;
+        if (g.kv != nullptr) {
+            g.kv_next = 0;
+            context   = nullptr;
+        }
         if (context != nullptr && context->ne[2] != x->ne[3]) {
             context = ggml_repeat(c, context, ggml_new_tensor_3d(c, GGML_TYPE_F32, context->ne[0], context->ne[1], x->ne[3]));
         }
@@ -207,6 +211,32 @@
         h = out_conv.forward(g, h);
         ggml_set_name(h, "bench-end");
         return h;
+    }
+
+    template <class F>
+    void for_each_cross_attention(F&& f) const {
+        auto level = [&](const Level& lv) {
+            if (lv.attn)
+                for (const auto& b : lv.attn->blocks) f(b.attn2);
+        };
+        for (const auto& lv : input_blocks) level(lv);
+        level(mid1);
+        for (const auto& lv : output_blocks) level(lv);
+    }
+    ggml_tensor* forward_context_kv(GraphCtx& g, ggml_tensor* context, int64_t n, const std::vector<std::pair<ggml_tensor*, ggml_tensor*>>& kv) const {
+        ggml_context* c = g.ctx;
+        if (context->ne[2] != n) context = ggml_repeat(c, context, ggml_new_tensor_3d(c, GGML_TYPE_F32, context->ne[0], context->ne[1], n));
+        size_t i          = 0;
+        ggml_tensor* last = nullptr;
+        for_each_cross_attention([&](const CrossAttention& a) {
+            ggml_tensor* k = ext_attention_store_operand(c, a.to_k.forward(g, context), a.n_head, kv[i].first);
+            ggml_tensor* v = ext_attention_store_operand(c, a.to_v.forward(g, context), a.n_head, kv[i].second);
+            g.extra_outputs.push_back(k);
+            g.extra_outputs.push_back(v);
+            last = v;
+            ++i;
+        });
+        return last;
     }
 };
 
diff --git a/stable-diffusion.cpp_amd/csrc/host/nn.hpp b/stable-diffusion.cpp_amd/csrc/host/nn.hpp
--- a/stable-diffusion.cpp_amd/csrc/host/nn.hpp
+++ b/stable-diffusion.cpp_amd/csrc/host/nn.hpp
@@ -48,6 +48,9 @@
     bool flash_attn        = false;
     bool conv_direct       = false;
     const std::vector<int>* skip_layers = nullptr;
+    const std::vector<std::pair<ggml_tensor*, ggml_tensor*>>* kv = nullptr;
+    size_t kv_next = 0;
+    std::vector<ggml_tensor*> extra_outputs;
 };
 
 inline bool is_padded_1d(const ggml_tensor* x) {
@@ -180,6 +183,27 @@
     return kqv;
 }
 
+inline ggml_tensor* ext_attention_kv(GraphCtx& g, ggml_tensor* q, ggml_tensor* k16, ggml_tensor* v16, int64_t n_head) {
+    ggml_context* c = g.ctx;
+    const int64_t L_q = q->ne[1], C = q->ne[0], N = q->ne[2], d_head = C / n_head;
+    q = ggml_reshape_4d(c, q, d_head, n_head, L_q, N);
+    q = ext_cont(c, ggml_permute(c, q, 0, 2, 1, 3));
+    q = ggml_reshape_3d(c, q, d_head, L_q, n_head * N);
+    const float scale = 1.0f / sqrtf((float)d_head);
+    ggml_tensor* out  = ggml_flash_attn_ext(c, q, k16, v16, nullptr, scale, 0, 0);
+    ggml_flash_attn_ext_set_prec(out, GGML_PREC_F32);
+    ggml_tensor* kqv = ggml_view_4d(c, out, d_head, n_head, L_q, N, out->nb[1], out->nb[2], out->nb[1] * n_head, 0);
+    kqv              = ext_cont(c, kqv);
+    return ggml_reshape_3d(c, kqv, d_head * n_head, L_q, N);
+}
+inline ggml_tensor* ext_attention_store_operand(ggml_context* c, ggml_tensor* kv, int64_t n_head, ggml_tensor* dst16) {
+    const int64_t d_head = kv->ne[0] / n_head, L = kv->ne[1], N = kv->ne[2];
+    kv = ggml_reshape_4d(c, kv, d_head, n_head, L, N);
+    kv = ext_cont(c, ggml_permute(c, kv, 0, 2, 1, 3));
+    kv = ggml_reshape_3d(c, kv, d_head, L, n_head * N);
+    return ggml_cpy(c, kv, dst16);
+}
+
 struct Linear {
     ggml_tensor *w = nullptr, *b = nullptr;
     bool force_prec_f32 = false;
@@ -295,6 +319,11 @@
         x              = ext_attention(g, q, k, v, n_head);
         return to_out.forward(g, x);
     }
+    ggml_tensor* forward_kv(GraphCtx& g, ggml_tensor* x, ggml_tensor* k16, ggml_tensor* v16) const {
+        ggml_tensor* q = to_q.forward(g, x);
+        x              = ext_attention_kv(g, q, k16, v16, n_head);
+        return to_out.forward(g, x);
+    }
 };
 
 struct BasicTransformerBlock {
@@ -317,7 +346,12 @@
         x               = ggml_add(c, x, r);
         r               = x;
         x               = norm2.forward(g, x);
-        x               = attn2.forward(g, x, context);
+        if (g.kv != nullptr) {
+            const auto& kv = (*g.kv)[g.kv_next++];
+            x              = attn2.forward_kv(g, x, kv.first, kv.second);
+        } else {
+            x = attn2.forward(g, x, context);
+        }
         x               = ggml_add(c, x, r);
         r               = x;
         x               = norm3.forward(g, x);
diff --git a/stable-diffusion.cpp_amd/csrc/host/sampler.hpp b/stable-diffusion.cpp_amd/csrc/host/sampler.hpp
--- a/stable-diffusion.cpp_amd/csrc/host/sampler.hpp
+++ b/stable-diffusion.cpp_amd/csrc/host/sampler.hpp
@@ -1232,3 +1232,40 @@
         }
     }
 }
+
+inline void sampler_update_fused_host(float* x, const float* eps, const float* noise, float* xin, size_t per, int k, size_t nb, bool euler_a, const float* sc, float c_in_next) {
+    const float cfg = sc[1], c_out = sc[2], c_skip = sc[3], a = sc[4], b = sc[5], gain = sc[6];
+    for (size_t im = 0; im < nb; ++im)
+        for (size_t i = 0; i < per; ++i) {
+            const size_t e = im * per + i, o = im * (size_t)k * per + i;
+            float v        = x[e];
+            if (eps) {
+                float guided = eps[o];
+                if (k == 2) {
+                    volatile float d0 = eps[o] - eps[o + per];
+                    volatile float d  = d0 * cfg;
+                    guided            = eps[o + per] + d;
+                }
+                volatile float m0  = guided * c_out;
+                volatile float m1  = v * c_skip;
+                volatile float den = m0 + m1;
+                if (euler_a) {
+                    volatile float p = v * a;
+                    volatile float q = den * b;
+                    volatile float r = p + q;
+                    volatile float z = noise[e] * gain;
+                    v                = r + z;
+                } else {
+                    volatile float d1 = v - den;
+                    volatile float d  = d1 / a;
+                    volatile float s  = d * b;
+                    v                 = v + s;
+                }
+                x[e] = v;
+            }
+            if (xin) {
+                const float s = v * c_in_next;
+                for (int j = 0; j < k; ++j) xin[o + (size_t)j * per] = s;
+            }
+        }
+}
diff --git a/stable-diffusion.cpp_amd/csrc/kernels/kernels.h b/stable-diffusion.cpp_amd/csrc/kernels/kernels.h
--- a/stable-diffusion.cpp_amd/csrc/kernels/kernels.h
+++ b/stable-diffusion.cpp_amd/csrc/kernels/kernels.h
@@ -54,6 +54,9 @@
                               float* partial, float* stats2);
 bool launch_step_cache_probe_rel(hipStream_t s, const float* x, float c_in, const float* prev_in, int64_t n, float* partial, float* stats);
 bool launch_spectrum_predict(hipStream_t s, const float* ring, int64_t slot_stride, const int* order, int k, const float* weights, float w, int64_t n, float* out);
+
+bool launch_sampler_update(hipStream_t s, float* x, const float* eps, const float* noise, float* xin, int64_t per, int k, int64_t nb, bool euler_a, const float* sc,
+                           float c_in_next);
 
 void launch_group_norm(hipStream_t s, float* dst, const float* x, int64_t hw, int64_t C, int64_t N, int groups, float eps,
                        const float* w, const float* b, bool silu);
diff --git a/stable-diffusion.cpp_amd/csrc/kernels/sampler_update.hip b/stable-diffusion.cpp_amd/csrc/kernels/sampler_update.hip
--- /dev/null
+++ b/stable-diffusion.cpp_amd/csrc/kernels/sampler_update.hip
@@ -0,0 +1,103 @@
+#include "kernels.h"
+#include "ktime.h"
+#include "device_utils.h"
+
+namespace mi355x {
+
+constexpr int SU_THREADS    = 256;
+constexpr int SU_MAX_BLOCKS = 2048;
+
+struct SamplerUpdateArgs {
+    float cfg, c_out, c_skip, a, b, gain, c_in_next;
+    int k, euler_a, has_eps, has_xin;
+};
+
+__device__ __forceinline__ float su_next(float xs, float ec, float eu, float nz, const SamplerUpdateArgs& g) {
+#pragma clang fp contract(off)
+    float guided = ec;
+    if (g.k == 2) {
+        const float d0 = ec - eu;
+        const float d  = d0 * g.cfg;
+        guided         = eu + d;
+    }
+    const float m0  = guided * g.c_out;
+    const float m1  = xs * g.c_skip;
+    const float den = m0 + m1;
+    if (g.euler_a) {
+        const float p = xs * g.a;
+        const float q = den * g.b;
+        const float r = p + q;
+        const float z = nz * g.gain;
+        return r + z;
+    }
+    const float d1 = xs - den;
+    const float d  = d1 / g.a;
+    const float e  = d * g.b;
+    return xs + e;
+}
+__device__ __forceinline__ float su_scale(float x, float c) {
+#pragma clang fp contract(off)
+    return x * c;
+}
+
+__global__ __launch_bounds__(SU_THREADS) void k_sampler_update(float* __restrict__ x, const float* __restrict__ eps, const float* __restrict__ noise, float* __restrict__ xin,
+                                                                int64_t per, int64_t nb, int vec, const SamplerUpdateArgs g) {
+    const int64_t gt  = (int64_t)gridDim.x * SU_THREADS, t0 = (int64_t)blockIdx.x * SU_THREADS + threadIdx.x;
+    const int64_t nq  = vec ? (per >> 2) : 0;
+    const int64_t ipi = nq + (per - 4 * nq);
+    const int64_t items = ipi * nb;
+    for (int64_t t = t0; t < items; t += gt) {
+        const int64_t b = t / ipi, r = t - b * ipi;
+        float* xb        = x + b * per;
+        const float* ec  = g.has_eps ? eps + b * g.k * per : nullptr;
+        const float* eu  = (g.has_eps && g.k == 2) ? ec + per : nullptr;
+        const float* nzb = (g.has_eps && g.euler_a) ? noise + b * per : nullptr;
+        float* xo        = g.has_xin ? xin + b * g.k * per : nullptr;
+        if (r < nq) {
+            float4 v = ((const float4*)xb)[r];
+            if (g.has_eps) {
+                const float4 c = ((const float4*)ec)[r];
+                const float4 u = eu ? ((const float4*)eu)[r] : c;
+                const float4 z = nzb ? ((const float4*)nzb)[r] : make_float4(0.f, 0.f, 0.f, 0.f);
+                v = make_float4(su_next(v.x, c.x, u.x, z.x, g), su_next(v.y, c.y, u.y, z.y, g), su_next(v.z, c.z, u.z, z.z, g), su_next(v.w, c.w, u.w, z.w, g));
+                ((float4*)xb)[r] = v;
+            }
+            if (xo) {
+                const float4 s = make_float4(su_scale(v.x, g.c_in_next), su_scale(v.y, g.c_in_next), su_scale(v.z, g.c_in_next), su_scale(v.w, g.c_in_next));
+                for (int j = 0; j < g.k; ++j) ((float4*)(xo + (int64_t)j * per))[r] = s;
+            }
+        } else {
+            const int64_t e = 4 * nq + (r - nq);
+            float v         = xb[e];
+            if (g.has_eps) {
+                const float c = ec[e];
+                v             = su_next(v, c, eu ? eu[e] : c, nzb ? nzb[e] : 0.f, g);
+                xb[e]         = v;
+            }
+            if (xo) {
+                const float s = su_scale(v, g.c_in_next);
+                for (int j = 0; j < g.k; ++j) xo[(int64_t)j * per + e] = s;
+            }
+        }
+    }
+}
+
+static inline bool su_aligned16(const void* p) { return ((uintptr_t)p & 15) == 0; }
+
+bool launch_sampler_update(hipStream_t s, float* x, const float* eps, const float* noise, float* xin, int64_t per, int k, int64_t nb, bool euler_a, const float* sc,
+                           float c_in_next) {
+    if (!x || per < 1 || nb < 1 || (k != 1 && k != 2) || !sc || (!eps && !xin) || (eps && euler_a && !noise)) return false;
+    SamplerUpdateArgs g{sc[1], sc[2], sc[3], sc[4], sc[5], sc[6], c_in_next, k, euler_a ? 1 : 0, eps ? 1 : 0, xin ? 1 : 0};
+    const bool bases = su_aligned16(x) && (!eps || su_aligned16(eps)) && (!(eps && euler_a) || su_aligned16(noise)) && (!xin || su_aligned16(xin));
+    const int vec    = (bases && (per % 4 == 0 || nb * k == 1)) ? 1 : 0;
+    const int64_t nq = vec ? (per >> 2) : 0;
+    const int64_t items = (nq + (per - 4 * nq)) * nb;
+    int64_t blocks      = (items + SU_THREADS - 1) / SU_THREADS;
+    if (blocks > SU_MAX_BLOCKS) blocks = SU_MAX_BLOCKS;
+    const double n = (double)per * (double)nb;
+    KScope ks_(s, KF_BINARY, 0.0, n * 4.0 * ((eps ? 2.0 + k + (euler_a ? 1.0 : 0.0) : 1.0) + (xin ? k : 0)));
+    hipLaunchKernelGGL(k_sampler_update, dim3((unsigned)blocks), dim3(SU_THREADS), 0, s, x, eps, noise, xin, per, nb, vec, g);
+    return hipGetLastError() == hipSuccess;
+}
+
+}
```
